# EmilioOlivastri/IPC

Hardware: AMD Instinct MI355X
Metric: candidate-pairs/s (consistency matrix + set-max) (higher is better)
Workload: dtype f64; 1 GPU; C2: INTEL-like SE2 synthetic (V=1228, 256 true loops) + 1000 injected outliers; N=1256 candidates, 789396 cells (i<=j), 531545 solved on rank 0, s=10, fast 6.251/50, slow 11.345/100; parallelism=1 GPU

## Files before the change

__graft_entry__.py:

```python
import os
import subprocess
import sys

ROOT = os.path.dirname(os.path.abspath(__file__))
if ROOT not in sys.path:
    sys.path.insert(0, ROOT)

CSRC = os.path.join(ROOT, "ipc_amd", "csrc")
LIB = os.path.join(ROOT, "ipc_amd", "libipc_amd.so")


def _newer(target, sources):
    if not os.path.exists(target):
        return False
    t = os.path.getmtime(target)
    return all(os.path.getmtime(s) <= t for s in sources)


UNITS = ["engine.hip", "se2_block.hip", "se2_wave.hip", "se2_wave_kt.hip", "se2_pair.hip", "se2_pair_kt.hip", "se2_quad.hip",
         "se3_block.hip",
         "se3_lds_a.hip", "se3_lds_b.hip", "se3_lds_c.hip", "se3_lds_d.hip", "se3_lds_e.hip"]


HIP_FLAGS = ["--offload-arch=gfx950", "-O3", "-std=c++17", "-fPIC", "-Wno-unused-value", "-ffp-contract=on"]


def _build_lib(lib, extra_flags=(), objdir=None):
    from concurrent.futures import ThreadPoolExecutor
    hipcc = os.environ.get("HIPCC", "/opt/rocm/bin/hipcc")
    objdir = objdir or os.path.join(ROOT, "build")
    os.makedirs(objdir, exist_ok=True)
    flags = HIP_FLAGS + list(extra_flags)
    hdrs = [os.path.join(CSRC, f) for f in os.listdir(CSRC) if f.endswith((".hpp", ".h"))]
    hdrs += [os.path.join(ROOT, "include", f) for f in ("ipc_amd.h", "ipc_amd_online_exact.h")]

    def compile_unit(u):
        src, obj = os.path.join(CSRC, u), os.path.join(objdir, u.replace(".hip", ".o"))
        if not _newer(obj, [src] + hdrs) or extra_flags:
            subprocess.check_call([hipcc] + flags + ["-c", src, "-o", obj])
        return obj

    with ThreadPoolExecutor(max_workers=min(len(UNITS), os.cpu_count() or 4)) as ex:
        objs = list(ex.map(compile_unit, UNITS))
    subprocess.check_call([hipcc, "--offload-arch=gfx950", "-shared", "-fPIC", "-o", lib] + objs)


def build(force=False):
    srcs = [os.path.join(CSRC, f) for f in sorted(os.listdir(CSRC)) if f.endswith((".hip", ".hpp", ".h"))]
    srcs += [os.path.join(ROOT, "include", f) for f in ("ipc_amd.h", "ipc_amd_online_exact.h")]
    if force or not _newer(LIB, srcs):
        _build_lib(LIB)
    host = os.path.join(ROOT, "ipc_amd", "host")
    hsrc = [os.path.join(host, f) for f in ("ipc_tester.cpp", "ipc_host.cpp", "ipc_host.hpp")] + [LIB]
    for d in (2, 3):
        exe = os.path.join(host, "ipc_tester_%dD" % d)
        if force or not _newer(exe, hsrc):
            subprocess.check_call(["g++", "-O2", "-std=c++17", "-DIPC_TESTER_DIM=%d" % d, "-o", exe,
                                   os.path.join(host, "ipc_tester.cpp"), os.path.join(host, "ipc_host.cpp"),
                                   "-L" + os.path.join(ROOT, "ipc_amd"), "-lipc_amd",
                                   "-Wl,-rpath,$ORIGIN/..", "-Wl,-rpath,/opt/rocm/lib"])
    gen = os.path.join(host, "generateDataset")
    gsrc = os.path.join(host, "generate_dataset.cpp")
    if force or not _newer(gen, [gsrc]):
        subprocess.check_call(["g++", "-O2", "-std=c++17", "-o", gen, gsrc])
    from oracle import oracle as O
    O.build(force=force)
    import ipc_amd
    from ipc_amd import capi
    capi.load()


def smoke():
    import numpy as np
    from ipc_amd import capi
    capi.export_recommended_environment()
    from ipc_amd import synth
    from ipc_amd.consensus import IPC, Config, unpack_bits
    from oracle import oracle as O

    g = synth.inject_outliers(synth.small_se2(), 6, seed=3)
    cfg = Config(s_factor=10.0)
    eng = IPC(g, cfg, device=0)
    bits, acc = eng.run()
    C = unpack_bits(bits, eng.N)
    ok, _ = O.consistency_matrix(2, g.odom_meas, g.odom_info, cfg.s_factor, g.loop_ids, g.loop_meas,
                                 g.loop_info, cfg.fast_reject_th, cfg.fast_reject_iter_base,
                                 cfg.slow_reject_th, cfg.slow_reject_iter_base)
    ref_acc = O.set_max(ok, O.candidate_order(g.loop_ids))
    assert np.array_equal(C, ok), "consistency matrix differs from the oracle"
    assert np.array_equal(acc, ref_acc), "accepted set differs from the oracle"
    print("smoke OK: N=%d cells=%d accepted=%d" % (eng.N, len(eng.cell_info()), int(acc.sum())))


if __name__ == "__main__":
    build()
    if len(sys.argv) > 1 and sys.argv[1] == "smoke":
        smoke()
```

include/ipc_amd.h:

```cpp
#ifndef IPC_AMD_H
#define IPC_AMD_H

#include <stddef.h>
#include <stdint.h>

#ifdef __cplusplus
extern "C" {
#endif

typedef struct ipc_engine ipc_engine_t;

typedef enum {
    IPC_OK = 0,
    IPC_ERR_ARG = -1,
    IPC_ERR_HIP = -2,
    IPC_ERR_STATE = -3,
    IPC_ERR_LIMIT = -4
} ipc_status;

typedef struct {
    double fast_reject_th;
    int    fast_reject_iter_base;
    double slow_reject_th;
    int    slow_reject_iter_base;
    double s_factor;
} ipc_params_t;

typedef struct {
    int    i, j;
    int    lo, hi;
    double max_chi2;
    double chi2_total;
    int    iterations;
    int    tries;
    int    flags;
    int    evals;
} ipc_cell_info_t;

const char* ipc_last_error(void);

int ipc_create(int dim, int n_vertices, const double* odom_meas, const double* odom_info,
               const ipc_params_t* params, int device, ipc_engine_t** out);

int ipc_destroy(ipc_engine_t* h);

int ipc_set_candidates(ipc_engine_t* h, int n, const int* ids, const double* meas,
                       const double* info);

int ipc_append_candidate(ipc_engine_t* h, const int* ids, const double* meas, const double* info, int* index_out);

int ipc_append_odometry(ipc_engine_t* h, int n_edges, const double* meas, const double* info);
int ipc_reserve_vertices(ipc_engine_t* h, int capacity);
int ipc_vertex_count(ipc_engine_t* h, int* n_vertices);

int ipc_candidate_order(ipc_engine_t* h, int* order_out);

int ipc_initial_poses(ipc_engine_t* h, double* poses_out);


int ipc_rows_per_rank(int n, int world);

int ipc_row_assignment(int n, const int* ids, int world, int policy, int* slot_out);

int ipc_solve_rows(ipc_engine_t* h, int rank, int world, uint64_t* d_upper, void* stream);

typedef struct {
    int cells;
    int long_cells;
    int failed_cells;
    int capped_cells;
    int nan_cells;
    int damped_cells;
    int literal_cells;
} ipc_solve_report_t;
int ipc_solve_report(ipc_engine_t* h, ipc_solve_report_t* out);

int ipc_assemble_matrix(ipc_engine_t* h, const uint64_t* d_gathered, int world,
                        uint64_t* d_bits, void* stream);

int ipc_set_max(ipc_engine_t* h, const uint64_t* d_bits, uint8_t* d_accepted, void* stream);

int ipc_run(ipc_engine_t* h, uint64_t* bits_out, uint8_t* accepted_out);

int ipc_run_set_only(ipc_engine_t* h, uint8_t* accepted_out, int* solved_cells_out);

int ipc_run_sharded(ipc_engine_t** engines, int n_engines, uint64_t* bits_out, uint8_t* accepted_out);

typedef struct {
    int covered_before, covered_after;
    int cells;
    int long_cells, literal_cells, damped_cells;
    int set_max_resumed;
    int grew;
} ipc_online_report_t;
int ipc_run_online(ipc_engine_t* h, uint64_t* bits_out, uint8_t* accepted_out, ipc_online_report_t* report);
int ipc_online_covered(ipc_engine_t* h, int* m);
int ipc_online_reset(ipc_engine_t* h);
int ipc_reserve_candidates(ipc_engine_t* h, int capacity);

typedef struct {
    int thresholds;
    int cells;
    int long_cells, damped_cells;
    int literal_cells;
    int literal_held;
    int reused_solve;
    int chunks;
} ipc_sweep_report_t;
int ipc_run_sweep(ipc_engine_t* h, int n_th, const double* fast_th, const double* slow_th, uint64_t* bits_out,
                  uint8_t* accepted_out, ipc_sweep_report_t* report);
int ipc_sweep_reset(ipc_engine_t* h);

typedef struct {
    int runs;
    int union_candidates;
    int cells;
    long long cells_separate;
    int long_cells, damped_cells, literal_cells;
    int chunks;
} ipc_batch_report_t;
int ipc_run_batch(ipc_engine_t* h, int n_runs, const int* run_offsets, const int* members, uint64_t* bits_out,
                  uint8_t* accepted_out, ipc_batch_report_t* report);

typedef struct {
    int live;
    int greedy_size;
    int best_size;
    int best_seed;
    int best_seed_position;
} ipc_multistart_report_t;
int ipc_set_max_multistart(ipc_engine_t* h, const uint64_t* d_bits, uint8_t* d_accepted, int32_t* d_sizes, void* stream);
int ipc_run_multistart(ipc_engine_t* h, uint64_t* bits_out, uint8_t* accepted_out, uint8_t* greedy_out, int32_t* sizes_out,
                       ipc_multistart_report_t* report);

typedef struct {
    int live, multistart_size, size, upper_bound, proven;
    int subproblems;
    int capped;
    long long steps;
} ipc_exact_report_t;
int ipc_set_max_exact(ipc_engine_t* h, const uint64_t* d_bits, uint8_t* d_accepted, ipc_exact_report_t* report, void* stream);
int ipc_run_exact(ipc_engine_t* h, uint64_t* bits_out, uint8_t* accepted_out, uint8_t* multistart_out, ipc_exact_report_t* report);

#include "ipc_amd_online_exact.h"

int ipc_cell_count(ipc_engine_t* h, int* n_cells);
int ipc_cell_info(ipc_engine_t* h, ipc_cell_info_t* out, int capacity);

int ipc_solver_time_ms(ipc_engine_t* h, double* ms, int* launches);

int ipc_synchronize(ipc_engine_t* h);


typedef struct {
    int    lo, hi;
    int    n_cluster_loops;
    int    iterations, tries, flags;
    double max_chi2;
    double chi2_total;
    double chi2_initial;
} ipc_check_info_t;

int ipc_incremental_reset(ipc_engine_t* h);

int ipc_incremental_prepare(ipc_engine_t* h);

int ipc_agreement_check(ipc_engine_t* h, int k, int* agrees, ipc_check_info_t* info);

typedef struct {
    long host_solver_fallbacks, lost_launches, relaunches, literal_band_solves;
} ipc_incremental_counters_t;
int ipc_incremental_counters(ipc_engine_t* h, ipc_incremental_counters_t* out);

int ipc_consensus_size(ipc_engine_t* h, int* n);
int ipc_consensus_set(ipc_engine_t* h, int* out);

int ipc_remove_from_consensus(ipc_engine_t* h, int k, int* removed);
int ipc_add_to_consensus(ipc_engine_t* h, int k);

int ipc_current_poses(ipc_engine_t* h, double* poses_out);

int ipc_incremental_set_state(ipc_engine_t* h, const double* poses, const int* cns, int n_cns, int resume_position);

int ipc_final_optimize(ipc_engine_t* h, const uint8_t* accepted, int iterations, double* poses_out,
                       ipc_check_info_t* info);

int ipc_debug_dense_solve(int n, const double* system, int mode, int workgroups, double* x_out, int* info_out);

int ipc_debug_band_solve(int nb, int m, int W, const double* system, int workgroups, double* x_out, int* info_out);
int ipc_debug_absorbed_edges(int klo, int khi, int n, const int* lo, const int* hi, int sweep, int* members_out, int* n_members_out,
                             int* lo_out, int* hi_out);
int ipc_debug_band_plan(int d, int nl, const int* a, const int* b, int min_n, int* use_out, int* nlb_out, int* bwb_out,
                        int* order_out);
int ipc_debug_live_resources(int out[3]);

#ifdef __cplusplus
}
#endif
#endif
```

ipc_amd/capi.py:

```python
import ctypes as C
import os

import numpy as np



def export_recommended_environment():
    os.environ.setdefault("GPU_MAX_HW_QUEUES", "24")


_HERE = os.path.dirname(os.path.abspath(__file__))
LIB_PATH = os.environ.get("IPC_AMD_LIB") or os.path.join(_HERE, "libipc_amd.so")

SYMBOLS = [
    "ipc_last_error", "ipc_create", "ipc_destroy", "ipc_set_candidates", "ipc_candidate_order",
    "ipc_initial_poses", "ipc_rows_per_rank", "ipc_solve_rows", "ipc_assemble_matrix", "ipc_set_max",
    "ipc_run", "ipc_cell_count", "ipc_cell_info", "ipc_solve_report", "ipc_solver_time_ms", "ipc_synchronize",
    "ipc_incremental_reset", "ipc_incremental_prepare", "ipc_agreement_check", "ipc_consensus_size", "ipc_consensus_set",
    "ipc_remove_from_consensus", "ipc_add_to_consensus", "ipc_current_poses", "ipc_final_optimize",
    "ipc_debug_dense_solve", "ipc_debug_band_solve", "ipc_debug_band_plan", "ipc_debug_absorbed_edges", "ipc_append_candidate", "ipc_incremental_set_state", "ipc_incremental_counters", "ipc_row_assignment", "ipc_run_sharded", "ipc_run_set_only",
    "ipc_append_odometry", "ipc_reserve_vertices", "ipc_vertex_count",
    "ipc_run_online", "ipc_online_covered", "ipc_online_reset", "ipc_reserve_candidates", "ipc_debug_live_resources",
    "ipc_run_sweep", "ipc_sweep_reset",
    "ipc_run_batch",
    "ipc_set_max_multistart", "ipc_run_multistart",
    "ipc_set_max_exact", "ipc_run_exact",
]
SYMBOLS_ONLINE_EXACT = ["ipc_set_max_exact_resume", "ipc_run_online_exact", "ipc_online_exact_state"]


class Params(C.Structure):
    _fields_ = [("fast_reject_th", C.c_double), ("fast_reject_iter_base", C.c_int),
                ("slow_reject_th", C.c_double), ("slow_reject_iter_base", C.c_int),
                ("s_factor", C.c_double)]


class CellInfo(C.Structure):
    _fields_ = [("i", C.c_int), ("j", C.c_int), ("lo", C.c_int), ("hi", C.c_int),
                ("max_chi2", C.c_double), ("chi2_total", C.c_double),
                ("iterations", C.c_int), ("tries", C.c_int), ("flags", C.c_int), ("evals", C.c_int)]


class CheckInfo(C.Structure):
    _fields_ = [("lo", C.c_int), ("hi", C.c_int), ("n_cluster_loops", C.c_int), ("iterations", C.c_int),
                ("tries", C.c_int), ("flags", C.c_int), ("max_chi2", C.c_double), ("chi2_total", C.c_double),
                ("chi2_initial", C.c_double)]


class IncrementalCounters(C.Structure):
    _fields_ = [("host_solver_fallbacks", C.c_long), ("lost_launches", C.c_long), ("relaunches", C.c_long),
                ("literal_band_solves", C.c_long)]


class SolveReport(C.Structure):
    _fields_ = [("cells", C.c_int), ("long_cells", C.c_int), ("failed_cells", C.c_int), ("capped_cells", C.c_int),
                ("nan_cells", C.c_int), ("damped_cells", C.c_int), ("literal_cells", C.c_int)]


class OnlineReport(C.Structure):
    _fields_ = [("covered_before", C.c_int), ("covered_after", C.c_int), ("cells", C.c_int), ("long_cells", C.c_int),
                ("literal_cells", C.c_int), ("damped_cells", C.c_int), ("set_max_resumed", C.c_int), ("grew", C.c_int)]


class SweepReport(C.Structure):
    _fields_ = [("thresholds", C.c_int), ("cells", C.c_int), ("long_cells", C.c_int), ("damped_cells", C.c_int),
                ("literal_cells", C.c_int), ("literal_held", C.c_int), ("reused_solve", C.c_int), ("chunks", C.c_int)]


class BatchReport(C.Structure):
    _fields_ = [("runs", C.c_int), ("union_candidates", C.c_int), ("cells", C.c_int), ("cells_separate", C.c_longlong),
                ("long_cells", C.c_int), ("damped_cells", C.c_int), ("literal_cells", C.c_int), ("chunks", C.c_int)]


class MultistartReport(C.Structure):
    _fields_ = [("live", C.c_int), ("greedy_size", C.c_int), ("best_size", C.c_int), ("best_seed", C.c_int),
                ("best_seed_position", C.c_int)]


class ExactReport(C.Structure):
    _fields_ = [("live", C.c_int), ("multistart_size", C.c_int), ("size", C.c_int), ("upper_bound", C.c_int),
                ("proven", C.c_int), ("subproblems", C.c_int), ("capped", C.c_int), ("steps", C.c_longlong)]


class ExactResumeReport(C.Structure):
    _fields_ = [("first", C.c_int), ("live", C.c_int), ("newcomers", C.c_int), ("size_before", C.c_int),
                ("multistart_size", C.c_int), ("size", C.c_int), ("upper_bound", C.c_int), ("proven", C.c_int),
                ("changed", C.c_int), ("subproblems", C.c_int), ("capped", C.c_int), ("steps", C.c_longlong)]


CELL_DTYPE = np.dtype([("i", "<i4"), ("j", "<i4"), ("lo", "<i4"), ("hi", "<i4"), ("max_chi2", "<f8"),
                       ("chi2_total", "<f8"), ("iterations", "<i4"), ("tries", "<i4"), ("flags", "<i4"),
                       ("evals", "<i4")])

_lib = None


class IpcError(RuntimeError):
    pass


def load():
    global _lib
    if _lib is not None:
        return _lib
    if not os.path.exists(LIB_PATH):
        raise IpcError("libipc_amd.so is not built (%s); run `python -c 'import __graft_entry__ as g; "
                       "g.build()'` -- there is no CPU fallback" % LIB_PATH)
    try:
        import torch
    except ImportError:
        pass
    lib = C.CDLL(LIB_PATH)
    lib.ipc_last_error.restype = C.c_char_p
    vp, ip, dp = C.c_void_p, C.c_int, C.c_double
    lib.ipc_create.argtypes = [ip, ip, vp, vp, C.POINTER(Params), ip, C.POINTER(vp)]
    lib.ipc_destroy.argtypes = [vp]
    lib.ipc_set_candidates.argtypes = [vp, ip, vp, vp, vp]
    lib.ipc_append_candidate.argtypes = [vp, vp, vp, vp, C.POINTER(ip)]
    lib.ipc_append_odometry.argtypes = [vp, ip, vp, vp]
    lib.ipc_reserve_vertices.argtypes = [vp, ip]
    lib.ipc_vertex_count.argtypes = [vp, C.POINTER(ip)]
    lib.ipc_candidate_order.argtypes = [vp, vp]
    lib.ipc_initial_poses.argtypes = [vp, vp]
    lib.ipc_rows_per_rank.argtypes = [ip, ip]
    lib.ipc_row_assignment.argtypes = [ip, vp, ip, ip, vp]
    lib.ipc_solve_rows.argtypes = [vp, ip, ip, vp, vp]
    lib.ipc_assemble_matrix.argtypes = [vp, vp, ip, vp, vp]
    lib.ipc_set_max.argtypes = [vp, vp, vp, vp]
    lib.ipc_run.argtypes = [vp, vp, vp]
    lib.ipc_run_online.argtypes = [vp, vp, vp, C.POINTER(OnlineReport)]
    lib.ipc_online_covered.argtypes = [vp, C.POINTER(ip)]
    lib.ipc_online_reset.argtypes = [vp]
    lib.ipc_reserve_candidates.argtypes = [vp, ip]
    lib.ipc_run_sweep.argtypes = [vp, ip, vp, vp, vp, vp, C.POINTER(SweepReport)]
    lib.ipc_sweep_reset.argtypes = [vp]
    lib.ipc_run_batch.argtypes = [vp, ip, vp, vp, vp, vp, C.POINTER(BatchReport)]
    lib.ipc_set_max_multistart.argtypes = [vp, vp, vp, vp, vp]
    lib.ipc_run_multistart.argtypes = [vp, vp, vp, vp, vp, C.POINTER(MultistartReport)]
    lib.ipc_set_max_exact.argtypes = [vp, vp, vp, C.POINTER(ExactReport), vp]
    lib.ipc_run_exact.argtypes = [vp, vp, vp, vp, C.POINTER(ExactReport)]
    lib.ipc_set_max_exact_resume.argtypes = [vp, vp, ip, vp, C.POINTER(ExactResumeReport), vp]
    lib.ipc_run_online_exact.argtypes = [vp, vp, vp, vp, C.POINTER(OnlineReport), C.POINTER(ExactResumeReport)]
    lib.ipc_online_exact_state.argtypes = [vp, C.POINTER(ip), C.POINTER(ip)]
    lib.ipc_run_sharded.argtypes =[C.POINTER(vp), ip, vp, vp]
    lib.ipc_run_set_only.argtypes = [vp, vp, C.POINTER(ip)]
    lib.ipc_cell_count.argtypes = [vp, C.POINTER(ip)]
    lib.ipc_cell_info.argtypes = [vp, vp, ip]
    lib.ipc_solve_report.argtypes = [vp, C.POINTER(SolveReport)]
    lib.ipc_solver_time_ms.argtypes = [vp, C.POINTER(dp), C.POINTER(ip)]
    lib.ipc_synchronize.argtypes = [vp]
    lib.ipc_incremental_reset.argtypes = [vp]
    lib.ipc_incremental_prepare.argtypes = [vp]
    lib.ipc_agreement_check.argtypes = [vp, ip, C.POINTER(ip), C.POINTER(CheckInfo)]
    lib.ipc_consensus_size.argtypes = [vp, C.POINTER(ip)]
    lib.ipc_consensus_set.argtypes = [vp, vp]
    lib.ipc_remove_from_consensus.argtypes = [vp, ip, C.POINTER(ip)]
    lib.ipc_add_to_consensus.argtypes = [vp, ip]
    lib.ipc_current_poses.argtypes = [vp, vp]
    lib.ipc_incremental_set_state.argtypes = [vp, vp, vp, ip, ip]
    lib.ipc_incremental_counters.argtypes = [vp, C.POINTER(IncrementalCounters)]
    lib.ipc_final_optimize.argtypes = [vp, vp, ip, vp, C.POINTER(CheckInfo)]
    lib.ipc_debug_dense_solve.argtypes = [ip, vp, ip, ip, vp, C.POINTER(ip)]
    lib.ipc_debug_band_solve.argtypes = [ip, ip, ip, vp, ip, vp, C.POINTER(ip)]
    lib.ipc_debug_absorbed_edges.argtypes = [ip, ip, ip, vp, vp, ip, vp, C.POINTER(ip), C.POINTER(ip), C.POINTER(ip)]
    lib.ipc_debug_band_plan.argtypes = [ip, ip, vp, vp, ip, C.POINTER(ip), C.POINTER(ip), C.POINTER(ip), vp]
    lib.ipc_debug_live_resources.argtypes = [C.POINTER(ip * 3)]
    assert C.sizeof(CellInfo) == CELL_DTYPE.itemsize
    _lib = lib
    return lib


def check(rc):
    if rc != 0:
        raise IpcError("ipc_amd error %d: %s" % (rc, load().ipc_last_error().decode()))
```

ipc_amd/consensus.py:

```python
import ctypes as C
from dataclasses import dataclass

import numpy as np

from . import capi
from .graphio import PoseGraph


@dataclass
class Config:
    fast_reject_th: float = 6.251
    fast_reject_iter_base: int = 50
    slow_reject_th: float = 11.345
    slow_reject_iter_base: int = 100
    s_factor: float = 10.0
    canonic_inliers: int = 0


def _d(a):
    return np.ascontiguousarray(a, dtype=np.float64)


def _p(a):
    return a.ctypes.data_as(C.c_void_p)
# ... 117 lines not shown
        capi.check(self.lib.ipc_reserve_candidates(self.h, int(n)))

    def run_sweep(self, fast_ths, slow_ths, want_bits=False):
        fast, slow = _d(fast_ths).reshape(-1), _d(slow_ths).reshape(-1)
        assert fast.shape == slow.shape
        T = int(fast.shape[0])
        acc = np.zeros((T, self.N), dtype=np.uint8)
        bits = np.zeros((T, self.N, self.words), dtype=np.uint64) if want_bits else None
        r = capi.SweepReport()
        capi.check(self.lib.ipc_run_sweep(self.h, T, _p(fast), _p(slow), _p(bits) if want_bits else None, _p(acc), C.byref(r)))
        report = {k: getattr(r, k) for k, _ in capi.SweepReport._fields_}
        return (bits, acc, report) if want_bits else (acc, report)

    def sweep_reset(self):
        capi.check(self.lib.ipc_sweep_reset(self.h))

    def run_batch(self, runs, want_bits=False):
        runs = [np.ascontiguousarray(r, dtype=np.int32).reshape(-1) for r in runs]
        sizes = [int(r.shape[0]) for r in runs]
        offsets = np.zeros(len(runs) + 1, dtype=np.int32)
        offsets[1:] = np.cumsum(sizes)
        members = np.ascontiguousarray(np.concatenate(runs) if runs else np.zeros(0), dtype=np.int32)
        mats = [n * ((n + 63) // 64) for n in sizes]
        acc = np.zeros(max(int(offsets[-1]), 1), dtype=np.uint8)
        bits = np.zeros(max(sum(mats), 1), dtype=np.uint64) if want_bits else None
        r = capi.BatchReport()
        capi.check(self.lib.ipc_run_batch(self.h, len(runs), _p(offsets), _p(members), _p(bits) if want_bits else None, _p(acc),
                                          C.byref(r)))
        report = {k: getattr(r, k) for k, _ in capi.BatchReport._fields_}
        accs = [acc[offsets[q]:offsets[q + 1]] for q in range(len(runs))]
        if not want_bits:
            return accs, report
        mo = np.concatenate([[0], np.cumsum(mats)])
        return [bits[mo[q]:mo[q + 1]].reshape(sizes[q], -1) for q in range(len(runs))], accs, report

    def run_multistart(self, want_bits=False):
        acc = np.zeros(self.N, dtype=np.uint8)
        greedy = np.zeros(self.N, dtype=np.uint8)
        sizes = np.zeros(self.N, dtype=np.int32)
        bits = np.zeros((self.N, self.words), dtype=np.uint64) if want_bits else None
        r = capi.MultistartReport()
        capi.check(self.lib.ipc_run_multistart(self.h, _p(bits) if want_bits else None, _p(acc), _p(greedy), _p(sizes), C.byref(r)))
        report = {k: getattr(r, k) for k, _ in capi.MultistartReport._fields_}
        return (bits, acc, greedy, sizes, report) if want_bits else (acc, greedy, sizes, report)

    def run_exact(self, want_bits=False):
        acc = np.zeros(self.N, dtype=np.uint8)
        ms = np.zeros(self.N, dtype=np.uint8)
        bits = np.zeros((self.N, self.words), dtype=np.uint64) if want_bits else None
        r = capi.ExactReport()
        capi.check(self.lib.ipc_run_exact(self.h, _p(bits) if want_bits else None, _p(acc), _p(ms), C.byref(r)))
        report = {k: getattr(r, k) for k, _ in capi.ExactReport._fields_}
        return (bits, acc, ms, report) if want_bits else (acc, ms, report)

    def consistency_matrix(self):
        bits, _ = self.run()
        return unpack_bits(bits, self.N)

    def getMaxConsensusSet(self):
        return self._max_consensus_set

    def reset(self):
        capi.check(self.lib.ipc_incremental_reset(self.h))
        self._max_consensus_set = np.zeros(0, dtype=np.int32)

    def agreementCheck(self, k, with_info=False):
        ok, info = C.c_int(0), capi.CheckInfo()
        capi.check(self.lib.ipc_agreement_check(self.h, int(k), C.byref(ok), C.byref(info)))
        self._max_consensus_set = self._consensus()
        return (bool(ok.value), info) if with_info else bool(ok.value)

    def _consensus(self):
        n = C.c_int(0)
        capi.check(self.lib.ipc_consensus_size(self.h, C.byref(n)))
        out = np.zeros(max(n.value, 1), dtype=np.int32)
        capi.check(self.lib.ipc_consensus_set(self.h, _p(out)))
        return out[:n.value]

    def removeEdgeFromCnS(self, k):
        r = C.c_int(0)
        capi.check(self.lib.ipc_remove_from_consensus(self.h, int(k), C.byref(r)))
        self._max_consensus_set = self._consensus()
        return bool(r.value)

    def addEdgeToCnS(self, k):
        capi.check(self.lib.ipc_add_to_consensus(self.h, int(k)))
        self._max_consensus_set = self._consensus()

    def current_poses(self):
        out = np.zeros((self.n_vertices, 3 if self.dim == 2 else 12))
        capi.check(self.lib.ipc_current_poses(self.h, _p(out)))
        return out

    def set_state(self, poses, consensus, resume_position=0):
        poses = _d(poses)
        assert poses.shape == (self.n_vertices, 3 if self.dim == 2 else 12)
        cns = np.ascontiguousarray(consensus, dtype=np.int32)
        capi.check(self.lib.ipc_incremental_set_state(self.h, _p(poses), _p(cns), int(cns.shape[0]), int(resume_position)))
        self._max_consensus_set = cns.copy()

    def incremental_counters(self):
        c = capi.IncrementalCounters()
        capi.check(self.lib.ipc_incremental_counters(self.h, C.byref(c)))
        return {k: getattr(c, k) for k, _ in capi.IncrementalCounters._fields_}

    def final_optimize(self, accepted, iterations=1000):
        acc = np.ascontiguousarray(accepted, dtype=np.uint8)
        out = np.zeros((self.n_vertices, 3 if self.dim == 2 else 12))
        info = capi.CheckInfo()
        capi.check(self.lib.ipc_final_optimize(self.h, _p(acc), int(iterations), _p(out), C.byref(info)))
        return out, info

    def rows_per_rank(self, world):
        return self.lib.ipc_rows_per_rank(self.N, world)

    def solve_rows(self, rank, world, d_upper_ptr, stream=0):
        capi.check(self.lib.ipc_solve_rows(self.h, rank, world, C.c_void_p(d_upper_ptr), C.c_void_p(stream)))

    def assemble_matrix(self, d_gathered_ptr, world, d_bits_ptr, stream=0):
        capi.check(self.lib.ipc_assemble_matrix(self.h, C.c_void_p(d_gathered_ptr), world,
                                                C.c_void_p(d_bits_ptr), C.c_void_p(stream)))

    def set_max(self, d_bits_ptr, d_accepted_ptr, stream=0):
        capi.check(self.lib.ipc_set_max(self.h, C.c_void_p(d_bits_ptr), C.c_void_p(d_accepted_ptr),
                                        C.c_void_p(stream)))

    def set_max_multistart(self, d_bits_ptr, d_accepted_ptr, d_sizes_ptr=0, stream=0):
        capi.check(self.lib.ipc_set_max_multistart(self.h, C.c_void_p(d_bits_ptr), C.c_void_p(d_accepted_ptr),
                                                   C.c_void_p(d_sizes_ptr) if d_sizes_ptr else None, C.c_void_p(stream)))

    def set_max_exact(self, d_bits_ptr, d_accepted_ptr, stream=0):
        r = capi.ExactReport()
        capi.check(self.lib.ipc_set_max_exact(self.h, C.c_void_p(d_bits_ptr), C.c_void_p(d_accepted_ptr), C.byref(r), C.c_void_p(stream)))
        return {k: getattr(r, k) for k, _ in capi.ExactReport._fields_}

    def set_max_exact_resume(self, d_bits_ptr, first, d_accepted_ptr, stream=0):
        r = capi.ExactResumeReport()
        capi.check(self.lib.ipc_set_max_exact_resume(self.h, C.c_void_p(d_bits_ptr), int(first), C.c_void_p(d_accepted_ptr), C.byref(r),
                                                     C.c_void_p(stream)))
        return {k: getattr(r, k) for k, _ in capi.ExactResumeReport._fields_}

    def cell_info(self):
        n = C.c_int(0)
        capi.check(self.lib.ipc_cell_count(self.h, C.byref(n)))
        out = np.zeros(max(n.value, 1), dtype=capi.CELL_DTYPE)
        capi.check(self.lib.ipc_cell_info(self.h, _p(out), n.value))
        return out[:n.value]

    def solve_report(self):
        r = capi.SolveReport()
        capi.check(self.lib.ipc_solve_report(self.h, C.byref(r)))
        return {k: getattr(r, k) for k, _ in capi.SolveReport._fields_}

    def solver_time_ms(self):
        ms, nl = C.c_double(0), C.c_int(0)
        capi.check(self.lib.ipc_solver_time_ms(self.h, C.byref(ms), C.byref(nl)))
        return ms.value, nl.value

    def synchronize(self):
        capi.check(self.lib.ipc_synchronize(self.h))

    def close(self):
        if getattr(self, "h", None) is not None and self.h:
            self.lib.ipc_destroy(self.h)
            self.h = None

    def __del__(self):
        try:
            self.close()
        except Exception:
            pass


def unpack_bits(bits, N):
    b = np.ascontiguousarray(bits, dtype=np.uint64)
    u8 = b.view(np.uint8).reshape(b.shape[0], -1)
    return np.unpackbits(u8, axis=1, bitorder="little")[:, :N].astype(np.uint8)
```

ipc_amd/csrc/cell_kernels.hpp:

```cpp
#pragma once
#include <hip/hip_runtime.h>

#include "se2_cell.hpp"
#include "se3_cell.hpp"

namespace ipc {

struct CellOut {
    double* max_chi2;
    double* chi2_total;
    int4* meta;
};

struct Variant { int W, M; };
static const Variant kVariants[] = {
    {1, 1}, {2, 1}, {3, 1}, {4, 1}, {5, 1}, {6, 1}, {7, 1}, {8, 1}, {10, 1}, {12, 1}, {14, 1}, {16, 1},
    {4, 2}, {5, 2}, {6, 2}, {7, 2}, {8, 2}, {10, 2}, {12, 2}, {16, 2},
    {5, 3}, {6, 3}, {7, 3}, {8, 3},
    {4, 4}, {6, 4}, {8, 4}, {16, 4}, {16, 8}, {16, 16},
    {2, 3}, {2, 4}, {2, 5}, {2, 6},
    {3, 4}, {3, 5}, {3, 6}, {4, 3}, {4, 5},
};
constexpr int kNumVariants = sizeof(kVariants) / sizeof(kVariants[0]);
static const Variant kVariants3[] = { {1, 1}, {2, 1}, {4, 1}, {8, 1}, {16, 1}, {16, 2}, {16, 4},
                                      {4, 2}, {4, 4}, {8, 2}, {8, 4}, {4, 8}, {8, 5},
                                      {1, 2}, {2, 2}, {1, 4}, {2, 4}, {1, 3}, {2, 3} };
constexpr int kNumVariants3 = sizeof(kVariants3) / sizeof(kVariants3[0]);

hipError_t launch_se2_block(int nl, int variant, int n, hipStream_t st, const Se2View& P, const int2* cells,
                            SolveParams prm, CellOut out);
hipError_t launch_se3_block(int nl, int variant, int n, hipStream_t st, const Se3View& P, const int2* cells,
                            SolveParams prm, CellOut out);

struct LdsVariant { int W, M; };
static const LdsVariant kLdsVariants3[] = { {1, 1}, {1, 2}, {1, 3}, {1, 4}, {1, 6}, {1, 8},
                                            {4, 2}, {4, 3}, {4, 4}, {4, 5}, {4, 6}, {4, 7}, {4, 8}, {4, 9}, {4, 10} };
constexpr int kNumLdsVariants3 = sizeof(kLdsVariants3) / sizeof(kLdsVariants3[0]);
constexpr int kLdsVariantBase3 = 400;
#define IPC_SE3_LDS_DECL(WW, MM)                                                                                \
    hipError_t launch_se3_lds_##WW##_##MM(int nl, int n, hipStream_t st, const Se3View& P, const int2* cells,   \
                                          SolveParams prm, CellOut out, unsigned* counter, int n_cu);
IPC_SE3_LDS_DECL(1, 1) IPC_SE3_LDS_DECL(1, 2) IPC_SE3_LDS_DECL(1, 3) IPC_SE3_LDS_DECL(1, 4) IPC_SE3_LDS_DECL(1, 6)
IPC_SE3_LDS_DECL(1, 8) IPC_SE3_LDS_DECL(4, 2) IPC_SE3_LDS_DECL(4, 3) IPC_SE3_LDS_DECL(4, 4) IPC_SE3_LDS_DECL(4, 5)
IPC_SE3_LDS_DECL(4, 6) IPC_SE3_LDS_DECL(4, 7) IPC_SE3_LDS_DECL(4, 8) IPC_SE3_LDS_DECL(4, 9) IPC_SE3_LDS_DECL(4, 10)
#undef IPC_SE3_LDS_DECL

static const int kWaveM[] = {1, 3, 5, 7, 9, 11, 13};
constexpr int kNumWaveM = sizeof(kWaveM) / sizeof(kWaveM[0]);
constexpr int kWaveVariantBase = 100;

hipError_t launch_se2_wave(int nl, int M, int n, hipStream_t st, const Se2View& P, const int2* cells,
                           SolveParams prm, CellOut out, unsigned* counter, int n_cu);

static const int kPairM[] = {5, 7, 9, 11};
constexpr int kNumPairM = sizeof(kPairM) / sizeof(kPairM[0]);
constexpr int kPairVariantBase = 200;
hipError_t launch_se2_pair(int nl, int M, int n, hipStream_t st, const Se2View& P, const int2* cells,
                           SolveParams prm, CellOut out, unsigned* counter, int n_cu);

static const int kQuadM[] = {7, 9, 11, 13};
constexpr int kNumQuadM = sizeof(kQuadM) / sizeof(kQuadM[0]);
constexpr int kQuadVariantBase = 300;
hipError_t launch_se2_quad(int nl, int M, int n, hipStream_t st, const Se2View& P, const int2* cells,
                           SolveParams prm, CellOut out, unsigned* counter, int n_cu);

static const int kWaveKtM[] = {5, 7, 9, 11};
constexpr int kNumWaveKtM = sizeof(kWaveKtM) / sizeof(kWaveKtM[0]);
constexpr int kWaveKtVariantBase = 500;
hipError_t launch_se2_wave_kt(int nl, int M, int n, hipStream_t st, const Se2View& P, const int2* cells,
                              SolveParams prm, CellOut out, unsigned* counter, int n_cu);
static const int kPairKtM[] = {7, 9, 11};
constexpr int kNumPairKtM = sizeof(kPairKtM) / sizeof(kPairKtM[0]);
constexpr int kPairKtVariantBase = 600;
hipError_t launch_se2_pair_kt(int nl, int M, int n, hipStream_t st, const Se2View& P, const int2* cells,
                              SolveParams prm, CellOut out, unsigned* counter, int n_cu);

}
```

ipc_amd/csrc/engine.hip:

```cpp
#include <hip/hip_runtime.h>

#include <algorithm>
#include <cstdarg>
#include <cstdlib>
#include <utility>
#include <cstdio>
#include <cstring>
#include <numeric>
#include <map>
#include <memory>
#include <mutex>
#include <string>
#include <chrono>
#include <thread>
#include <vector>

#include "../../include/ipc_amd.h"
#include "cell_kernels.hpp"
#include "cluster_se2.hpp"
#include "cluster_se3.hpp"
#include "cluster_persist.hpp"

using namespace ipc;

static thread_local std::string g_err;
static int fail(int code, const char* fmt, ...)
{
    char buf[512];
    va_list ap;
    va_start(ap, fmt);
    vsnprintf(buf, sizeof buf, fmt, ap);
    va_end(ap);
    g_err = buf;
    return code;
}
#define HIPCHK(expr)                                                                       \
    do {                                                                                   \
        hipError_t e_ = (expr);                                                            \
        if (e_ != hipSuccess)                                                              \
            return fail(IPC_ERR_HIP, "%s failed: %s (%s:%d)", #expr, hipGetErrorString(e_), \
                        __FILE__, __LINE__);                                               \
    } while (0)

extern "C" const char* ipc_last_error(void) { return g_err.c_str(); }

constexpr int kMaxBins = 32;
struct BinCaps { int n; int cap[kMaxBins]; };

__device__ __forceinline__ int bin_of(const BinCaps& bc, int L)
{
    int b = 0;
    while (b < bc.n && L > bc.cap[b]) ++b;
    return b;
}

__device__ __forceinline__ void inv_sym3(const double* a, double* o)
{
    const double c00 = a[3] * a[5] - a[4] * a[4];
    const double c01 = a[2] * a[4] - a[1] * a[5];
    const double c02 = a[1] * a[4] - a[2] * a[3];
    const double det = a[0] * c00 + a[1] * c01 + a[2] * c02;
    const double id = 1.0 / det;
    o[0] = c00 * id; o[1] = c01 * id; o[2] = c02 * id;
    o[3] = (a[0] * a[5] - a[2] * a[2]) * id;
    o[4] = (a[1] * a[2] - a[0] * a[4]) * id;
    o[5] = (a[0] * a[3] - a[1] * a[1]) * id;
}

__device__ __forceinline__ void se2_prep_record(const double* m, const double* inf, double scale, double unscale, double* rec,
                                                int stride, int k)
{
    const double tx = m[0], ty = m[1], th = m[2];
    double s, c;
    sincos(th, &s, &c);
    rec[(size_t)F_TZX * stride + k] = tx;
    rec[(size_t)F_TZY * stride + k] = ty;
    rec[(size_t)F_CZ * stride + k] = c;
    rec[(size_t)F_SZ * stride + k] = s;
    rec[(size_t)F_THZ * stride + k] = th;
    double om[6], sg[6];
    for (int q = 0; q < 6; ++q) om[q] = unscale == 1.0 ? inf[q] * scale : (inf[q] * scale) / unscale;
    inv_sym3(om, sg);
    for (int q = 0; q < 6; ++q) {
        rec[(size_t)(F_OM + q) * stride + k] = om[q];
        rec[(size_t)(F_SG + q) * stride + k] = sg[q];
    }
}
__global__ void k_se2_prep(int n, const double* meas, const double* info, double scale, double* rec, int stride,
                           double unscale = 1.0)
{
    const int k = blockIdx.x * blockDim.x + threadIdx.x;
    if (k >= n) return;
    se2_prep_record(meas + 3 * (size_t)k, info + 6 * (size_t)k, scale, unscale, rec, stride, k);
}

__global__ void k_records(int n, int nf, const double* rec, int stride, double* out)
{
    const int k = blockIdx.x * blockDim.x + threadIdx.x;
    if (k >= n) return;
    for (int f = 0; f < nf; ++f) out[(size_t)k * nf + f] = rec[(size_t)f * stride + k];
}

__device__ __forceinline__ void se2_compose_step(double& x, double& y, double& th, const double* rec, int stride, int i)
{
    double s, c;
    sincos(th, &s, &c);
    const double tx = rec[(size_t)F_TZX * stride + i - 1], ty = rec[(size_t)F_TZY * stride + i - 1];
    x += c * tx - s * ty;
    y += s * tx + c * ty;
    th = normalize_theta(th + rec[(size_t)F_THZ * stride + i - 1]);
}
__global__ void k_se2_propagate(int V, const double* rec, int stride, double* pose0, int vs)
{
    if (threadIdx.x != 0 || blockIdx.x != 0) return;
    double x = 0, y = 0, th = 0;
    pose0[0] = x; pose0[vs] = y; pose0[2 * (size_t)vs] = th;
    for (int i = 1; i < V; ++i) {
        se2_compose_step(x, y, th, rec, stride, i);
        pose0[i] = x; pose0[(size_t)vs + i] = y; pose0[2 * (size_t)vs + i] = th;
    }
}

__device__ void inv_sym6(const double* up, double* out)
{
    double A[6][6], Li[6][6];
    for (int i = 0; i < 6; ++i)
        for (int j = 0; j < 6; ++j) { A[i][j] = up[sym6_idx(i, j)]; Li[i][j] = 0.0; }
    for (int i = 0; i < 6; ++i)
        for (int j = 0; j <= i; ++j) {
            double sum = A[i][j];
            for (int k = 0; k < j; ++k) sum -= A[i][k] * A[j][k];
            A[i][j] = (j < i) ? sum / A[j][j] : sqrt(sum);
        }
    for (int c = 0; c < 6; ++c)
        for (int i = c; i < 6; ++i) {
            double sum = (i == c) ? 1.0 : 0.0;
            for (int k = c; k < i; ++k) sum -= A[i][k] * Li[k][c];
            Li[i][c] = sum / A[i][i];
        }
    for (int i = 0; i < 6; ++i)
        for (int j = i; j < 6; ++j) {
            double sum = 0.0;
            for (int k = j; k < 6; ++k) sum += Li[k][i] * Li[k][j];
            out[sym6_idx(i, j)] = sum;
        }
}

__device__ __forceinline__ void se3_prep_record(const double* m, const double* inf, double scale, double unscale, double* rec,
                                                int stride, int k)
{
    const double qn = sqrt(m[3] * m[3] + m[4] * m[4] + m[5] * m[5] + m[6] * m[6]);
    double R[9];
    R_from_quat(m[6] / qn, m[3] / qn, m[4] / qn, m[5] / qn, R);
    for (int q = 0; q < 9; ++q) rec[(size_t)(G_RZ + q) * stride + k] = R[q];
    for (int q = 0; q < 3; ++q) rec[(size_t)(G_TZ + q) * stride + k] = m[q];
// ... 203 lines not shown
            if (lane == r) mine = word;
        }
        if (vr) bits[(size_t)ir * words + w] = mine;
    }
}

__device__ __forceinline__ void assemble_tiles(int N, int M, int stride, const int* lo, const int* hi,
                                               const unsigned long long* upper, unsigned long long* bits)
{
    const int lane = threadIdx.x & 63, wave = threadIdx.x >> 6;
    const int w = blockIdx.x;
    auto U = [&](int a, int c) -> unsigned {
        const unsigned long long word = upper[(size_t)a * stride + (c >> 6)];
        return (unsigned)((word >> (c & 63)) & 1ull);
    };
    const int w0 = M >> 6, w1 = (N - 1) >> 6;
    const bool neww = w >= w0;
    const unsigned long long keep = (w == w0 && (M & 63)) ? (1ull << (M & 63)) - 1ull : 0ull;
    const int j = w * 64 + lane;
    const bool vj = j < N;
    const int loj = vj ? lo[j] : 0, hij = vj ? hi[j] : 0;
    const unsigned long long Dword = __ballot(vj && U(j, j));
    for (int rb = (neww ? 0 : w0) + blockIdx.y * 4 + wave; rb <= w1; rb += gridDim.y * 4) {
        const int ir = rb * 64 + lane;
        const bool vr = ir < N;
        const int lor = vr ? lo[ir] : 0, hir = vr ? hi[ir] : 0;
        const unsigned long long dmask = __ballot(vr && U(ir, ir));
        const int nrows = min(64, N - rb * 64);
        unsigned long long mine = 0ull;
        for (int r = 0; r < nrows; ++r) {
            const int i = rb * 64 + r;
            if (i < M && !neww) continue;
            const int loi = __builtin_amdgcn_readlane(lor, r), hii = __builtin_amdgcn_readlane(hir, r);
            unsigned long long word = ((dmask >> r) & 1ull) ? Dword : 0ull;
            const bool ov = vj && j != i && (min(hii, hij) - max(loi, loj) > 0);
            const unsigned long long ovmask = __ballot(ov);
            if (ovmask) {
                const bool bit = ov && U(min(i, j), max(i, j));
                word = (word & ~ovmask) | __ballot(bit);
            }
            if (lane == r) mine = word;
        }
        if (vr) {
            unsigned long long* dst = bits + (size_t)ir * stride + w;
            if (ir >= M) *dst = mine;
            else if (neww) *dst = keep ? ((*dst & keep) | (mine & ~keep)) : mine;
        }
    }
}
__global__ __launch_bounds__(256) void k_assemble_delta(int N, int M, int stride, const int* lo, const int* hi,
                                                        const unsigned long long* upper, unsigned long long* bits)
{
    assemble_tiles(N, M, stride, lo, hi, upper, bits);
}

__device__ __forceinline__ void set_max_rounds(int N, int words, int stride, const int* order,
                                               const unsigned long long* bits, unsigned char* accepted, int* live,
                                               int first, unsigned long long* mask, int* nlive_io)
{
    constexpr int CPW = 4, RC = 16 * CPW;
    extern __shared__ unsigned long long acc[];
    __shared__ int okflag[RC];
    __shared__ unsigned long long conf[RC];
    __shared__ int kk[RC];
    __shared__ int wcount[16];
    __shared__ int nlive_s;
    const int tid = threadIdx.x, wave = tid >> 6, lane = tid & 63;
    for (int w = tid; w < words; w += blockDim.x) acc[w] = first ? mask[w] : 0ull;
    if (first) { for (int q = first + tid; q < N; q += blockDim.x) accepted[order[q]] = 0; }
    else { for (int k = tid; k < N; k += blockDim.x) accepted[k] = 0; }
    if (tid == 0) nlive_s = first ? *nlive_io : 0;
    __syncthreads();
    const int nlive0 = nlive_s;
    for (int base = first; base < N; base += 1024) {
        const int pos = base + tid;
        const int k = pos < N ? order[pos] : -1;
        const bool keep = k >= 0 && ((bits[(size_t)k * stride + (k >> 6)] >> (k & 63)) & 1ull);
        const unsigned long long m = __ballot(keep);
        if (lane == 0) wcount[wave] = __popcll(m);
        __syncthreads();
        int off = nlive_s;
        for (int v = 0; v < wave; ++v) off += wcount[v];
        if (keep) live[off + __popcll(m & ((1ull << lane) - 1ull))] = k;
        __syncthreads();
        if (tid == 0) { int t = 0; for (int v = 0; v < 16; ++v) t += wcount[v]; nlive_s += t; }
        __syncthreads();
    }
    __threadfence_block();
    const int nlive = nlive_s;
    for (int base = nlive0; base < nlive; base += RC) {
        int k[CPW];
        bool bad[CPW];
#pragma unroll
        for (int c = 0; c < CPW; ++c) {
            const int pos = base + c * 16 + wave;
            k[c] = pos < nlive ? live[pos] : -1;
            bad[c] = false;
        }
        for (int w = lane; w < words; w += 64) {
            const unsigned long long a = acc[w];
#pragma unroll
            for (int c = 0; c < CPW; ++c) {
                const unsigned long long r = k[c] >= 0 ? bits[(size_t)k[c] * stride + w] : ~0ull;
                bad[c] = bad[c] || (r & a) != a;
            }
        }
#pragma unroll
        for (int c = 0; c < CPW; ++c) {
            const bool ok = k[c] >= 0 && __ballot(bad[c]) == 0ull;
            if (lane == 0) { okflag[c * 16 + wave] = ok ? 1 : 0; kk[c * 16 + wave] = k[c]; }
        }
        __syncthreads();
#pragma unroll
        for (int c = 0; c < CPW; ++c) {
            if (k[c] < 0) continue;
            unsigned m = 0;
            if (lane < RC && kk[lane] >= 0) {
                const int o = kk[lane];
                m = (unsigned)((bits[(size_t)k[c] * stride + (o >> 6)] >> (o & 63)) & 1ull);
            }
            const unsigned long long bal = __ballot(m != 0);
            if (lane == 0) conf[c * 16 + wave] = bal;
        }
        __syncthreads();
        if (tid == 0) {
            unsigned long long taken = 0;
            for (int w = 0; w < RC; ++w) {
                if (kk[w] < 0 || !okflag[w]) continue;
                if ((conf[w] & taken) != taken) continue;
                taken |= 1ull << w;
                acc[kk[w] >> 6] |= 1ull << (kk[w] & 63);
                accepted[kk[w]] = 1;
            }
        }
        __syncthreads();
    }
    if (mask) {
        for (int w = tid; w < words; w += blockDim.x) mask[w] = acc[w];
        if (tid == 0) *nlive_io = nlive;
    }
}
__global__ __launch_bounds__(1024) void k_set_max(int N, int words, int stride, const int* order,
                                                  const unsigned long long* bits, unsigned char* accepted, int* live,
                                                  int first = 0, unsigned long long* mask = nullptr, int* nlive_io = nullptr)
{
    set_max_rounds(N, words, stride, order, bits, accepted, live, first, mask, nlive_io);
}

struct BinPlan {
    BinCaps caps;
    int variant[kMaxBins];
    int latency_variant[kMaxBins];
    int latency_below[kMaxBins];
};
static const char* kDefaultPolicy = "w1,w3,kw5,kw7,kw9,w11,w13,kp7,kp9,p11,q7,q9,q11,q13,16x4,16x8,16x16";
static const int kDefaultSideStreams2 = 7, kDefaultSideStreams3 = 7;
static const char* kDefaultPolicy3 = "w1,w2,w3,w4,w6,w8,g3,g4,g5,g6,g7,g8,g9,g10,16x4";
static const char* kBlockPolicy3 = "1x1,1x2,1x3,2x2,2x3,4x2,4x4,8x4,8x5,16x4";
static const char* kDefaultLatencyPolicy3 = "1x1,2x1,4x1,4x2,4x4,8x4,8x5,16x4";
static bool make_plan(BinPlan& bp, int dim, std::string& err)
{
    const char* env = getenv(dim == 2 ? "IPC_SE2_POLICY" : "IPC_SE3_POLICY");
    std::string pol = env && *env ? env : (dim == 2 ? kDefaultPolicy : kDefaultPolicy3);
    if (dim == 3 && pol == "block") pol = kBlockPolicy3;
    const Variant* table = dim == 2 ? kVariants : kVariants3;
    const int ntable = dim == 2 ? kNumVariants : kNumVariants3;
    std::vector<std::pair<int, int>> items;
    size_t pos = 0;
    while (pos < pol.size()) {
        size_t e = pol.find(',', pos);
        if (e == std::string::npos) e = pol.size();
        int w = 0, m = 0;
        const std::string tok = pol.substr(pos, e - pos);
        int v = -1;
        if (dim == 2 && sscanf(tok.c_str(), "kw%d", &m) == 1) {
            w = 1;
            for (int k = 0; k < kNumWaveKtM; ++k) if (kWaveKtM[k] == m) v = kWaveKtVariantBase + m;
        } else if (dim == 2 && sscanf(tok.c_str(), "kp%d", &m) == 1) {
            w = 2;
            for (int k = 0; k < kNumPairKtM; ++k) if (kPairKtM[k] == m) v = kPairKtVariantBase + m;
        } else if (dim == 2 && sscanf(tok.c_str(), "w%d", &m) == 1) {
            w = 1;
            for (int k = 0; k < kNumWaveM; ++k) if (kWaveM[k] == m) v = kWaveVariantBase + m;
        } else if (dim == 2 && sscanf(tok.c_str(), "p%d", &m) == 1) {
            w = 2;
            for (int k = 0; k < kNumPairM; ++k) if (kPairM[k] == m) v = kPairVariantBase + m;
        } else if (dim == 2 && sscanf(tok.c_str(), "q%d", &m) == 1) {
            w = 4;
            for (int k = 0; k < kNumQuadM; ++k) if (kQuadM[k] == m) v = kQuadVariantBase + m;
        } else if (dim == 3 && (sscanf(tok.c_str(), "w%d", &m) == 1 || sscanf(tok.c_str(), "g%d", &m) == 1)) {
            w = tok[0] == 'w' ? 1 : 4;
            for (int k = 0; k < kNumLdsVariants3; ++k)
                if (kLdsVariants3[k].W == w && kLdsVariants3[k].M == m) v = kLdsVariantBase3 + k;
        } else {
            if (sscanf(tok.c_str(), "%dx%d", &w, &m) != 2) { err = "bad IPC_SE2_POLICY token"; return false; }
            for (int k = 0; k < ntable; ++k) if (table[k].W == w && table[k].M == m) v = k;
        }
        if (v < 0) { err = "IPC_SE*_POLICY names a variant that is not compiled: " + tok; return false; }
        items.push_back({64 * w * m, v});
        pos = e + 1;
    }
    std::sort(items.begin(), items.end());
    if (items.empty() || (int)items.size() > kMaxBins) { err = "IPC_SE2_POLICY: 1..32 variants"; return false; }
    bp.caps.n = (int)items.size();
    for (int b = 0; b < kMaxBins; ++b) {
        bp.caps.cap[b] = b < bp.caps.n ? items[b].first : 0;
        bp.variant[b] = b < bp.caps.n ? items[b].second : -1;
        bp.latency_variant[b] = -1;
        bp.latency_below[b] = 0;
    }
    if (dim == 3) {
        const char* lenv = getenv("IPC_SE3_LATENCY_POLICY");
        const std::string lpol = lenv && *lenv ? lenv : kDefaultLatencyPolicy3;
        if (lpol != "none") {
            size_t lp = 0;
            std::vector<std::pair<int, int>> lat;
            while (lp < lpol.size()) {
                size_t e = lpol.find(',', lp);
                if (e == std::string::npos) e = lpol.size();
                int w = 0, m = 0, v = -1;
                if (sscanf(lpol.substr(lp, e - lp).c_str(), "%dx%d", &w, &m) != 2) { err = "bad IPC_SE3_LATENCY_POLICY token"; return false; }
                for (int k = 0; k < ntable; ++k) if (table[k].W == w && table[k].M == m) v = k;
                if (v < 0) { err = "IPC_SE3_LATENCY_POLICY names a variant that is not compiled"; return false; }
                lat.push_back({64 * w * m, v});
                lp = e + 1;
            }
            std::sort(lat.begin(), lat.end());
            for (int b = 0; b < bp.caps.n; ++b) {
                if (bp.variant[b] >= kLdsVariantBase3) continue;
                const int wt = table[bp.variant[b]].W;
                for (const auto& lv : lat) {
                    if (lv.first < bp.caps.cap[b]) continue;
                    if (table[lv.second].W > wt) {
                        bp.latency_variant[b] = lv.second;
                        bp.latency_below[b] = wt <= 4 ? 4 / wt : 1;
                    }
                    break;
                }
            }
        }
    }
    return true;
}

static hipError_t launch_se3_lds(int nl, int idx, int n, hipStream_t st, const Se3View& P, const int2* cells,
                                 SolveParams prm, CellOut out, unsigned* counter, int n_cu)
{
#define IPC_LCASE(i, WW, MM) case i: return launch_se3_lds_##WW##_##MM(nl, n, st, P, cells, prm, out, counter, n_cu);
    switch (idx) {
        IPC_LCASE(0, 1, 1) IPC_LCASE(1, 1, 2) IPC_LCASE(2, 1, 3) IPC_LCASE(3, 1, 4) IPC_LCASE(4, 1, 6) IPC_LCASE(5, 1, 8)
        IPC_LCASE(6, 4, 2) IPC_LCASE(7, 4, 3) IPC_LCASE(8, 4, 4) IPC_LCASE(9, 4, 5) IPC_LCASE(10, 4, 6) IPC_LCASE(11, 4, 7)
        IPC_LCASE(12, 4, 8) IPC_LCASE(13, 4, 9) IPC_LCASE(14, 4, 10)
        default: return hipErrorInvalidValue;
    }
#undef IPC_LCASE
}

struct BatchRun;
struct ipc_engine {
    struct OwnStream {
        hipStream_t s = nullptr;
        ~OwnStream() { if (s) hipStreamDestroy(s); }
        operator hipStream_t() const { return s; }
    } own_stream;
    int dim = 2, V = 0, N = 0, device = 0;
    int vcap = 0;
    PinnedBuf<double> h_stage; double* d_stage = nullptr; size_t stage_cap = 0;
    Event ev_stage; bool stage_used = false;
    long chain_growths = 0;
    ipc_params_t prm{};
    double term_eps = 1e-13;
    BinPlan plan{};
    DevBuf<double> d_chain; int estride = 0;
    DevBuf<double> d_chain_rec;
    DevBuf<double2> d_chain_blk;
    DevBuf<double> d_pose0;
    DevBuf<double> d_cand; int cstride = 0;
    DevBuf<int> d_from, d_to, d_lo, d_hi, d_order;
    DevBuf<int> d_live;
    DevBuf<int> d_rowperm;
    std::vector<int> row_group_off;
    bool order_stale = false;
    std::vector<DevBuf<void>> retired;
    Event ev_cand; bool cand_event = false;
    std::vector<int> order, h_lo, h_hi;
    std::vector<int> h_cand_ids; std::vector<double> h_cand_meas, h_cand_info;
    DevBuf<unsigned> d_counters;
    DevBuf<unsigned> d_offsets;
    DevBuf<unsigned> d_wave_ctr;
    int n_cu = 256;
    struct CellBufs {
        DevBuf<int2> d_cells, d_lit_cells; DevBuf<double> d_chi, d_chitot, d_lit_chi, d_lit_chitot; DevBuf<int4> d_meta, d_lit_meta;
        DevBuf<int> d_lit_idx;
        ScratchCap cap;
    } cells;
    bool plan_cached = false; int plan_rank = -1, plan_world = 0; size_t plan_total = 0;
    int slow_first_iterations = 96;
    std::vector<unsigned> plan_counts, plan_offsets;
    DevBuf<unsigned> d_slot_off;
    DevBuf<int> d_recount; PinnedBuf<int> h_recount;
    int last_cells = 0, last_long_cells = 0;
    Event ev0, ev1; bool ev_valid = false; int last_launches = 0;
    static constexpr int kMaxSide = 7;
    int n_side = 0;
    bool side_forced = false;
    hipStream_t side[kMaxSide] = {};
    Event ev_fork, ev_join[kMaxSide], ev_join_own;
    struct RunScratch { DevBuf<uint64_t> d_upper, d_bits; DevBuf<unsigned char> d_acc; ScratchCap cap; } run;
    int on_cov = 0, on_ccap = 0, on_wcap = 0, reserved_cands = 0;
    DevBuf<unsigned long long> d_on_upper, d_on_bits;
    DevBuf<unsigned long long> d_on_mask;
    DevBuf<unsigned char> d_on_acc;
    DevBuf<int> d_on_live;
    long online_growths = 0;
    bool sw_valid = false;
    bool info_from_sweep = false;
    size_t sw_total = 0;
    int sw_long = 0, sw_damped = 0, sw_held = 0;
    struct SweepScratch {
        DevBuf<int2> d_cells; DevBuf<double> d_chi, d_chitot, d_lit; DevBuf<int4> d_meta; DevBuf<int> d_flags;
        ScratchCap cap;
        DevBuf<double> d_th; ScratchCap th;
        DevBuf<unsigned long long> d_upper, d_bits; DevBuf<unsigned char> d_acc; DevBuf<int> d_live;
        ScratchCap mat, vec;
    } sw;
    DevBuf<unsigned> d_sw_slot_off;
    std::vector<unsigned> sw_counts, sw_offsets;
    int sweep_chunk = 0;
    struct BatchScratch {
        DevBuf<unsigned long long> d_memb, d_sep; ScratchCap memb;
        DevBuf<unsigned long long> d_upper, d_bits; ScratchCap mat;
        DevBuf<unsigned char> d_acc; DevBuf<int> d_vec; ScratchCap vec;
        DevBuf<int> d_loc; ScratchCap loc;
        DevBuf<BatchRun> d_runs; ScratchCap runs;
        PinnedBuf<unsigned long long> h_stage; ScratchCap stage;
    } bt;
    int batch_chunk = 0;
    size_t batch_budget = 0;
    struct MultistartScratch {
        DevBuf<unsigned long long> d_P; ScratchCap mat;
        DevBuf<int> d_vec, d_info; DevBuf<unsigned char> d_acc; ScratchCap vec;
        int* live() const { return vec.part(d_vec, 0); }
        int* pos() const { return vec.part(d_vec, 1); }
        int* sz() const { return vec.part(d_vec, 2); }
        int* sizes() const { return vec.part(d_vec, 3); }
    } ms;
    int ms_reg_words = 2;
    struct ExactScratch {
        DevBuf<int> d_info, d_vec; ScratchCap vec;
        DevBuf<unsigned long long> d_ws; ScratchCap ws;
        DevBuf<unsigned short> d_clq; ScratchCap clq;
        DevBuf<int> d_rinfo, d_roots; ScratchCap roots;
        DevBuf<unsigned long long> d_new;
        int* flag() const { return vec.part(d_vec, 0); }
        int* sizes() const { return vec.part(d_vec, 1); }
        unsigned* steps() const { return (unsigned*)vec.part(d_vec, 2); }
    } ex;
    unsigned ex_step_cap = 1u << 20;
    DevBuf<unsigned char> d_on_exact;
    int on_ex_cov = 0, on_ex_proven = 0;
    bool on_ex_resume = true;
    std::vector<double> h_odom_meas, h_odom_info;
    std::vector<int> h_from, h_to, cns;
    DevBuf<double> d_chain1;
    double* d_open = nullptr;
    DevBuf<double> d_open_own;
    DevBuf<double> d_cur;
    std::unique_ptr<ClusterSolver<PersistSe2>> cluster;
    std::unique_ptr<ClusterSolver<PersistSe3>> cluster3;
    bool persist = true;
    bool last_persist = false;
    DevBuf<int> d_slot; int slot_world = 0; int row_policy = 1;
    struct FailedList { DevBuf<int> d_list; ScratchCap cap; } failed;
    int last_lm_cells = 0;
    bool lm_retry = true;
    double borderline_band = -1.0;
    int last_literal_cells = 0;
    long lm_fallbacks = 0;
    long persist_timeouts = 0;
    long persist_relaunches = 0;
    bool cns_dups = false;
    std::unique_ptr<PersistSolver<PersistSe2>> persist2;
    std::unique_ptr<PersistSolver<PersistSe3>> persist3;
    DevBuf<unsigned long long> d_prof;
    int max_helpers = -1;
    PersistKnobs knobs;
    int literal_band_min_n = 3072;
    struct SpecSlot {
        std::unique_ptr<PersistSolver<PersistSe2>> s2;
        std::unique_ptr<PersistSolver<PersistSe3>> s3;
        hipStream_t st = nullptr;
        Event done;
        int cand = -1, pos = -1;
        int state = -1;
        int launch_id = 0;
        int busy_wgs = 0;
        int expect = -1;
        std::chrono::steady_clock::time_point t_launch;
        int lo = 0, hi = 0, nclu = 0;
        double th = 0.0;
        double pred_ratio = -1.0;
    };
    struct SpecState {
        double* d_poses = nullptr;
        DevBuf<double> own_poses;
        bool owned = false;
        Event ready;
        bool has_ready = false;
        std::vector<int> cns;
        int pos = -1;
        int users = 0;
        bool live = false;
        double* d_pred = nullptr; PinnedBuf<double> h_pred; int pred_cap = 0, pred_n = 0;
        Event pred_ev; bool has_pred = false, pred_ready = false;
    };
    struct SpecResult {
        bool valid = false, agree = false, retry_host = false;
        int state = -1, child = -1;
        int lo = 0, hi = 0, nclu = 0;
        ClusterOut o;
    };
    std::vector<SpecSlot> slots;
    std::vector<SpecState> spec_states;
    std::vector<int> tent;
    std::vector<SpecResult> spec_res;
    int committed_state = -1;
    std::vector<int> porder, ppos;
    std::vector<char> handed;
    int spec_head = -1;
    int spec_window = 4, spec_ahead = 256;
    bool window_forced = false;
    int stream_concurrency = 0;
    int spec_active = 0;
    double accept_rate = 0.5;
    std::vector<char> pred_accept;
    double pred_k = 30.0;
    std::vector<double> pred_last;
    int spec_behind = 1;
    double uncertain_from = 0.0;
    int xcd_cus = 0;
    int spec_hedge = 0;
    int helper_limit_reject = 8;
    double gate_release_ms = 0.0;
    int helper_limit = 39;
    double st_acc_s = 0, st_rej_s = 0; long st_acc_it = 0, st_rej_it = 0, st_acc_n = 0, st_rej_n = 0;
    double st_acc_dev_s = 0, st_rej_dev_s = 0;
    unsigned long long commit_count = 0;
    Event ev_commit;
    PinnedBuf<int> h_abort;
    int* d_abort = nullptr;
    int next_launch_id = 1;
    long spec_hits = 0, spec_launches = 0, spec_wasted = 0, spec_tentative = 0, spec_promoted = 0;
    double spec_t_launch = 0, spec_t_tent = 0, spec_t_total = 0;
    unsigned long long idle_why[5] = {0, 0, 0, 0, 0};
// ... 689 lines not shown
    }
}
__global__ void k_slow_first_permute(int ncells, const unsigned* slot_off, int nslots, const int* excl_normal, const int2* cells,
                                     const double* chi, const double* chitot, const int4* meta, int2* cells2, double* chi2,
                                     double* chitot2, int4* meta2)
{
    const int c = blockIdx.x * blockDim.x + threadIdx.x;
    if (c >= ncells) return;
    const int sl = slot_of_cell(slot_off, nslots, c);
    const int s0 = (int)slot_off[sl], s1 = (int)slot_off[sl + 1];
    const int n0 = excl_normal[s0], nc = excl_normal[c], n1 = excl_normal[s1];
    const bool normal = excl_normal[c + 1] != nc;
    const int nslow = (s1 - s0) - (n1 - n0);
    const int dst = normal ? s0 + nslow + (nc - n0) : s0 + ((c - s0) - (nc - n0));
    cells2[dst] = cells[c]; chi2[dst] = chi[c]; chitot2[dst] = chitot[c]; meta2[dst] = meta[c];
}

__global__ void k_scatter_literal(int ncells, const unsigned* slot_off, int nslots, const int* recount, const int* lit_idx,
                                  const double* lit_chi, const double* lit_chitot, const int4* lit_meta, double* chi, double* chitot, int4* meta)
{
    const int t = blockIdx.x * blockDim.x + threadIdx.x;
    if (t >= ncells) return;
    const int sl = slot_of_cell(slot_off, nslots, t);
    if ((int)(t - slot_off[sl]) >= recount[sl]) return;
    const int c = lit_idx[t];
    chi[c] = lit_chi[t]; chitot[c] = lit_chitot[t]; meta[c] = lit_meta[t];
}
static int host_cell_solve(ipc_engine* h, int2 cell, bool damped, bool literal, ClusterOut& o)
{
    const int i = cell.x, j = cell.y, nl = i == j ? 1 : 2;
    const int lo = std::min(h->h_lo[i], h->h_lo[j]), hi = std::max(h->h_hi[i], h->h_hi[j]);
    std::vector<int> members{i};
    if (nl == 2) members.push_back(j);
    int iters = nl == 1 ? h->prm.fast_reject_iter_base : h->prm.slow_reject_iter_base;
    if ((hi - lo) + nl > 100) iters *= 5;
    if (damped) {
        HIPCHK(cluster_solve(h, h->d_chain, h->d_open, lo, hi, members, iters, o, true));
        return IPC_OK;
    }
    const double te = h->term_eps;
    auto set_eps = [&](double v) {
        with_host(h, [&](auto& s) { s.term_eps = v; });
        with_persist(h, [&](auto& s) { s.term_eps = v; });
    };
    if (literal) set_eps(0.0);
    const hipError_t e = cluster_solve(h, h->d_chain, h->d_open, lo, hi, members, iters, o);
    if (literal) set_eps(te);
    HIPCHK(e);
    return IPC_OK;
}

static int resolve_failed_cells(ipc_engine* h, int n)
{
    h->last_lm_cells = 0;
    if (n == 0) return IPC_OK;
    n = std::min(n, (int)h->failed.cap.size());
    if (int rc = ensure_incremental(h, "ipc_solve_rows")) return rc;
    std::vector<int> idx(n);
    HIPCHK(hipMemcpy(idx.data(), h->failed.d_list, sizeof(int) * n, hipMemcpyDeviceToHost));
    std::sort(idx.begin(), idx.end());
    for (int q = 0; q < n; ++q) {
        int2 cell;
        HIPCHK(hipMemcpy(&cell, h->cells.d_cells + idx[q], sizeof(int2), hipMemcpyDeviceToHost));
        ClusterOut o;
        int4 was;
        HIPCHK(hipMemcpy(&was, h->cells.d_meta + idx[q], sizeof(int4), hipMemcpyDeviceToHost));
        if (was.z & 2) {
            if (int rc = host_cell_solve(h, cell, true, false, o)) return rc;
            ++h->last_lm_cells;
        } else {
            if (int rc = host_cell_solve(h, cell, false, true, o)) return rc;
            ++h->last_literal_cells;
        }
        const int4 meta = make_int4(o.iterations, o.tries, o.flags, o.evals);
        HIPCHK(hipMemcpy(h->cells.d_chi + idx[q], &o.max_chi2, sizeof(double), hipMemcpyHostToDevice));
        HIPCHK(hipMemcpy(h->cells.d_chitot + idx[q], &o.chi2_total, sizeof(double), hipMemcpyHostToDevice));
        HIPCHK(hipMemcpy(h->cells.d_meta + idx[q], &meta, sizeof(int4), hipMemcpyHostToDevice));
    }
    HIPCHK(hipStreamSynchronize(nullptr));
    return IPC_OK;
}

static int solve_rows_impl(ipc_engine* h, int rank, int world, uint64_t* d_upper, void* stream, int phase);

constexpr int kPlanSlots = 2 * (kMaxBins + 1);
struct CellPlan { unsigned counts[kPlanSlots], offsets[kPlanSlots]; size_t total = 0; };

template <class LaunchPass>
static int plan_cells(ipc_engine* h, hipStream_t st, CellPlan& pl, size_t min_cap, LaunchPass&& launch_pass)
{
    constexpr int NS = kPlanSlots;
    unsigned* counts = pl.counts; unsigned* offsets = pl.offsets;
    size_t total = 0;
    h->plan_cached = false;
    HIPCHK(hipMemsetAsync(h->d_counters, 0, sizeof(unsigned) * NS * kPlanSub, st));
    launch_pass((int2*)nullptr, 0);
    HIPCHK(hipGetLastError());
    static thread_local unsigned subcounts[NS * kPlanSub], suboffsets[NS * kPlanSub];
    HIPCHK(hipMemcpyAsync(subcounts, h->d_counters, sizeof subcounts, hipMemcpyDeviceToHost, st));
    HIPCHK(hipStreamSynchronize(st));
    for (int s = 0; s < NS; ++s) {
        counts[s] = 0;
        for (int q = 0; q < kPlanSub; ++q) counts[s] += subcounts[s * kPlanSub + q];
    }
    for (int s = 0; s < NS; ++s) { offsets[s] = (unsigned)total; total += counts[s]; }
    for (int s = 0; s < NS; ++s) {
        unsigned o = offsets[s];
        for (int q = 0; q < kPlanSub; ++q) { suboffsets[s * kPlanSub + q] = o; o += subcounts[s * kPlanSub + q]; }
    }
    if (auto& c = h->cells; std::max(total, min_cap) > c.cap.size()) {
        const size_t cap = std::max(total + total / 8 + 1024, min_cap);
        HIPCHK(c.cap.grow(cap, sized(c.d_cells, cap), sized(c.d_chi, cap), sized(c.d_chitot, cap), sized(c.d_meta, cap), sized(c.d_lit_cells, cap),
                          sized(c.d_lit_idx, cap + 1), sized(c.d_lit_chi, cap), sized(c.d_lit_chitot, cap), sized(c.d_lit_meta, cap)));
    }
    if (!h->h_recount) {
        HIPCHK(h->d_slot_off.alloc(NS + 1));
        HIPCHK(h->d_recount.alloc(NS + 1));
        HIPCHK(h->h_recount.alloc(NS + 1));
    }
    static thread_local unsigned slot_off[NS + 1];
    for (int s = 0; s < NS; ++s) slot_off[s] = offsets[s];
    slot_off[NS] = (unsigned)total;
    HIPCHK(hipMemcpyAsync(h->d_slot_off, slot_off, sizeof slot_off, hipMemcpyHostToDevice, st));
    HIPCHK(hipMemcpyAsync(h->d_offsets, suboffsets, sizeof suboffsets, hipMemcpyHostToDevice, st));
    HIPCHK(hipMemsetAsync(h->d_counters, 0, sizeof(unsigned) * NS * kPlanSub, st));
    launch_pass(h->cells.d_cells, 1);
    HIPCHK(hipGetLastError());
    pl.total = total;
    return IPC_OK;
}
static int solve_planned(ipc_engine* h, hipStream_t st, const CellPlan& pl);

extern "C" int ipc_solve_rows(ipc_engine_t* h, int rank, int world, uint64_t* d_upper, void* stream)
{
    if (!h) return fail(IPC_ERR_ARG, "ipc_solve_rows: NULL handle");
    if (h->N <= 0) return fail(IPC_ERR_STATE, "ipc_solve_rows: no candidates set");
    if (world < 1 || rank < 0 || rank >= world) return fail(IPC_ERR_ARG, "ipc_solve_rows: rank %d of %d", rank, world);
    if (!d_upper) return fail(IPC_ERR_ARG, "ipc_solve_rows: d_upper is NULL");
    return solve_rows_impl(h, rank, world, d_upper, stream, 0);
}

struct SlotLauncher {
    const ipc_engine* h;
    Se2View P; Se3View P3; SolveParams sp;
    SlotLauncher(const ipc_engine* e, bool literal)
        : h(e), P(make_view(e)), P3(make_view3(e)), sp{e->prm.fast_reject_iter_base, e->prm.slow_reject_iter_base}
    {
        if (literal) { P.term_eps = 0.0; P3.term_eps = 0.0; }
    }
    hipError_t operator()(int b, int nl, int n, const int2* cells, const CellOut& out, hipStream_t ls, unsigned* ctr) const
    {
        int var = h->plan.variant[b];
        if (h->plan.latency_variant[b] >= 0 && n < h->plan.latency_below[b] * h->n_cu) var = h->plan.latency_variant[b];
        if (h->dim == 2)
            return var >= kPairKtVariantBase ? launch_se2_pair_kt(nl, var - kPairKtVariantBase, n, ls, P, cells, sp, out, ctr, h->n_cu)
                   : var >= kWaveKtVariantBase ? launch_se2_wave_kt(nl, var - kWaveKtVariantBase, n, ls, P, cells, sp, out, ctr, h->n_cu)
                   : var >= kQuadVariantBase ? launch_se2_quad(nl, var - kQuadVariantBase, n, ls, P, cells, sp, out, ctr, h->n_cu)
                   : var >= kPairVariantBase ? launch_se2_pair(nl, var - kPairVariantBase, n, ls, P, cells, sp, out, ctr, h->n_cu)
                   : var >= kWaveVariantBase ? launch_se2_wave(nl, var - kWaveVariantBase, n, ls, P, cells, sp, out, ctr, h->n_cu)
                                             : launch_se2_block(nl, var, n, ls, P, cells, sp, out);
        if (var >= kLdsVariantBase3) return launch_se3_lds(nl, var - kLdsVariantBase3, n, ls, P3, cells, sp, out, ctr, h->n_cu);
        return launch_se3_block(nl, var, n, ls, P3, cells, sp, out);
    }
};

static double borderline_band_of(const ipc_engine* h)
{
    return h->term_eps > 0 ? (h->borderline_band >= 0 ? h->borderline_band : 4.0 * std::sqrt(h->term_eps)) : 0.0;
}

static int solve_first_pass(ipc_engine* h, hipStream_t st, const CellPlan& pl)
{
    constexpr int NS = kPlanSlots;
    const unsigned* counts = pl.counts; const unsigned* offsets = pl.offsets;
    const size_t total = pl.total;
    const int nb = h->plan.caps.n;
    const unsigned n_long = counts[nb] + counts[(kMaxBins + 1) + nb];
    const SlotLauncher launch_slot(h, false);
    int launches = 0;
    HIPCHK(hipMemsetAsync(h->d_wave_ctr, 0, sizeof(unsigned) * NS, st));
    HIPCHK(hipEventRecord(h->ev0, st));
    const int n_side = h->side_forced || total < 300000 ? h->n_side : std::min(h->n_side, h->dim == 2 ? 2 : 3);
    hipStream_t st0 = n_side ? h->own_stream : st;
    if (n_side) {
        HIPCHK(hipEventRecord(h->ev_fork, st));
        if (st0 != st) HIPCHK(hipStreamWaitEvent(st0, h->ev_fork, 0));
        for (int k = 0; k < n_side; ++k) HIPCHK(hipStreamWaitEvent(h->side[k], h->ev_fork, 0));
    }
    for (int b = nb - 1; b >= 0; --b) {
        for (int nl = 2; nl >= 1; --nl) {
            const int s = (nl == 1 ? 0 : (kMaxBins + 1)) + b;
            if (!counts[s]) continue;
            CellOut out{h->cells.d_chi + offsets[s], h->cells.d_chitot + offsets[s], h->cells.d_meta + offsets[s]};
            const int lane_q = launches % (n_side + 1);
            hipStream_t ls = lane_q == 0 ? st0 : h->side[lane_q - 1];
            const hipError_t e = launch_slot(b, nl, (int)counts[s], h->cells.d_cells + offsets[s], out, ls, h->d_wave_ctr + s);
            if (e != hipSuccess) return fail(IPC_ERR_HIP, "cell kernel launch failed: %s", hipGetErrorString(e));
            ++launches;
        }
    }
    if (st0 != st) {
        HIPCHK(hipEventRecord(h->ev_join_own, st0));
        HIPCHK(hipStreamWaitEvent(st, h->ev_join_own, 0));
    }
    for (int k = 0; k < n_side; ++k) {
        HIPCHK(hipEventRecord(h->ev_join[k], h->side[k]));
        HIPCHK(hipStreamWaitEvent(st, h->ev_join[k], 0));
    }
    if (n_long) {
        if (int rc = solve_long_cells(h, st, nb, counts, offsets)) return rc;
    }
    HIPCHK(hipEventRecord(h->ev1, st));
    h->ev_valid = true;
    h->last_launches = launches;
    h->last_cells = (int)total;
    h->last_long_cells = (int)n_long;
    h->last_lm_cells = h->last_literal_cells = 0;
    h->info_from_sweep = false;
    return IPC_OK;
}

static int launch_literal_lists(ipc_engine* h, hipStream_t st, const unsigned* offsets)
{
    constexpr int NS = kPlanSlots;
    const int nb = h->plan.caps.n;
    const SlotLauncher launch_slot(h, true);
    HIPCHK(hipMemsetAsync(h->d_wave_ctr, 0, sizeof(unsigned) * NS, st));
    for (int b = nb - 1; b >= 0; --b) {
        for (int nl = 2; nl >= 1; --nl) {
            const int s = (nl == 1 ? 0 : (kMaxBins + 1)) + b;
            const int n = h->h_recount[s];
            if (!n) continue;
            CellOut out{h->cells.d_lit_chi + offsets[s], h->cells.d_lit_chitot + offsets[s], h->cells.d_lit_meta + offsets[s]};
            const hipError_t e = launch_slot(b, nl, n, h->cells.d_lit_cells + offsets[s], out, st, h->d_wave_ctr + s);
            if (e != hipSuccess) return fail(IPC_ERR_HIP, "cell kernel launch failed: %s", hipGetErrorString(e));
        }
    }
    return IPC_OK;
}

static int ensure_failed_list(ipc_engine* h, size_t total)
{
    if (total <= h->failed.cap.size()) return IPC_OK;
    const size_t cap = std::max<size_t>(16384, total + total / 8);
    HIPCHK(h->failed.cap.grow(cap, sized(h->failed.d_list, cap + 1)));
    return IPC_OK;
}

static int solve_collect(ipc_engine* h, hipStream_t st, const CellPlan& pl, double band)
{
    constexpr int NS = kPlanSlots;
    const size_t total = pl.total;
    const int nb = h->plan.caps.n;
    if (total && (h->lm_retry || band > 0.0)) {
        if (int rc = ensure_failed_list(h, total)) return rc;
        HIPCHK(hipMemsetAsync(h->d_recount, 0, sizeof(int) * (NS + 1), st));
        hipLaunchKernelGGL(k_collect_failed, dim3((unsigned)((total + 255) / 256)), dim3(256), 0, st, (int)total, (const int4*)h->cells.d_meta,
                           (const double*)h->cells.d_chi, (const int2*)h->cells.d_cells, h->prm.fast_reject_th, h->prm.slow_reject_th, band,
                           h->lm_retry, (int)h->failed.cap.size(), h->failed.d_list, h->d_recount, (const unsigned*)h->d_slot_off, NS, h->cells.d_lit_cells, h->cells.d_lit_idx, nb);
        HIPCHK(hipGetLastError());
        HIPCHK(hipMemcpyAsync(h->h_recount, h->d_recount, sizeof(int) * (NS + 1), hipMemcpyDeviceToHost, st));
        HIPCHK(hipStreamSynchronize(st));
        int n_lit = 0;
        for (int s = 0; s < NS; ++s) n_lit += h->h_recount[s];
        if (n_lit) {
            if (int rc = launch_literal_lists(h, st, pl.offsets)) return rc;
            hipLaunchKernelGGL(k_scatter_literal, dim3((unsigned)((total + 255) / 256)), dim3(256), 0, st, (int)total,
                               (const unsigned*)h->d_slot_off, NS, (const int*)h->d_recount, (const int*)h->cells.d_lit_idx, (const double*)h->cells.d_lit_chi,
                               (const double*)h->cells.d_lit_chitot, (const int4*)h->cells.d_lit_meta, h->cells.d_chi, h->cells.d_chitot, h->cells.d_meta);
            HIPCHK(hipGetLastError());
            h->last_literal_cells += n_lit;
        }
        if (h->h_recount[NS]) {
            if (int rc = resolve_failed_cells(h, h->h_recount[NS])) return rc;
        }
    }
    return IPC_OK;
}

static int solve_planned(ipc_engine* h, hipStream_t st, const CellPlan& pl)
{
    if (int rc = solve_first_pass(h, st, pl)) return rc;
    return solve_collect(h, st, pl, borderline_band_of(h));
}

static int plan_rows(ipc_engine* h, hipStream_t st, int rank, int world, int phase, const uint64_t* d_upper, bool keep,
                     CellPlan& pl, bool& cached)
{
    const int N = h->N, words = (N + 63) / 64;
    const BinCaps bc = h->plan.caps;
    constexpr int NS = kPlanSlots;
    cached = phase == 0 && h->plan_cached && h->plan_rank == rank && h->plan_world == world;
    if (cached) {
        std::copy(h->plan_counts.begin(), h->plan_counts.end(), pl.counts);
        std::copy(h->plan_offsets.begin(), h->plan_offsets.end(), pl.offsets);
        pl.total = h->plan_total;
    } else {
        const int nrows = h->row_group_off[rank + 1] - h->row_group_off[rank];
        const int* rows = h->d_rowperm + h->row_group_off[rank];
        const dim3 pgrid((N + 255) / 256, std::max(1, std::min(nrows, 2048))), pblock(256);
        if (int rc = plan_cells(h, st, pl, 0, [&](int2* cells, int fill) {
                hipLaunchKernelGGL(k_plan, pgrid, pblock, 0, st, N, h->d_lo, h->d_hi, rows, nrows, bc, h->d_counters,
                                   h->d_offsets, cells, fill, phase, (const unsigned long long*)d_upper, words);
            })) return rc;
        if (phase == 0 && keep) {
            h->plan_counts.assign(pl.counts, pl.counts + NS);
// ... 766 lines not shown
        for (int k = run_offsets[r]; k < run_offsets[r + 1]; ++k) memb[(size_t)members[k] * mw + (r >> 6)] |= 1ull << (r & 63);
    HIPCHK(hipMemcpyAsync(h->bt.d_memb, memb, sizeof(unsigned long long) * need_memb, hipMemcpyHostToDevice, st));
    HIPCHK(hipMemsetAsync(h->bt.d_sep, 0, sizeof(unsigned long long), st));
    if (int rc = ensure_row_map(h, 1)) return rc;
    CellPlan pl;
    {
        const BinCaps bc = h->plan.caps;
        const dim3 pgrid((N + 255) / 256, std::max(1, std::min(N, 2048))), pblock(256);
        if (int rc = plan_cells(h, st, pl, 0, [&](int2* cells, int fill) {
                hipLaunchKernelGGL(k_plan_batch, pgrid, pblock, 0, st, N, (const int*)h->d_lo, (const int*)h->d_hi, (const int*)h->d_rowperm, N, bc,
                                   h->d_counters, (const unsigned*)h->d_offsets, cells, fill, (const unsigned long long*)h->bt.d_memb, mw, h->bt.d_sep);
            })) return rc;
    }
    const size_t total = pl.total;
    if (int rc = solve_planned(h, st, pl)) return rc;
    ipc_batch_report_t rep{};
    rep.runs = R; rep.union_candidates = N; rep.cells = (int)total;
    rep.long_cells = h->last_long_cells; rep.damped_cells = h->last_lm_cells; rep.literal_cells = h->last_literal_cells;
    {
        unsigned long long sep = 0;
        HIPCHK(hipMemcpyAsync(&sep, h->bt.d_sep, sizeof sep, hipMemcpyDeviceToHost, st));
        HIPCHK(hipStreamSynchronize(st));
        rep.cells_separate = (long long)sep;
    }
    std::vector<int> locmap((size_t)N);
    size_t bits_done = 0;
    for (int q = 0; q < n_chunks; ++q) {
        const int c0 = chunk_first[q], n = chunk_first[q + 1] - c0, v0 = run_offsets[c0];
        const size_t nvec = (size_t)(run_offsets[c0 + n] - v0);
        BatchRun* s_runs = (BatchRun*)(unsigned long long*)h->bt.h_stage;
        int* s_order = (int*)((unsigned long long*)h->bt.h_stage + stage_runs);
        int* s_memb = (int*)((unsigned long long*)h->bt.h_stage + stage_runs + stage_vec);
        int* s_loc = (int*)((unsigned long long*)h->bt.h_stage + stage_runs + 2 * stage_vec);
        size_t mat = 0;
        int max_n = 0;
        for (int rc = 0; rc < n; ++rc) {
            const int r = c0 + rc, nr = run_n(r), words = (nr + 63) / 64, voff = run_offsets[r] - v0;
            s_runs[rc] = BatchRun{nr, words, voff, 0, (long long)mat};
            mat += (size_t)nr * words;
            max_n = std::max(max_n, nr);
            int* loc = s_loc + (size_t)rc * N;
            std::fill(loc, loc + N, -1);
            for (int k = 0; k < nr; ++k) { loc[members[run_offsets[r] + k]] = k; s_memb[voff + k] = members[run_offsets[r] + k]; }
            int pos = 0;
            for (int p = 0; p < N; ++p) { const int l = loc[h->order[p]]; if (l >= 0) s_order[voff + pos++] = l; }
        }
        int* d_live = b.vec.part(b.d_vec, 0); int* d_lo_r = b.vec.part(b.d_vec, 1); int* d_hi_r = b.vec.part(b.d_vec, 2);
        int* d_order_r = b.vec.part(b.d_vec, 3); int* d_memb_r = b.vec.part(b.d_vec, 4);
        HIPCHK(hipMemcpyAsync(h->bt.d_runs, s_runs, sizeof(BatchRun) * n, hipMemcpyHostToDevice, st));
        HIPCHK(hipMemcpyAsync(d_order_r, s_order, sizeof(int) * nvec, hipMemcpyHostToDevice, st));
        HIPCHK(hipMemcpyAsync(d_memb_r, s_memb, sizeof(int) * nvec, hipMemcpyHostToDevice, st));
        HIPCHK(hipMemcpyAsync(h->bt.d_loc, s_loc, sizeof(int) * (size_t)n * N, hipMemcpyHostToDevice, st));
        HIPCHK(hipMemsetAsync(h->bt.d_upper, 0, sizeof(unsigned long long) * mat, st));
        const int max_words = (max_n + 63) / 64, max_tiles = ((max_n - 1) >> 6) + 1;
        hipLaunchKernelGGL(k_batch_gather, dim3((max_n + 255) / 256, n), dim3(256), 0, st, (const BatchRun*)h->bt.d_runs, (const int*)d_memb_r,
                           (const int*)h->d_lo, (const int*)h->d_hi, d_lo_r, d_hi_r);
        if (total)
            hipLaunchKernelGGL(k_batch_scatter, dim3((unsigned)((total + 255) / 256)), dim3(256), 0, st, (int)total, (const int2*)h->cells.d_cells,
                               (const double*)h->cells.d_chi, h->prm.fast_reject_th, h->prm.slow_reject_th, (const unsigned long long*)h->bt.d_memb, mw, c0, n,
                               N, (const BatchRun*)h->bt.d_runs, (const int*)h->bt.d_loc, h->bt.d_upper);
        hipLaunchKernelGGL(k_batch_assemble, dim3(max_words, std::min((max_tiles + 3) / 4, 1024), n), dim3(256), 0, st, (const BatchRun*)h->bt.d_runs,
                           (const int*)d_lo_r, (const int*)d_hi_r, (const unsigned long long*)h->bt.d_upper, h->bt.d_bits);
        hipLaunchKernelGGL(k_batch_set_max, dim3(n), dim3(1024), sizeof(unsigned long long) * max_words, st, (const BatchRun*)h->bt.d_runs,
                           (const int*)d_order_r, (const unsigned long long*)h->bt.d_bits, h->bt.d_acc, d_live);
        HIPCHK(hipGetLastError());
        HIPCHK(hipStreamSynchronize(st));
        if (bits_out) HIPCHK(hipMemcpy(bits_out + bits_done, h->bt.d_bits, sizeof(uint64_t) * mat, hipMemcpyDeviceToHost));
        if (accepted_out) HIPCHK(hipMemcpy(accepted_out + v0, h->bt.d_acc, nvec, hipMemcpyDeviceToHost));
        bits_done += mat;
        ++rep.chunks;
    }
    if (report) *report = rep;
    return IPC_OK;
}

extern "C" int ipc_cell_count(ipc_engine_t* h, int* n_cells)
{
    if (!h || !n_cells) return fail(IPC_ERR_ARG, "ipc_cell_count: NULL argument");
    *n_cells = h->last_cells;
    return IPC_OK;
}

extern "C" int ipc_cell_info(ipc_engine_t* h, ipc_cell_info_t* out, int capacity)
{
    if (!h || !out) return fail(IPC_ERR_ARG, "ipc_cell_info: NULL argument");
    HIPCHK(hipSetDevice(h->device));
    HIPCHK(hipDeviceSynchronize());
    const int n = std::min(capacity, h->last_cells);
    if (n <= 0) return IPC_OK;
    std::vector<int2> cells(n);
    std::vector<double> chi(n), tot(n);
    std::vector<int4> meta(n);
    const bool sw = h->info_from_sweep;
    HIPCHK(hipMemcpy(cells.data(), sw ? h->sw.d_cells : h->cells.d_cells, sizeof(int2) * n, hipMemcpyDeviceToHost));
    HIPCHK(hipMemcpy(chi.data(), sw ? h->sw.d_chi : h->cells.d_chi, sizeof(double) * n, hipMemcpyDeviceToHost));
    HIPCHK(hipMemcpy(tot.data(), sw ? h->sw.d_chitot : h->cells.d_chitot, sizeof(double) * n, hipMemcpyDeviceToHost));
    HIPCHK(hipMemcpy(meta.data(), sw ? h->sw.d_meta : h->cells.d_meta, sizeof(int4) * n, hipMemcpyDeviceToHost));
    for (int c = 0; c < n; ++c) {
        ipc_cell_info_t& o = out[c];
        o.i = cells[c].x; o.j = cells[c].y;
        o.lo = std::min(h->h_lo[o.i], h->h_lo[o.j]);
        o.hi = std::max(h->h_hi[o.i], h->h_hi[o.j]);
        o.max_chi2 = chi[c]; o.chi2_total = tot[c];
        o.iterations = meta[c].x; o.tries = meta[c].y; o.flags = meta[c].z; o.evals = meta[c].w;
    }
    return IPC_OK;
}

__global__ void k_report(int n, const int4* meta, const double* chi, unsigned* out)
{
    const int c = blockIdx.x * blockDim.x + threadIdx.x;
    if (c >= n) return;
    const int4 m = meta[c];
    if (m.z & 2) atomicAdd(&out[0], 1u);
    if (!(m.z & 1) && !(m.z & 2)) atomicAdd(&out[1], 1u);
    if (chi[c] != chi[c]) atomicAdd(&out[2], 1u);
}

extern "C" int ipc_solve_report(ipc_engine_t* h, ipc_solve_report_t* out)
{
    if (!h || !out) return fail(IPC_ERR_ARG, "ipc_solve_report: NULL argument");
    HIPCHK(hipSetDevice(h->device));
    HIPCHK(hipDeviceSynchronize());
    memset(out, 0, sizeof *out);
    out->cells = h->last_cells;
    out->long_cells = h->last_long_cells;
    if (h->last_cells <= 0) return IPC_OK;
    unsigned host[3] = {0, 0, 0};
    HIPCHK(hipMemsetAsync(h->d_counters, 0, sizeof(unsigned) * 3, h->own_stream));
    const bool sw = h->info_from_sweep;
    hipLaunchKernelGGL(k_report, dim3((h->last_cells + 255) / 256), dim3(256), 0, h->own_stream, h->last_cells,
                       (const int4*)(sw ? h->sw.d_meta : h->cells.d_meta), (const double*)(sw ? h->sw.d_chi : h->cells.d_chi), h->d_counters);
    HIPCHK(hipGetLastError());
    HIPCHK(hipMemcpyAsync(host, h->d_counters, sizeof host, hipMemcpyDeviceToHost, h->own_stream));
    HIPCHK(hipStreamSynchronize(h->own_stream));
    out->failed_cells = (int)host[0];
    out->capped_cells = (int)host[1];
    out->nan_cells = (int)host[2];
    out->damped_cells = h->last_lm_cells;
    out->literal_cells = h->last_literal_cells;
    return IPC_OK;
}

extern "C" int ipc_solver_time_ms(ipc_engine_t* h, double* ms, int* launches)
{
    if (!h || !ms) return fail(IPC_ERR_ARG, "ipc_solver_time_ms: NULL argument");
    if (!h->ev_valid) return fail(IPC_ERR_STATE, "ipc_solver_time_ms: no solve recorded");
    HIPCHK(hipSetDevice(h->device));
    HIPCHK(hipEventSynchronize(h->ev1));
    float t = 0;
    HIPCHK(hipEventElapsedTime(&t, h->ev0, h->ev1));
    *ms = t;
    if (launches) *launches = h->last_launches;
    return IPC_OK;
}

#if defined(IPC_PHASE_TIMING)
extern "C" int ipc_dbg_read(ipc_engine_t* h, double* out, int n)
{
    Se2View P = make_view(h);
    hipDeviceSynchronize();
    hipMemcpy(out, P.dbg, sizeof(double) * n, hipMemcpyDeviceToHost);
    return 0;
}
#endif
extern "C" int ipc_synchronize(ipc_engine_t* h)
{
    if (!h) return fail(IPC_ERR_ARG, "ipc_synchronize: NULL handle");
    HIPCHK(hipSetDevice(h->device));
    HIPCHK(hipDeviceSynchronize());
    return IPC_OK;
}

__global__ void k_pose5_init(int V, const double* pose0, int is, double* out, int os, int first = 0)
{
    const int i = first + blockIdx.x * blockDim.x + threadIdx.x;
    if (i >= V) return;
    const double th = pose0[2 * (size_t)is + i];
    double s, c;
    sincos_pi(th, s, c);
    out[i] = pose0[i]; out[(size_t)os + i] = pose0[(size_t)is + i]; out[2 * (size_t)os + i] = th;
    out[3 * (size_t)os + i] = c; out[4 * (size_t)os + i] = s;
}

__global__ void k_se2_propagate_tail(int V, int start, const double* rec, int stride, double* cur)
{
    if (threadIdx.x != 0 || blockIdx.x != 0) return;
    double x = cur[start], y = cur[(size_t)V + start], th = cur[2 * (size_t)V + start];
    double c = cur[3 * (size_t)V + start], s = cur[4 * (size_t)V + start];
    for (int i = start + 1; i < V; ++i) {
        const double tx = rec[(size_t)F_TZX * stride + i - 1], ty = rec[(size_t)F_TZY * stride + i - 1];
        x += c * tx - s * ty;
        y += s * tx + c * ty;
        th = normalize_theta(th + rec[(size_t)F_THZ * stride + i - 1]);
        sincos_pi(th, s, c);
        cur[i] = x; cur[(size_t)V + i] = y; cur[2 * (size_t)V + i] = th;
        cur[3 * (size_t)V + i] = c; cur[4 * (size_t)V + i] = s;
    }
}

__global__ void k_se3_propagate_tail(int V, int start, const double* rec, int stride, double* cur)
{
    if (threadIdx.x != 0 || blockIdx.x != 0) return;
    double R[9], t[3];
    for (int q = 0; q < 9; ++q) R[q] = cur[(size_t)q * V + start];
    for (int q = 0; q < 3; ++q) t[q] = cur[(size_t)(9 + q) * V + start];
    for (int i = start + 1; i < V; ++i) {
        double Rz[9], tz[3], Rn[9], d[3];
        for (int q = 0; q < 9; ++q) Rz[q] = rec[(size_t)(G_RZ + q) * stride + i - 1];
        for (int q = 0; q < 3; ++q) tz[q] = rec[(size_t)(G_TZ + q) * stride + i - 1];
        m3_mul(R, Rz, Rn);
        m3_vec(R, tz, d);
        for (int q = 0; q < 3; ++q) t[q] += d[q];
        for (int q = 0; q < 9; ++q) R[q] = Rn[q];
        for (int q = 0; q < 9; ++q) cur[(size_t)q * V + i] = R[q];
        for (int q = 0; q < 3; ++q) cur[(size_t)(9 + q) * V + i] = t[q];
    }
}

__global__ void k_cand_own_chi2_se2(const double* poses, int V, const double* cand, int cstride, const int* from, const int* to,
                                    int n, double* out)
{
    const int c = blockIdx.x * blockDim.x + threadIdx.x;
    if (c >= n) return;
    const int ia = from[c], ib = to[c];
    const Pose2 a{poses[ia], poses[V + ia], poses[2 * (size_t)V + ia], poses[3 * (size_t)V + ia], poses[4 * (size_t)V + ia]};
    const Pose2 b{poses[ib], poses[V + ib], poses[2 * (size_t)V + ib], poses[3 * (size_t)V + ib], poses[4 * (size_t)V + ib]};
    double e0, e1, e2;
    se2_error(a, b, cand[(size_t)F_TZX * cstride + c], cand[(size_t)F_TZY * cstride + c], cand[(size_t)F_CZ * cstride + c],
              cand[(size_t)F_SZ * cstride + c], cand[(size_t)F_THZ * cstride + c], e0, e1, e2);
    out[c] = gk_sym(cand, cstride, F_OM, c).quad(e0, e1, e2);
}
__global__ void k_cand_own_chi2_se3(const double* poses, int V, const double* cand, int cstride, const int* from, const int* to,
                                    int n, double* out)
{
    const int c = blockIdx.x * blockDim.x + threadIdx.x;
    if (c >= n) return;
    double Rz[9], tz[3], om[21];
    gk3_rz(cand, cstride, c, Rz, tz);
    Edge3 E;
    se3_edge(gk3_pose(poses, V, from[c]), gk3_pose(poses, V, to[c]), Rz, tz, E);
    gk3_sym(cand, cstride, G_OM, c, om);
    out[c] = sym6_quad(om, E.e);
}

__device__ __forceinline__ void se2_tail_D(double xT, double yT, double thT, const double* open, size_t Vs, int hi, double* D)
{
    const double thP = open[2 * Vs + hi];
    const double thD = normalize_theta(thT - thP);
    double sD, cD;
    sincos_pi(thD, sD, cD);
    const double xP = open[hi], yP = open[Vs + hi];
    const double xD = xT - (cD * xP - sD * yP), yD = yT - (sD * xP + cD * yP);
    D[0] = xD; D[1] = yD; D[2] = thD; D[3] = cD; D[4] = sD;
}
__device__ __forceinline__ void se2_tail_apply(const double* D, const double* open, size_t Vs, double* dst, int i)
{
    const double xD = D[0], yD = D[1], thD = D[2], cD = D[3], sD = D[4];
    const double x = open[i], y = open[Vs + i];
    const double th = normalize_theta(thD + open[2 * Vs + i]);
    double sn, cs;
    sincos_pi(th, sn, cs);
    dst[i] = xD + (cD * x - sD * y);
    dst[Vs + i] = yD + (sD * x + cD * y);
    dst[2 * Vs + i] = th;
    dst[3 * Vs + i] = cs;
    dst[4 * Vs + i] = sn;
}
__device__ __forceinline__ void se3_tail_D(const double* T, size_t ldt, const double* open, size_t Vs, int hi, double* D)
{
    double RT[9], tT[3], RP[9], tP[3], d[3];
    double* RD = D;
    for (int q = 0; q < 9; ++q) { RT[q] = T[(size_t)q * ldt]; RP[q] = open[(size_t)q * Vs + hi]; }
    for (int q = 0; q < 3; ++q) { tT[q] = T[(size_t)(9 + q) * ldt]; tP[q] = open[(size_t)(9 + q) * Vs + hi]; }
    for (int r = 0; r < 3; ++r)
        for (int c = 0; c < 3; ++c) RD[3 * r + c] = RT[3 * r] * RP[3 * c] + RT[3 * r + 1] * RP[3 * c + 1] + RT[3 * r + 2] * RP[3 * c + 2];
    m3_vec(RD, tP, d);
    for (int q = 0; q < 3; ++q) D[9 + q] = tT[q] - d[q];
}
__device__ __forceinline__ void se3_tail_apply(const double* D, const double* open, size_t Vs, double* dst, int i)
{
    const double* RD = D;
    const double* tD = D + 9;
    double Ri[9], ti[3], Rn[9], d[3];
    for (int q = 0; q < 9; ++q) Ri[q] = open[(size_t)q * Vs + i];
    for (int q = 0; q < 3; ++q) ti[q] = open[(size_t)(9 + q) * Vs + i];
    m3_mul(RD, Ri, Rn);
    m3_vec(RD, ti, d);
    for (int q = 0; q < 9; ++q) dst[(size_t)q * Vs + i] = Rn[q];
    for (int q = 0; q < 3; ++q) dst[(size_t)(9 + q) * Vs + i] = tD[q] + d[q];
}
template <int NF>
__global__ __launch_bounds__(256) void k_apply_accept(int V, int vs, int lo, int hi, const double* parent, const double* X, int ldx,
                                                      const double* open, double* dst)
{
    const int tid = threadIdx.x;
    for (int q = tid; q < NF * V; q += 256) {
        const int f = q / V, i = q - f * V;
        const size_t a = (size_t)f * vs + i;
        if (i >= lo && i <= hi) dst[a] = X[(size_t)f * ldx + (i - lo)];
        else if (i < lo && dst != parent) dst[a] = parent[a];
    }
    const size_t Vs = (size_t)vs;
    double D[12];
    if (NF == 5) se2_tail_D(X[hi - lo], X[(size_t)ldx + (hi - lo)], X[2 * (size_t)ldx + (hi - lo)], open, Vs, hi, D);
    else se3_tail_D(X + (hi - lo), (size_t)ldx, open, Vs, hi, D);
// ... 1339 lines not shown
```

ipc_amd/csrc/se2_group_kernel.hpp:

```cpp
#pragma once
#include "cell_kernels.hpp"
#include "se2_wave_cell.hpp"

namespace ipc {

constexpr int kWavesPerGroup = 4;
#ifndef IPC_LDS_BUDGET
#define IPC_LDS_BUDGET (160 * 1024)
#endif
constexpr int kLdsBudget = IPC_LDS_BUDGET;

#define IPC_GROUP_KERNEL_NAME se2_group_kernel
#define IPC_GROUP_KEEP_TRIAL false
#include "se2_group_kernel_def.hpp"
#undef IPC_GROUP_KERNEL_NAME
#undef IPC_GROUP_KEEP_TRIAL
#define IPC_GROUP_KERNEL_NAME se2_group_kernel_kt
#define IPC_GROUP_KEEP_TRIAL true
#include "se2_group_kernel_def.hpp"
#undef IPC_GROUP_KERNEL_NAME
#undef IPC_GROUP_KEEP_TRIAL

template <int W, int M, int NL, bool STAGED, bool KEEP_TRIAL>
constexpr auto se2_group_kernel_of()
{
    if constexpr (KEEP_TRIAL) return &se2_group_kernel_kt<W, M, NL, STAGED>;
    else return &se2_group_kernel<W, M, NL, STAGED>;
}

template <int W, int M, int NL, bool KEEP_TRIAL = false>
static hipError_t launch_group(int n, hipStream_t st, const Se2View& P, const int2* cells, SolveParams prm, CellOut out,
                              unsigned* counter, int n_cu)
{
    const int E = P.V - 1;
    const int wstride = E + 32;
    constexpr int kPairs = kWavesPerGroup / W;
    const size_t scratch = kPairs * (((sizeof(WaveScratch<NL>) + 7) / 8) + ((sizeof(PairBox) + 7) / 8)) * sizeof(double);
    const size_t staged = scratch + sizeof(double) * (size_t)F_SG * wstride;
    const int groups = std::max(1, std::min(n_cu, (n + kPairs - 1) / kPairs));
    if (staged <= (size_t)kLdsBudget) {
        auto k = se2_group_kernel_of<W, M, NL, true, KEEP_TRIAL>();
        hipError_t e = hipFuncSetAttribute(reinterpret_cast<const void*>(k), hipFuncAttributeMaxDynamicSharedMemorySize, (int)staged);
        if (e != hipSuccess) return e;
        hipLaunchKernelGGL(k, dim3(groups), dim3(64 * kWavesPerGroup), staged, st, P, cells, n, counter, prm, out, 0, E, wstride);
    } else {
        auto k = se2_group_kernel_of<W, M, NL, false, KEEP_TRIAL>();
        hipLaunchKernelGGL(k, dim3(groups), dim3(64 * kWavesPerGroup), scratch, st, P, cells, n, counter, prm, out, 0, E, wstride);
    }
    return hipGetLastError();
}

}
```

ipc_amd/csrc/se2_group_kernel_def.hpp:

```cpp
template <int W, int M, int NL, bool STAGED>
__global__ __launch_bounds__(64 * kWavesPerGroup, 1) void IPC_GROUP_KERNEL_NAME(Se2View P, const int2* cells, int ncells,
                                                                                unsigned* counter, SolveParams prm,
                                                                                CellOut out, int wlo, int wlen, int wstride)
{
    extern __shared__ double dyn_lds[];
    constexpr int kPairs = kWavesPerGroup / W;
    constexpr int kScratchDoubles = (sizeof(WaveScratch<NL>) + 7) / 8;
    constexpr int kBoxDoubles = (sizeof(PairBox) + 7) / 8;
    const int wave = threadIdx.x >> 6, lane = threadIdx.x & 63, pair = wave / W, wsub = wave & (W - 1);
    WaveScratch<NL>& sh = *reinterpret_cast<WaveScratch<NL>*>(dyn_lds + pair * kScratchDoubles);
    PairBox* box = reinterpret_cast<PairBox*>(dyn_lds + kPairs * kScratchDoubles + pair * kBoxDoubles);
    double* cst = dyn_lds + kPairs * (kScratchDoubles + kBoxDoubles);
    if (STAGED) {
        for (int f = 0; f < (int)F_SG; ++f)
            for (int i = threadIdx.x; i < wstride; i += 64 * kWavesPerGroup)
                cst[i * (int)F_SG + f] = i < wlen ? P.chain[(size_t)f * P.estride + wlo + i] : 0.0;
    }
    if (lane == 0) box->flag[wsub] = 0;
    __syncthreads();
    int seq = 0;
    for (;;) {
        ++seq;
        unsigned c = 0;
        if (wsub == 0 && lane == 0) {
            c = atomicAdd(counter, 1u);
            mb_store(&box->data[0][seq & 1][0], (double)c);
        }
        wave_sync();
        if (lane == 0) __hip_atomic_store(&box->flag[wsub], seq, __ATOMIC_RELEASE, __HIP_MEMORY_SCOPE_WORKGROUP);
#pragma unroll
        for (int o = 0; o < W; ++o) {
            if (o == wsub) continue;
            while (__hip_atomic_load(&box->flag[o], __ATOMIC_ACQUIRE, __HIP_MEMORY_SCOPE_WORKGROUP) - seq < 0)
                IPC_SPIN_WAIT();
        }
        wave_sync();
        c = (unsigned)mb_load(&box->data[0][seq & 1][0]);
        c = (unsigned)__builtin_amdgcn_readfirstlane((int)c);
        if (c >= (unsigned)ncells) break;
        const int2 cc = cells[c];
        int cand[2] = {cc.x, cc.y};
        int lo = min(P.cand_from[cc.x], P.cand_to[cc.x]), hi = max(P.cand_from[cc.x], P.cand_to[cc.x]);
        if (NL == 2) {
            lo = min(lo, min(P.cand_from[cc.y], P.cand_to[cc.y]));
            hi = max(hi, max(P.cand_from[cc.y], P.cand_to[cc.y]));
        }
        const int L = hi - lo;
        const int base = NL == 1 ? prm.fast_iter : prm.slow_iter;
        const int iterations = (L + NL > 100) ? base * 5 : base;
        CellResult r;
        se2_wave_solve<M, NL, STAGED, W, se2_err_store<M>(), IPC_GROUP_KEEP_TRIAL>(P, lo, L, cand, iterations, sh, cst, wlo,
                                                                                   wstride, r, box, seq, &seq);
        if (wsub == 0 && lane == 0) {
            out.max_chi2[c] = r.max_chi2;
            out.chi2_total[c] = r.chi2_total;
            out.meta[c] = make_int4(r.iterations, r.tries, r.flags, r.evals);
        }
        wave_sync();
    }
}
```

ipc_amd/csrc/se2_wave_cell.hpp:

```cpp
#pragma once
#include "se2_cell.hpp"

namespace ipc {

template <int NL>
struct WaveScratch {
    LoopConst lc[NL];
    LoopState ls[2][NL];
    double lvec[NL][2][3];
    double red[4][32];
};

struct PairBox {
    double data[4][2][8];
    int flag[4];
};
__device__ __forceinline__ void mb_store(double* p, double v)
{
#ifdef IPC_MAILBOX_PLAIN
    *p = v;
#else
    __hip_atomic_store(p, v, __ATOMIC_RELAXED, __HIP_MEMORY_SCOPE_WORKGROUP);
#endif
}
__device__ __forceinline__ double mb_load(const double* p)
{
#ifdef IPC_MAILBOX_PLAIN
    return *p;
#else
    return __hip_atomic_load(p, __ATOMIC_RELAXED, __HIP_MEMORY_SCOPE_WORKGROUP);
#endif
}

#ifndef IPC_SPIN_SLEEP
#define IPC_SPIN_SLEEP 1
#endif
#if IPC_SPIN_SLEEP > 0
#define IPC_SPIN_WAIT() __builtin_amdgcn_s_sleep(IPC_SPIN_SLEEP)
#else
#define IPC_SPIN_WAIT() asm volatile("s_nop 0")
#endif

__device__ __forceinline__ void wave_sync()
{
    __builtin_amdgcn_fence(__ATOMIC_ACQ_REL, "wavefront");
    __builtin_amdgcn_wave_barrier();
}

template <int N>
__device__ __forceinline__ bool ldl_solve(double (&A)[N][N], double (&b)[N])
{
    bool ok = true;
    double inv[N];
#pragma unroll
    for (int j = 0; j < N; ++j) {
        double d = A[j][j];
#pragma unroll
        for (int k = 0; k < j; ++k) d -= A[j][k] * A[j][k] * A[k][k];
        ok = ok && (d > 0);
        double r = __builtin_amdgcn_rcp(d);
        r = fma(fma(-d, r, 1.0), r, r);
        r = fma(fma(-d, r, 1.0), r, r);
        inv[j] = r;
        A[j][j] = d;
#pragma unroll
        for (int i = j + 1; i < N; ++i) {
            double v = A[i][j];
#pragma unroll
            for (int k = 0; k < j; ++k) v -= A[i][k] * A[j][k] * A[k][k];
            A[i][j] = v * r;
        }
    }
#pragma unroll
    for (int i = 0; i < N; ++i) {
        double v = b[i];
#pragma unroll
        for (int k = 0; k < i; ++k) v -= A[i][k] * b[k];
        b[i] = v;
    }
#pragma unroll
    for (int i = 0; i < N; ++i) b[i] *= inv[i];
#pragma unroll
    for (int i = N - 1; i >= 0; --i) {
        double v = b[i];
#pragma unroll
        for (int k = i + 1; k < N; ++k) v -= A[k][i] * b[k];
        b[i] = v;
    }
    return ok;
}

__device__ __forceinline__ double se2_gamma(double Aq, double Bq, double Kx, double Ky, double sigma, int i, int a)
{
    const double g02 = Aq * Kx + Bq * Ky, g12 = -Bq * Kx + Aq * Ky, nB = -Bq;
    const double g0 = a == 0 ? Aq : (a == 1 ? Bq : g02);
    const double g1 = a == 0 ? nB : (a == 1 ? Aq : g12);
    const double g2 = a == 2 ? 1.0 : 0.0;
    const double g = i == 0 ? g0 : (i == 1 ? g1 : g2);
    return sigma * g;
}

template <int V> struct IntC { static constexpr int value = V; };

#define IPC_SLOT_FENCE() __builtin_amdgcn_sched_barrier(0)
#define IPC_PIN1(a) asm volatile("" : "+v"(a) : : "memory")
#define IPC_PIN2(a, b) asm volatile("" : "+v"(a), "+v"(b) : : "memory")
#define IPC_PIN3(a, b, c) asm volatile("" : "+v"(a), "+v"(b), "+v"(c) : : "memory")

#ifndef IPC_KEEPE_MAX
#define IPC_KEEPE_MAX 8
#endif
#ifndef IPC_PF_MAX
#define IPC_PF_MAX 9
#endif
#ifndef IPC_PF_MAX_W1
#define IPC_PF_MAX_W1 (IPC_PF_MAX < 9 ? IPC_PF_MAX : 11)
#endif
#ifndef IPC_PARKE_SET
#define IPC_PARKE_SET ((1 << 9) | (1 << 11))
#endif
template <int M>
constexpr int se2_err_store() { return M <= IPC_KEEPE_MAX ? 1 : (((IPC_PARKE_SET >> M) & 1) ? 2 : 0); }

struct ParkedE { int w[6]; };
__device__ __forceinline__ void park_e(ParkedE& p, double e0, double e1, double e2)
{
    asm volatile("v_accvgpr_write_b32 %0, %6\n\tv_accvgpr_write_b32 %1, %7\n\tv_accvgpr_write_b32 %2, %8\n\t"
                 "v_accvgpr_write_b32 %3, %9\n\tv_accvgpr_write_b32 %4, %10\n\tv_accvgpr_write_b32 %5, %11"
                 : "=a"(p.w[0]), "=a"(p.w[1]), "=a"(p.w[2]), "=a"(p.w[3]), "=a"(p.w[4]), "=a"(p.w[5])
                 : "v"(__double2loint(e0)), "v"(__double2hiint(e0)), "v"(__double2loint(e1)), "v"(__double2hiint(e1)),
                   "v"(__double2loint(e2)), "v"(__double2hiint(e2)));
}
__device__ __forceinline__ void unpark_e(const ParkedE& p, double& e0, double& e1, double& e2)
{
    int l0, h0, l1, h1, l2, h2;
    asm volatile("v_accvgpr_read_b32 %0, %6\n\tv_accvgpr_read_b32 %1, %7\n\tv_accvgpr_read_b32 %2, %8\n\t"
                 "v_accvgpr_read_b32 %3, %9\n\tv_accvgpr_read_b32 %4, %10\n\tv_accvgpr_read_b32 %5, %11"
                 : "=v"(l0), "=v"(h0), "=v"(l1), "=v"(h1), "=v"(l2), "=v"(h2)
                 : "a"(p.w[0]), "a"(p.w[1]), "a"(p.w[2]), "a"(p.w[3]), "a"(p.w[4]), "a"(p.w[5]));
    e0 = __hiloint2double(h0, l0); e1 = __hiloint2double(h1, l1); e2 = __hiloint2double(h2, l2);
}

struct ParkedPose { int w[10]; };
__device__ __forceinline__ void park_pose(ParkedPose& p, const Pose2& Y)
{
    asm volatile("v_accvgpr_write_b32 %0, %10\n\tv_accvgpr_write_b32 %1, %11\n\tv_accvgpr_write_b32 %2, %12\n\t"
                 "v_accvgpr_write_b32 %3, %13\n\tv_accvgpr_write_b32 %4, %14\n\tv_accvgpr_write_b32 %5, %15\n\t"
                 "v_accvgpr_write_b32 %6, %16\n\tv_accvgpr_write_b32 %7, %17\n\tv_accvgpr_write_b32 %8, %18\n\t"
                 "v_accvgpr_write_b32 %9, %19"
                 : "=a"(p.w[0]), "=a"(p.w[1]), "=a"(p.w[2]), "=a"(p.w[3]), "=a"(p.w[4]), "=a"(p.w[5]), "=a"(p.w[6]),
                   "=a"(p.w[7]), "=a"(p.w[8]), "=a"(p.w[9])
                 : "v"(__double2loint(Y.x)), "v"(__double2hiint(Y.x)), "v"(__double2loint(Y.y)), "v"(__double2hiint(Y.y)),
                   "v"(__double2loint(Y.th)), "v"(__double2hiint(Y.th)), "v"(__double2loint(Y.c)), "v"(__double2hiint(Y.c)),
                   "v"(__double2loint(Y.s)), "v"(__double2hiint(Y.s)));
}
__device__ __forceinline__ void unpark_pose(const ParkedPose& p, Pose2& Y)
{
    int l0, h0, l1, h1, l2, h2, l3, h3, l4, h4;
    asm volatile("v_accvgpr_read_b32 %0, %10\n\tv_accvgpr_read_b32 %1, %11\n\tv_accvgpr_read_b32 %2, %12\n\t"
                 "v_accvgpr_read_b32 %3, %13\n\tv_accvgpr_read_b32 %4, %14\n\tv_accvgpr_read_b32 %5, %15\n\t"
                 "v_accvgpr_read_b32 %6, %16\n\tv_accvgpr_read_b32 %7, %17\n\tv_accvgpr_read_b32 %8, %18\n\t"
                 "v_accvgpr_read_b32 %9, %19"
                 : "=v"(l0), "=v"(h0), "=v"(l1), "=v"(h1), "=v"(l2), "=v"(h2), "=v"(l3), "=v"(h3), "=v"(l4), "=v"(h4)
                 : "a"(p.w[0]), "a"(p.w[1]), "a"(p.w[2]), "a"(p.w[3]), "a"(p.w[4]), "a"(p.w[5]), "a"(p.w[6]), "a"(p.w[7]),
                   "a"(p.w[8]), "a"(p.w[9]));
    Y.x = __hiloint2double(h0, l0); Y.y = __hiloint2double(h1, l1); Y.th = __hiloint2double(h2, l2);
    Y.c = __hiloint2double(h3, l3); Y.s = __hiloint2double(h4, l4);
}

template <int M, int NL, bool STAGED, int W = 1, int E_STORE = se2_err_store<M>(), bool KEEP_TRIAL = false>
__device__ __forceinline__ void se2_wave_solve(const Se2View& P, int lo_abs, int L, const int (&cand)[2], int iterations,
                               WaveScratch<NL>& sh, const double* cst, int wlo, int wstride, CellResult& res,
                               PairBox* box = nullptr, int seq0 = 0, int* seq_out = nullptr)
{
    static_assert(W == 1 || W == 2 || W == 4, "one, two or four cooperating waves per cell");
    constexpr bool KEEP_E = E_STORE == 1, PARK_E = E_STORE == 2;
    constexpr int NS = NL * 3;
    const double term_scale = P.term_eps / (double)(L + NL);
    bool lastGN = false;
    const int lane = threadIdx.x & 63;
    const int wsub = W > 1 ? (__builtin_amdgcn_readfirstlane((int)(threadIdx.x >> 6)) & (W - 1)) : 0;
    const int gl = wsub * 64 + lane;
    int j0 = gl * M + 1;

#ifdef IPC_PHASE_TIMING
    unsigned long long gnEvals = 0, gnRejected = 0, nBig = 0, tmBig = 0, tmSmall = 0;
    unsigned long long tmA = 0, tmB1 = 0, tmB2 = 0, tmC = 0, tmT = 0, tmW = 0, tmK = 0, tm0 = __builtin_amdgcn_s_memtime();
#define IPC_WTICK(acc) { const unsigned long long t_ = __builtin_amdgcn_s_memtime(); acc += t_ - tm0; tm0 = t_; }
#else
#define IPC_WTICK(acc)
#endif
    int seq = seq0;
    auto post_wait = [&](const double (&mine)[8], int n) {
        if constexpr (W > 1) {
            ++seq;
            double* my = box->data[wsub][seq & 1];
            if (lane == 0) {
#pragma unroll
                for (int k = 0; k < 8; ++k) if (k < n) mb_store(&my[k], mine[k]);
            }
            wave_sync();
            if (lane == 0) __hip_atomic_store(&box->flag[wsub], seq, __ATOMIC_RELEASE, __HIP_MEMORY_SCOPE_WORKGROUP);
#ifdef IPC_PHASE_TIMING
            const unsigned long long tw0 = __builtin_amdgcn_s_memtime();
#endif
#pragma unroll
            for (int o = 0; o < W; ++o) {
                if (o == wsub) continue;
                while (__hip_atomic_load(&box->flag[o], __ATOMIC_ACQUIRE, __HIP_MEMORY_SCOPE_WORKGROUP) - seq < 0)
                    IPC_SPIN_WAIT();
            }
#ifdef IPC_PHASE_TIMING
            tmW += __builtin_amdgcn_s_memtime() - tw0;
#endif
#ifdef IPC_MB_DELAY_WAVE
            if (wsub == IPC_MB_DELAY_WAVE) { __builtin_amdgcn_s_sleep(127); __builtin_amdgcn_s_sleep(127); }
#endif
            __builtin_amdgcn_fence(__ATOMIC_ACQUIRE, "workgroup", "local");
            wave_sync();
        }
    };
    auto peer = [&](int o, int k) -> double { return mb_load(&box->data[o][seq & 1][k]); };
    auto pair_barrier = [&]() {
        if constexpr (W > 1) { double a[8] = {0, 0, 0, 0, 0, 0, 0, 0}; post_wait(a, 0); }
    };
    auto cell_sum2 = [&](double v0, double v1, double& s0, double& s1) {
        const double t0 = wave_sum(v0), t1 = wave_sum(v1);
        if constexpr (W > 1) {
            double a[8] = {t0, t1, 0, 0, 0, 0, 0, 0};
            post_wait(a, 2);
#if defined(IPC_MAILBOX_PLAIN) && defined(IPC_DBG_SUM_SIDE)
            auto rdx = [&](int o, int k) -> double {
                return ((IPC_DBG_SUM_SIDE >> o) & 1) ? __hip_atomic_load(&box->data[o][seq & 1][k], __ATOMIC_RELAXED, __HIP_MEMORY_SCOPE_WORKGROUP) : peer(o, k);
            };
#else
            auto rdx = [&](int o, int k) -> double { return peer(o, k); };
#endif
            s0 = wsub == 0 ? t0 : rdx(0, 0);
            s1 = wsub == 0 ? t1 : rdx(0, 1);
#pragma unroll
            for (int o = 1; o < W; ++o) { s0 += o == wsub ? t0 : rdx(o, 0); s1 += o == wsub ? t1 : rdx(o, 1); }
        } else { s0 = t0; s1 = t1; }
    };
    auto cell_excl = [&](double run) -> double {
        const double inc = wave_inclusive_scan(run);
        double off = inc - run;
        if constexpr (W > 1) {
            double a[8] = {read_lane(inc, 63), 0, 0, 0, 0, 0, 0, 0};
            post_wait(a, 1);
            double lower = 0.0;
#pragma unroll
            for (int o = 0; o < W - 1; ++o) if (o < wsub) lower += peer(o, 0);
            off += lower;
        }
        return off;
    };
    auto cell_excl2 = [&](double r0, double r1, double& o0, double& o1) {
        const double i0 = wave_inclusive_scan(r0), i1 = wave_inclusive_scan(r1);
        o0 = i0 - r0; o1 = i1 - r1;
        if constexpr (W > 1) {
            double a[8] = {read_lane(i0, 63), read_lane(i1, 63), 0, 0, 0, 0, 0, 0};
            post_wait(a, 2);
            double l0 = 0.0, l1 = 0.0;
#pragma unroll
            for (int o = 0; o < W - 1; ++o) if (o < wsub) { l0 += peer(o, 0); l1 += peer(o, 1); }
            o0 += l0; o1 += l1;
        }
    };

    if (lane < NL && wsub == 0) {
        const int l = lane, c = cand[l];
        LoopConst& q = sh.lc[l];
        q.f = P.cand_from[c] - lo_abs;
        q.t = P.cand_to[c] - lo_abs;
        q.lo = min(q.f, q.t);
        q.hi = max(q.f, q.t);
        q.sigma = q.t > q.f ? 1.0 : -1.0;
        q.tzx = P.cand[(size_t)F_TZX * P.cstride + c];
        q.tzy = P.cand[(size_t)F_TZY * P.cstride + c];
        q.cz = P.cand[(size_t)F_CZ * P.cstride + c];
        q.sz = P.cand[(size_t)F_SZ * P.cstride + c];
        q.thz = P.cand[(size_t)F_THZ * P.cstride + c];
#pragma unroll
        for (int k = 0; k < 6; ++k) {
            q.om[k] = P.cand[(size_t)(F_OM + k) * P.cstride + c];
            q.sg[k] = P.cand[(size_t)(F_SG + k) * P.cstride + c];
        }
    }

    Pose2 X[M];
    double ex[KEEP_E ? M : 1], ey[KEEP_E ? M : 1], eth[KEEP_E ? M : 1];
    ParkedE pe[PARK_E ? M : 1];
    ParkedPose tY[KEEP_TRIAL ? M : 1];
    ParkedE tE[(KEEP_TRIAL && KEEP_E) ? M : 1];
    double bx[M], by[M], bth[M];
    double hx[M], hy[M], hth[M];
    Pose2 gauge;
    gauge.x = P.pose0[lo_abs];
    gauge.y = P.pose0[(size_t)P.VS + lo_abs];
    gauge.th = P.pose0[(size_t)2 * P.VS + lo_abs];
    sincos_pi(gauge.th, gauge.s, gauge.c);
#pragma unroll
    for (int s = 0; s < M; ++s) {
        const int j = j0 + s;
        const int ja = j <= L ? lo_abs + j : lo_abs;
        X[s].x = P.pose0[ja];
        X[s].y = P.pose0[(size_t)P.VS + ja];
        X[s].th = P.pose0[(size_t)2 * P.VS + ja];
        sincos_pi(X[s].th, X[s].s, X[s].c);
        if (KEEP_E) ex[s] = ey[s] = eth[s] = 0.0;
        bx[s] = by[s] = bth[s] = 0.0;
        hx[s] = hy[s] = hth[s] = 0.0;
    }
    wave_sync();
    pair_barrier();
    int lf[NL], lt[NL], of[NL], sf[NL], ot[NL], st_[NL], llo[NL], lhi[NL];
#pragma unroll
    for (int l = 0; l < NL; ++l) {
        lf[l] = __builtin_amdgcn_readfirstlane(sh.lc[l].f);
        lt[l] = __builtin_amdgcn_readfirstlane(sh.lc[l].t);
        llo[l] = min(lf[l], lt[l]); lhi[l] = max(lf[l], lt[l]);
        of[l] = lf[l] > 0 ? (lf[l] - 1) / M : -1; sf[l] = lf[l] > 0 ? (lf[l] - 1) % M : -1;
        ot[l] = lt[l] > 0 ? (lt[l] - 1) / M : -1; st_[l] = lt[l] > 0 ? (lt[l] - 1) % M : -1;
    }
    unsigned ownSlots = 0;
#pragma unroll
    for (int l = 0; l < NL; ++l) {
        if (of[l] >= 0 && (of[l] >> 6) == wsub) ownSlots |= 1u << sf[l];
        if (ot[l] >= 0 && (ot[l] >> 6) == wsub) ownSlots |= 1u << st_[l];
    }
    if (gl == 0) {
#pragma unroll
        for (int l = 0; l < NL; ++l)
#pragma unroll
            for (int bsel = 0; bsel < 2; ++bsel) {
                double* pf = sh.ls[bsel][l].pf;
                double* pt = sh.ls[bsel][l].pt;
                if (lf[l] == 0) { pf[0] = gauge.x; pf[1] = gauge.y; pf[2] = gauge.th; pf[3] = gauge.c; pf[4] = gauge.s; }
                if (lt[l] == 0) { pt[0] = gauge.x; pt[1] = gauge.y; pt[2] = gauge.th; pt[3] = gauge.c; pt[4] = gauge.s; }
            }
    }

    int eloc = gl * M < L ? gl * M : 0;
    typedef const __attribute__((address_space(3))) double* LdsRec;
    LdsRec crec = nullptr;
    auto opaque = [&]() {
        asm volatile("" : "+v"(eloc), "+v"(j0));
        if (STAGED) { crec = (LdsRec)(cst + (lo_abs - wlo + eloc) * (int)F_SG); asm volatile("" : "+v"(crec)); }
    };
    auto ldc = [&](int field, int s) -> double {
        if (STAGED && field < (int)F_SG) return crec[s * (int)F_SG + field];
        return P.chain_rec[((size_t)(lo_abs + eloc) + s) * (int)F_NFIELDS + field];
    };
    auto ldsym = [&](int field0, int s) -> Sym3 {
        Sym3 m;
        m.a00 = ldc(field0 + 0, s); m.a01 = ldc(field0 + 1, s); m.a02 = ldc(field0 + 2, s);
        m.a11 = ldc(field0 + 3, s); m.a12 = ldc(field0 + 4, s); m.a22 = ldc(field0 + 5, s);
        return m;
    };
    struct SlotConst { double tzx, tzy, thz, cz, sz; Sym3 om, sg; };
    auto ld_slot = [&](int s, SlotConst& c, auto want_c) {
        constexpr int WANT = decltype(want_c)::value;
        if (WANT & 1) { c.tzx = ldc(F_TZX, s); c.tzy = ldc(F_TZY, s); c.thz = ldc(F_THZ, s); }
        if (WANT & 2) { c.cz = ldc(F_CZ, s); c.sz = ldc(F_SZ, s); }
        if (WANT & 4) c.om = ldsym(F_OM, s);
        if (WANT & 8) c.sg = ldsym(F_SG, s);
    };
    constexpr int kErrWant = KEEP_E ? 0 : 3;
    constexpr int kErrWantBC = (KEEP_E || PARK_E) ? 0 : 3;
    constexpr bool PF = M <= (W == 1 ? IPC_PF_MAX_W1 : IPC_PF_MAX);

    auto prev0 = [&](const Pose2& last) -> Pose2 {
        Pose2 cr = gauge;
        if constexpr (W > 1) {
            double a[8] = {read_lane(last.x, 63), read_lane(last.y, 63), read_lane(last.th, 63), read_lane(last.c, 63),
                           read_lane(last.s, 63), 0, 0, 0};
            post_wait(a, 5);
            if (wsub > 0) { cr.x = peer(wsub - 1, 0); cr.y = peer(wsub - 1, 1); cr.th = peer(wsub - 1, 2); cr.c = peer(wsub - 1, 3); cr.s = peer(wsub - 1, 4); }
        }
        Pose2 p;
        p.x = lane_prev(last.x, cr.x); p.y = lane_prev(last.y, cr.y); p.th = lane_prev(last.th, cr.th);
        p.c = lane_prev(last.c, cr.c); p.s = lane_prev(last.s, cr.s);
        return p;
    };
    auto prev3 = [&](double vx, double vy, double vth, double& ox, double& oy, double& oth) {
        double c0 = 0.0, c1 = 0.0, c2 = 0.0;
        if constexpr (W > 1) {
            double a[8] = {read_lane(vx, 63), read_lane(vy, 63), read_lane(vth, 63), 0, 0, 0, 0, 0};
            post_wait(a, 3);
            if (wsub > 0) { c0 = peer(wsub - 1, 0); c1 = peer(wsub - 1, 1); c2 = peer(wsub - 1, 2); }
        }
        ox = lane_prev(vx, c0); oy = lane_prev(vy, c1); oth = lane_prev(vth, c2);
    };
    auto next3 = [&](double vx, double vy, double vth, double& ox, double& oy, double& oth) {
        double c0 = 0.0, c1 = 0.0, c2 = 0.0;
        if constexpr (W > 1) {
            double a[8] = {read_lane(vx, 0), read_lane(vy, 0), read_lane(vth, 0), 0, 0, 0, 0, 0};
            post_wait(a, 3);
            if (wsub < W - 1) { c0 = peer(wsub + 1, 0); c1 = peer(wsub + 1, 1); c2 = peer(wsub + 1, 2); }
        }
        ox = lane_next(vx, c0); oy = lane_next(vy, c1); oth = lane_next(vth, c2);
    };

    auto loop_eval = [&](int l, int bsel) -> double {
        const LoopConst& q = sh.lc[l];
        LoopState& st = sh.ls[bsel][l];
        Pose2 a{st.pf[0], st.pf[1], st.pf[2], st.pf[3], st.pf[4]};
        Pose2 b{st.pt[0], st.pt[1], st.pt[2], st.pt[3], st.pt[4]};
        double e0, e1, e2;
        se2_error(a, b, q.tzx, q.tzy, q.cz, q.sz, q.thz, e0, e1, e2);
        Sym3 om{q.om[0], q.om[1], q.om[2], q.om[3], q.om[4], q.om[5]};
        double q0, q1, q2;
        om.mul(e0, e1, e2, q0, q1, q2);
        const double chi = e0 * q0 + e1 * q1 + e2 * q2;
        st.e[0] = e0; st.e[1] = e1; st.e[2] = e2;
        st.chi = chi;
        return chi;
    };
    int cur = 0;
    auto loop_force = [&](int l) {
        const LoopConst& q = sh.lc[l];
        LoopState& st = sh.ls[cur][l];
        Sym3 om{q.om[0], q.om[1], q.om[2], q.om[3], q.om[4], q.om[5]};
        double q0, q1, q2;
        om.mul(st.e[0], st.e[1], st.e[2], q0, q1, q2);
        const double cP = st.pf[3] * q.cz - st.pf[4] * q.sz, sP = st.pf[4] * q.cz + st.pf[3] * q.sz;
        st.g[0] = cP * q0 - sP * q1; st.g[1] = sP * q0 + cP * q1; st.g[2] = q2;
    };

    bool sweepChanged = false;
    auto launder = [&]() {
#pragma unroll
        for (int s = 0; s < M; ++s) {
            asm volatile("" : "+v"(X[s].x), "+v"(X[s].y), "+v"(X[s].c), "+v"(X[s].s));
            if (KEEP_E) asm volatile("" : "+v"(ex[s]), "+v"(ey[s]), "+v"(eth[s]));
        }
    };
    auto err_of = [&](int s, const Pose2& a, const SlotConst& K, double& e0, double& e1, double& e2) {
        if (KEEP_E) { e0 = ex[s]; e1 = ey[s]; e2 = eth[s]; return; }
        se2_error(a, X[s], K.tzx, K.tzy, K.cz, K.sz, K.thz, e0, e1, e2);
        if (!(j0 + s <= L)) { e0 = 0.0; e1 = 0.0; e2 = 0.0; }
    };
    auto err_again = [&](int s, const Pose2& a, const SlotConst& K, double& e0, double& e1, double& e2) {
        if (PARK_E) unpark_e(pe[s], e0, e1, e2);
        else err_of(s, a, K, e0, e1, e2);
    };
    auto sweep = [&](auto mode_c, bool big, double p, double q, int bsel, bool gn = false, bool wantChanged = true) -> double {
        constexpr int MODE = decltype(mode_c)::value;
        opaque();
        launder();
        asm volatile("" : "+v"(p), "+v"(q));
        auto stepped = [&](int s) -> Pose2 {
            Pose2 Y;
            double dx, dy, dth;
            if (gn) { dx = hx[s]; dy = hy[s]; dth = hth[s]; }
            else { dx = fma(p, bx[s], q * hx[s]); dy = fma(p, by[s], q * hy[s]); dth = fma(p, bth[s], q * hth[s]); }
            Y.x = X[s].x + dx;
            Y.y = X[s].y + dy;
            Y.th = wrap_pi(X[s].th + dth);
            if (big) sincos_pi(Y.th, Y.s, Y.c);
            else rotate_small(X[s].c, X[s].s, Y.th - X[s].th, Y.c, Y.s);
            return Y;
        };
        const Pose2 last = MODE == 0 ? X[M - 1] : stepped(M - 1);
        Pose2 prev = last;
        if (MODE != 2 || KEEP_E) prev = prev0(last);
        double part = 0.0;
        bool changed = false;
        constexpr int kWant = (MODE != 2 || KEEP_E) ? (MODE != 2 ? 7 : 3) : 0;
        SlotConst Kn;
        if (PF) ld_slot(0, Kn, IntC<kWant>{});
#pragma unroll
        for (int s = 0; s < M; ++s) {
            SlotConst K;
            if (PF) { K = Kn; if (s + 1 < M) ld_slot(s + 1, Kn, IntC<kWant>{}); }
            else ld_slot(s, K, IntC<kWant>{});
            const Pose2 Y = MODE == 0 ? X[s] : (s == M - 1 ? last : stepped(s));
            const bool v = j0 + s <= L;
            if (MODE == 1 && wantChanged) changed |= v && ((Y.x != X[s].x) || (Y.y != X[s].y) || (Y.th != X[s].th));
            double e0 = 0.0, e1 = 0.0, e2 = 0.0;
            if (MODE != 2 || KEEP_E) se2_error(prev, Y, K.tzx, K.tzy, K.cz, K.sz, K.thz, e0, e1, e2);
            if (MODE != 2) {
                const double c2 = K.om.quad(e0, e1, e2);
                part += v ? c2 : 0.0;
            }
            if (MODE != 1 && KEEP_E) { ex[s] = v ? e0 : 0.0; ey[s] = v ? e1 : 0.0; eth[s] = v ? e2 : 0.0; }
            if constexpr (MODE == 1 && KEEP_TRIAL) {
                park_pose(tY[s], Y);
                if constexpr (KEEP_E) park_e(tE[s], v ? e0 : 0.0, v ? e1 : 0.0, v ? e2 : 0.0);
            }
            if (MODE != 2 && ((ownSlots >> s) & 1u)) {
#pragma unroll
                for (int l = 0; l < NL; ++l) {
                    if (sf[l] == s && gl == of[l]) {
                        double* w = sh.ls[bsel][l].pf;
                        w[0] = Y.x; w[1] = Y.y; w[2] = Y.th; w[3] = Y.c; w[4] = Y.s;
                    }
                    if (st_[l] == s && gl == ot[l]) {
                        double* w = sh.ls[bsel][l].pt;
                        w[0] = Y.x; w[1] = Y.y; w[2] = Y.th; w[3] = Y.c; w[4] = Y.s;
                    }
                }
            }
            if (MODE == 2) X[s] = Y;
            prev = Y;
            if (MODE != 2) IPC_PIN1(part);
            if (MODE != 1 && KEEP_E) IPC_PIN3(ex[s], ey[s], eth[s]);
            if (MODE == 2) IPC_PIN3(X[s].x, X[s].y, X[s].th);
            IPC_PIN3(prev.x, prev.y, prev.th);
            IPC_PIN2(prev.c, prev.s);
            IPC_SLOT_FENCE();
        }
        if (MODE == 2) return 0.0;
        wave_sync();
        if constexpr (W > 1) {
            double tot, chg;
            cell_sum2(part, (MODE == 1 && changed) ? 1.0 : 0.0, tot, chg);
            const double lc = lane < NL ? loop_eval(lane, bsel) : 0.0;
#pragma unroll
            for (int l = 0; l < NL; ++l) tot += read_lane(lc, l);
            if (MODE == 1) sweepChanged = chg != 0.0;
            return tot;
        } else {
            if (lane < NL) part += loop_eval(lane, bsel);
            double tot, chg;
            cell_sum2(part, (MODE == 1 && changed) ? 1.0 : 0.0, tot, chg);
            if (MODE == 1) sweepChanged = chg != 0.0;
            return tot;
        }
    };

    int evals = 1;
    double currentChi = sweep(IntC<0>{}, false, 0.0, 0.0, cur);

    double delta = 1e4;
    const int maxTrials = 100;
    int it_done = 0, tries_total = 0, flags = 0;

    IPC_WTICK(tmT)
    for (int it = 0; it < iterations; ++it) {
        opaque();
        launder();
        if (gl < NL) loop_force(gl);
        wave_sync();
        const Pose2 a0 = prev0(X[M - 1]);
        constexpr int kWantA = 2 | 4 | kErrWant;
        auto force = [&](int s, const Pose2& a, const SlotConst& K, double& gx, double& gy, double& gth, double& mx,
                         double& my, double& mth) {
            const double cz = K.cz, sz = K.sz;
            const double cP = a.c * cz - a.s * sz, sP = a.s * cz + a.c * sz;
            double e0, e1, e2, qx, qy, qth;
            err_of(s, a, K, e0, e1, e2);
            if (PARK_E) park_e(pe[s], e0, e1, e2);
            K.om.mul(e0, e1, e2, qx, qy, qth);
            gx = cP * qx - sP * qy;
            gy = sP * qx + cP * qy;
            gth = qth;
            const double dx = X[s].x - a.x, dy = X[s].y - a.y;
            mx = gx; my = gy;
            mth = gth + (-dy * gx + dx * gy);
        };
        double bbp = 0.0;
        {
            double g0x, g0y, g0th, m0x, m0y, m0th;
            SlotConst Kn;
            {
                SlotConst K0;
                ld_slot(0, K0, IntC<kWantA>{});
                if (PF && M > 1) ld_slot(M - 1, Kn, IntC<kWantA>{});
                force(0, a0, K0, g0x, g0y, g0th, m0x, m0y, m0th);
            }
            double nx, ny, nth;
            next3(m0x, m0y, m0th, nx, ny, nth);
#pragma unroll
            for (int s = M - 1; s >= 0; --s) {
                double gx, gy, gth, mx, my, mth;
                if (s == 0) { gx = g0x; gy = g0y; gth = g0th; mx = m0x; my = m0y; mth = m0th; }
                else {
                    SlotConst K;
                    if (PF) { K = Kn; if (s - 1 > 0) ld_slot(s - 1, Kn, IntC<kWantA>{}); }
                    else ld_slot(s, K, IntC<kWantA>{});
                    force(s, X[s - 1], K, gx, gy, gth, mx, my, mth);
                }
                const bool v = j0 + s <= L;
                double tx = nx - gx, ty = ny - gy, tth = nth - gth;
                if ((ownSlots >> s) & 1u) {
#pragma unroll
                for (int l = 0; l < NL; ++l) {
                    const LoopState& st = sh.ls[cur][l];
                    if (st_[l] == s && gl == ot[l]) { tx -= st.g[0]; ty -= st.g[1]; tth -= st.g[2]; }
                    if (sf[l] == s && gl == of[l]) {
                        const double dx = st.pt[0] - st.pf[0], dy = st.pt[1] - st.pf[1];
                        tx += st.g[0]; ty += st.g[1];
                        tth += st.g[2] + (-dy * st.g[0] + dx * st.g[1]);
                    }
                }
                }
                bx[s] = v ? tx : 0.0; by[s] = v ? ty : 0.0; bth[s] = v ? tth : 0.0;
                bbp += bx[s] * bx[s] + by[s] * by[s] + bth[s] * bth[s];
                nx = mx; ny = my; nth = mth;
                IPC_PIN3(bx[s], by[s], bth[s]);
                IPC_PIN3(nx, ny, nth);
                IPC_PIN1(bbp);
                IPC_SLOT_FENCE();
            }
        }
        IPC_WTICK(tmA)
        double bb, bHb, alpha, hsdNorm;
        double nu[NL][3];
        opaque();
        launder();
        {
#pragma unroll
            for (int l = 0; l < NL; ++l) {
                if (gl == 0) {
                    if (lf[l] == 0) { sh.lvec[l][0][0] = 0.0; sh.lvec[l][0][1] = 0.0; sh.lvec[l][0][2] = 0.0; }
                    if (lt[l] == 0) { sh.lvec[l][1][0] = 0.0; sh.lvec[l][1][1] = 0.0; sh.lvec[l][1][2] = 0.0; }
                }
#pragma unroll
                for (int s = 0; s < M; ++s) {
                    if (!((ownSlots >> s) & 1u)) continue;
                    if (sf[l] == s && gl == of[l]) { sh.lvec[l][0][0] = bx[s]; sh.lvec[l][0][1] = by[s]; sh.lvec[l][0][2] = bth[s]; }
                    if (st_[l] == s && gl == ot[l]) { sh.lvec[l][1][0] = bx[s]; sh.lvec[l][1][1] = by[s]; sh.lvec[l][1][2] = bth[s]; }
                }
            }
            double v1[16], v2[16];
#pragma unroll
            for (int k = 0; k < 16; ++k) { v1[k] = 0.0; v2[k] = 0.0; }
            v1[0] = bbp;
            double qbx, qby, qbth;
            prev3(bx[M - 1], by[M - 1], bth[M - 1], qbx, qby, qbth);
            constexpr int kWantB = 2 | 4 | 8 | kErrWantBC;
            SlotConst Kn;
            if (PF) ld_slot(0, Kn, IntC<kWantB>{});
#pragma unroll
            for (int s = 0; s < M; ++s) {
                SlotConst K;
                if (PF) { K = Kn; if (s + 1 < M) ld_slot(s + 1, Kn, IntC<kWantB>{}); }
                else ld_slot(s, K, IntC<kWantB>{});
                const Pose2& a = s == 0 ? a0 : X[s - 1];
                const bool v = j0 + s <= L;
                const double cz = K.cz, sz = K.sz;
                double wx, wy, wth;
                se2_apply_J(a, X[s], cz, sz, qbx, qby, qbth, bx[s], by[s], bth[s], wx, wy, wth);
                const double hq = K.om.quad(wx, wy, wth);
                v1[1] += v ? hq : 0.0;
                const Sym3 sg = K.sg;
                const double c = a.c * cz - a.s * sz, sn = a.s * cz + a.c * sz;
                const double kx = -(X[s].y - gauge.y), ky = X[s].x - gauge.x;
                const double cc = c * c, ss = sn * sn, cs = c * sn;
                const double C00 = cc * sg.a00 - 2 * cs * sg.a01 + ss * sg.a11;
                const double C01 = cs * (sg.a00 - sg.a11) + (cc - ss) * sg.a01;
                const double C11 = ss * sg.a00 + 2 * cs * sg.a01 + cc * sg.a11;
                const double c0 = c * sg.a02 - sn * sg.a12, c1 = sn * sg.a02 + c * sg.a12;
                const double sth = sg.a22;
                double psi[6];
                psi[2] = c0 - sth * kx;
                psi[4] = c1 - sth * ky;
                psi[0] = C00 - kx * c0 - kx * psi[2];
                psi[1] = C01 - kx * c1 - ky * psi[2];
                psi[3] = C11 - ky * c1 - ky * psi[4];
                psi[5] = sth;
                double e0, e1, e2;
                err_again(s, a, K, e0, e1, e2);
                const double w0 = c * e0 - sn * e1 - kx * e2;
                const double w1 = sn * e0 + c * e1 - ky * e2;
                const double w2 = e2;
                const int j = j0 + s;
                const double m1 = (v && j > llo[0] && j <= lhi[0]) ? 1.0 : 0.0;
                v1[2] += m1 * w0; v1[3] += m1 * w1; v1[4] += m1 * w2;
#pragma unroll
                for (int k = 0; k < 6; ++k) v1[5 + k] += m1 * psi[k];
                if constexpr (NL == 2) {
                    const double m2 = (v && j > llo[1] && j <= lhi[1]) ? 1.0 : 0.0;
                    const double m12 = m1 * m2;
                    v2[0] += m2 * w0; v2[1] += m2 * w1; v2[2] += m2 * w2;
#pragma unroll
                    for (int k = 0; k < 6; ++k) { v2[3 + k] += m2 * psi[k]; v2[9 + k] += m12 * psi[k]; }
                }
                qbx = bx[s]; qby = by[s]; qbth = bth[s];
                asm volatile("" : "+v"(v1[0]), "+v"(v1[1]), "+v"(v1[2]), "+v"(v1[3]), "+v"(v1[4]), "+v"(v1[5]),
                             "+v"(v1[6]), "+v"(v1[7]), "+v"(v1[8]), "+v"(v1[9]), "+v"(v1[10]) : : "memory");
                if constexpr (NL == 2)
                    asm volatile("" : "+v"(v2[0]), "+v"(v2[1]), "+v"(v2[2]), "+v"(v2[3]), "+v"(v2[4]), "+v"(v2[5]),
                                 "+v"(v2[6]), "+v"(v2[7]), "+v"(v2[8]), "+v"(v2[9]), "+v"(v2[10]), "+v"(v2[11]),
                                 "+v"(v2[12]), "+v"(v2[13]), "+v"(v2[14]) : : "memory");
                IPC_SLOT_FENCE();
            }
            wave_sum16_store(v1, &sh.red[wsub][0]);
            if constexpr (NL == 2) wave_sum16_store(v2, &sh.red[wsub][16]);
            wave_sync();
            pair_barrier();
            IPC_WTICK(tmB1)
            constexpr int RS = NS + 1;
            int bl = lane;
            asm volatile("" : "+v"(bl));
            const int r = bl / RS, c = bl % RS;
            const bool inS = bl < NS * RS;
            const int l1 = (NL > 1 && inS) ? r / 3 : 0, i = r % 3;
            const int l2 = (NL > 1 && c < NS) ? c / 3 : 0, k3 = c % 3;
            const int lq_l = bl < NL ? bl : 0;
            const int g_l = (NL > 1 && bl < NL * 9) ? bl / 9 : 0, g_i = (bl % 9) / 3, g_a = bl % 3;
            const LoopConst& qg = sh.lc[g_l];
            const LoopState& sg_ = sh.ls[cur][g_l];
            const double gcz = qg.cz, gsz = qg.sz, gsig = qg.sigma;
            const double gpc = sg_.pf[3], gps = sg_.pf[4], gtx = sg_.pt[0], gty = sg_.pt[1];
            const double s1e = sh.ls[cur][l1].e[i];
            const int mb = l1 == l2 ? (l1 == 0 ? 5 : 19) : 25, wb = l1 == 0 ? 2 : 16;
            double mred[W][6], wred[W][3], bred[W][2];
#pragma unroll
            for (int o = 0; o < W; ++o) {
#pragma unroll
                for (int k = 0; k < 6; ++k) mred[o][k] = sh.red[o][mb + k];
#pragma unroll
                for (int k = 0; k < 3; ++k) wred[o][k] = sh.red[o][wb + k];
                bred[o][0] = sh.red[o][0]; bred[o][1] = sh.red[o][1];
            }
            const int lo_ = i < k3 ? i : k3, hi_ = i < k3 ? k3 : i;
            const double sgv = sh.lc[l1].sg[lo_ * 3 - lo_ * (lo_ - 1) / 2 + (hi_ - lo_)];
            const LoopConst& qq = sh.lc[lq_l];
            const LoopState& sq = sh.ls[cur][lq_l];
            const Pose2 qa{sq.pf[0], sq.pf[1], sq.pf[2], sq.pf[3], sq.pf[4]};
            const Pose2 qb{sq.pt[0], sq.pt[1], sq.pt[2], sq.pt[3], sq.pt[4]};
            const double qcz = qq.cz, qsz = qq.sz;
            const Sym3 qom{qq.om[0], qq.om[1], qq.om[2], qq.om[3], qq.om[4], qq.om[5]};
            double qv[2][3];
#pragma unroll
            for (int e = 0; e < 2; ++e)
#pragma unroll
                for (int k = 0; k < 3; ++k) qv[e][k] = sh.lvec[lq_l][e][k];
            __builtin_amdgcn_sched_barrier(0);
            double g1[3], g2[3], gam;
            {
                const double Aq = gpc * gcz - gps * gsz, Bq = gps * gcz + gpc * gsz;
                const double Kx = -(gty - gauge.y), Ky = gtx - gauge.x;
                gam = se2_gamma(Aq, Bq, Kx, Ky, gsig, g_i, g_a);
#pragma unroll
                for (int a = 0; a < 3; ++a) {
                    g1[a] = __shfl(gam, l1 * 9 + i * 3 + a, 64);
                    g2[a] = __shfl(gam, l2 * 9 + k3 * 3 + a, 64);
                }
            }
            __builtin_amdgcn_sched_barrier(0);
            double m[6], w[3];
#pragma unroll
            for (int k = 0; k < 6; ++k) {
                m[k] = mred[0][k];
#pragma unroll
                for (int o = 1; o < W; ++o) m[k] += mred[o][k];
            }
#pragma unroll
            for (int k = 0; k < 3; ++k) {
                w[k] = wred[0][k];
#pragma unroll
                for (int o = 1; o < W; ++o) w[k] += wred[o][k];
            }
            bb = bred[0][0];
            bHb = bred[0][1];
#pragma unroll
            for (int o = 1; o < W; ++o) { bb += bred[o][0]; bHb += bred[o][1]; }
            {
                double wx, wy, wth;
                se2_apply_J(qa, qb, qcz, qsz, qv[0][0], qv[0][1], qv[0][2], qv[1][0], qv[1][1], qv[1][2], wx, wy, wth);
                const double lq = bl < NL ? qom.quad(wx, wy, wth) : 0.0;
#pragma unroll
                for (int l = 0; l < NL; ++l) bHb += read_lane(lq, l);
            }
            IPC_PIN2(bb, bHb);
            __builtin_amdgcn_sched_barrier(0);
            double val;
            {
                const double g10 = g1[0], g11 = g1[1], g12 = g1[2];
                const double m00 = m[0], m01 = m[1], m02 = m[2], m11 = m[3], m12 = m[4], m22 = m[5];
                const double t0 = g10 * m00 + g11 * m01 + g12 * m02;
                const double t1 = g10 * m01 + g11 * m11 + g12 * m12;
                const double t2 = g10 * m02 + g11 * m12 + g12 * m22;
                double vS = t0 * g2[0] + t1 * g2[1] + t2 * g2[2];
                const double vSd = vS + sgv;
                vS = l1 == l2 ? vSd : vS;
                const double vR = s1e - (g10 * w[0] + g11 * w[1] + g12 * w[2]);
                val = c < NS ? vS : vR;
                val = inS ? val : 0.0;
            }
            bool okS = true;
            alpha = 0.0; hsdNorm = 0.0;
#pragma unroll
            for (int k = 0; k < NS; ++k) {
                const double rowk = __shfl(val, k * RS + c, 64);
                const double colk = __shfl(val, r * RS + k, 64);
                __builtin_amdgcn_sched_barrier(0);
                const double piv = read_lane(val, k * RS + k);
                okS = okS && (piv > 0);
                double inv = __builtin_amdgcn_rcp(piv);
                inv = fma(fma(-piv, inv, 1.0), inv, inv);
                inv = fma(fma(-piv, inv, 1.0), inv, inv);
                if (k == 0) {
                    alpha = bb / bHb;
                    IPC_PIN1(alpha);
                } else if (k == 1) {
                    hsdNorm = sqrt(alpha * alpha * bb);
                    IPC_PIN1(hsdNorm);
                }
                __builtin_amdgcn_sched_barrier(0);
                val = (r == k) ? rowk * inv : fma(-(colk * rowk), inv, val);
            }
            {
                double mu[3], gn[3];
#pragma unroll
                for (int rr = 0; rr < 3; ++rr) {
                    mu[rr] = __shfl(val, (3 * l1 + rr) * RS + NS, 64);
                    gn[rr] = __shfl(gam, l1 * 9 + rr * 3 + k3, 64);
                }
                double nv = 0.0;
#pragma unroll
                for (int rr = 0; rr < 3; ++rr) nv += gn[rr] * mu[rr];
#pragma unroll
                for (int l = 0; l < NL; ++l)
#pragma unroll
                    for (int k = 0; k < 3; ++k) nu[l][k] = read_lane(nv, 3 * l * RS + k);
            }
            if (!okS) { flags |= 2; break; }
        }
        IPC_WTICK(tmB2)
        double hgnNorm, bh, hHh;
        opaque();
        launder();
        {
            double run = 0.0;
            constexpr int kWantC = 2 | 8 | kErrWantBC;
            SlotConst Kn;
            if (PF) ld_slot(0, Kn, IntC<kWantC>{});
#pragma unroll
            for (int s = 0; s < M; ++s) {
                SlotConst K;
                if (PF) { K = Kn; if (s + 1 < M) ld_slot(s + 1, Kn, IntC<kWantC>{}); }
                else ld_slot(s, K, IntC<kWantC>{});
                const Pose2& a = s == 0 ? a0 : X[s - 1];
                const int j = j0 + s;
                const bool v = j <= L;
                const double m1 = (v && j > llo[0] && j <= lhi[0]) ? 1.0 : 0.0;
                double n0 = m1 * nu[0][0], n1 = m1 * nu[0][1], n2 = m1 * nu[0][2];
                if constexpr (NL == 2) {
                    const double m2 = (v && j > llo[1] && j <= lhi[1]) ? 1.0 : 0.0;
                    n0 += m2 * nu[1][0]; n1 += m2 * nu[1][1]; n2 += m2 * nu[1][2];
                }
                const double cz = K.cz, sz = K.sz;
                const double c = a.c * cz - a.s * sz, sn = a.s * cz + a.c * sz;
                const double kx = -(X[s].y - gauge.y), ky = X[s].x - gauge.x;
                const double wx = c * n0 + sn * n1, wy = -sn * n0 + c * n1, wth = -(kx * n0 + ky * n1) + n2;
                double vx, vy, vth;
                K.sg.mul(wx, wy, wth, vx, vy, vth);
                double e0, e1, e2;
                err_again(s, a, K, e0, e1, e2);
                const double ux = -vx - e0, uy = -vy - e1, uth = -vth - e2;
                hx[s] = v ? c * ux - sn * uy : 0.0;
                hy[s] = v ? sn * ux + c * uy : 0.0;
                run += v ? uth : 0.0;
                hth[s] = run;
                IPC_PIN3(hx[s], hy[s], hth[s]);
                IPC_SLOT_FENCE();
            }
            const double offT = cell_excl(run);
            double rx = 0.0, ry = 0.0, thPrev = offT;
#pragma unroll
            for (int s = 0; s < M; ++s) {
                const Pose2& a = s == 0 ? a0 : X[s - 1];
                const bool v = j0 + s <= L;
                hth[s] += offT;
                const double dx = X[s].x - a.x, dy = X[s].y - a.y;
                rx += v ? hx[s] - dy * thPrev : 0.0;
                ry += v ? hy[s] + dx * thPrev : 0.0;
                hx[s] = rx; hy[s] = ry;
                thPrev = hth[s];
                IPC_PIN3(hx[s], hy[s], hth[s]);
                IPC_SLOT_FENCE();
            }
            double offX, offY;
            cell_excl2(rx, ry, offX, offY);
            double p0 = 0.0, p1 = 0.0;
#pragma unroll
            for (int s = 0; s < M; ++s) {
                const bool v = j0 + s <= L;
                hx[s] = v ? hx[s] + offX : 0.0;
                hy[s] = v ? hy[s] + offY : 0.0;
                hth[s] = v ? hth[s] : 0.0;
                p0 += hx[s] * hx[s] + hy[s] * hy[s] + hth[s] * hth[s];
                p1 += bx[s] * hx[s] + by[s] * hy[s] + bth[s] * hth[s];
            }
            double hh;
            cell_sum2(p0, p1, hh, bh);
            hgnNorm = sqrt(hh);
            hHh = bh;
        }
        IPC_WTICK(tmC)
        if (lastGN && hgnNorm < delta && fabs(bh) < term_scale * currentChi) { it_done = it + 1; tries_total += maxTrials; flags |= 1; break; }
        const double deltaAtEntry = delta;
        bool goodStep = false, dlReady = false;
        double dlC = 0.0, dlBma = 0.0;
        int numTries = 0;
        do {
            ++numTries;
            int stepType;
            double beta = 0.0, sdScale = 0.0;
            if (hgnNorm < delta) stepType = 0;
            else if (hsdNorm > delta) { stepType = 1; sdScale = delta / hsdNorm; }
            else {
                stepType = 2;
                if (!dlReady) {
                    double p0 = 0.0, p1 = 0.0;
#pragma unroll
                    for (int s = 0; s < M; ++s) {
                        const double sx = alpha * bx[s], sy = alpha * by[s], sth = alpha * bth[s];
                        const double ax = hx[s] - sx, ay = hy[s] - sy, ath = hth[s] - sth;
                        p0 += sx * ax + sy * ay + sth * ath;
                        p1 += ax * ax + ay * ay + ath * ath;
                    }
                    cell_sum2(p0, p1, dlC, dlBma);
                    dlReady = true;
                }
                const double c = dlC, bma = dlBma;
                const double hsdSq = alpha * alpha * bb;
                if (c <= 0.) beta = (-c + sqrt(c * c + bma * (delta * delta - hsdSq))) / bma;
                else beta = (delta * delta - hsdSq) / (c + sqrt(c * c + bma * (delta * delta - hsdSq)));
            }
            double pcoef, qcoef, hdlNorm;
            if (stepType == 0) { pcoef = 0.0; qcoef = 1.0; hdlNorm = hgnNorm; }
            else if (stepType == 1) { pcoef = sdScale * alpha; qcoef = 0.0; hdlNorm = delta; }
            else { pcoef = alpha - beta * alpha; qcoef = beta; hdlNorm = delta; }
            const double hdlHhdl = pcoef * pcoef * bHb + 2 * pcoef * qcoef * bb + qcoef * qcoef * hHh;
            const double bhdl = pcoef * bb + qcoef * bh;
            double linearGain = -1 * hdlHhdl + 2 * bhdl;
            bool big = false;
            double pc2 = pcoef, qc2 = qcoef;
            asm volatile("" : "+v"(pc2), "+v"(qc2));
#pragma unroll
            for (int s = 0; s < M; ++s) {
                const double thn = wrap_pi(X[s].th + (stepType == 0 ? hth[s] : fma(pc2, bth[s], qc2 * hth[s])));
                big |= fabs(thn - X[s].th) >= 0.015625;
            }
            const bool anyBig = __ballot(big) != 0ull;
            const int trial = cur ^ 1;
#ifdef IPC_PHASE_TIMING
            const unsigned long long tb0 = __builtin_amdgcn_s_memtime();
#endif
            const double newChi = sweep(IntC<1>{}, anyBig, pcoef, qcoef, trial, stepType == 0, stepType == 1);
#ifdef IPC_PHASE_TIMING
            if (anyBig) { ++nBig; tmBig += __builtin_amdgcn_s_memtime() - tb0; } else { tmSmall += __builtin_amdgcn_s_memtime() - tb0; }
#endif
            const bool anyChanged = stepType == 1 ? sweepChanged : true;
            ++evals;
            const double nonLinearGain = currentChi - newChi;
#ifdef IPC_PHASE_TIMING
            if (stepType == 0) { ++gnEvals; if (!(linearGain > 0 ? nonLinearGain > 0 : nonLinearGain < 0)) ++gnRejected; }
#endif
            if (fabs(linearGain) < 1e-12) linearGain = 1e-12;
            const bool linPos = linearGain > 0;
            auto rho_gt = [&](double t) { return linPos ? nonLinearGain > t * linearGain : nonLinearGain < t * linearGain; };
            auto rho_lt = [&](double t) { return linPos ? nonLinearGain < t * linearGain : nonLinearGain > t * linearGain; };
            if (rho_gt(0.0)) {
                goodStep = true;
                currentChi = newChi;
                cur = trial;
                IPC_WTICK(tmT)
                if constexpr (KEEP_TRIAL) {
#pragma unroll
                    for (int s = 0; s < M; ++s) {
                        unpark_pose(tY[s], X[s]);
                        if constexpr (W > 1) IPC_PIN3(X[s].x, X[s].y, X[s].th);
                        if constexpr (KEEP_E) unpark_e(tE[s], ex[s], ey[s], eth[s]);
                    }
                } else {
                    sweep(IntC<2>{}, anyBig, pcoef, qcoef, trial, stepType == 0, false);
                }
                IPC_WTICK(tmK)
            }
            if (rho_gt(0.75)) delta = fmax(delta, 3 * hdlNorm);
            else if (rho_lt(0.25)) delta *= 0.5;
            if (!goodStep) {
                if (nonLinearGain != nonLinearGain) {
                    numTries = maxTrials;
                } else if (stepType == 0) {
                    while (numTries < maxTrials && hgnNorm < delta) { ++numTries; delta *= 0.5; }
                } else if (stepType == 1 && !anyChanged) {
                    numTries = maxTrials;
                }
            }
        } while (!goodStep && numTries < maxTrials);
        lastGN = goodStep && numTries == 1 && hgnNorm < deltaAtEntry;
        it_done = it + 1;
        tries_total += numTries;
        IPC_WTICK(tmT)
        if (numTries == maxTrials || !goodStep) { flags |= 1; break; }
    }
#ifdef IPC_PHASE_TIMING
    if (lane == 0 && wsub == 0 && P.dbg) {
        unsigned long long* d = reinterpret_cast<unsigned long long*>(P.dbg) + 64 + 16 * (M + 16 * (W - 1));
        atomicAdd(d + 0, tmA); atomicAdd(d + 1, tmB1); atomicAdd(d + 2, tmB2); atomicAdd(d + 3, tmC);
        atomicAdd(d + 4, tmT); atomicAdd(d + 5, tmW);
        atomicAdd(d + 6, (unsigned long long)it_done); atomicAdd(d + 7, (unsigned long long)evals);
        atomicAdd(d + 8, (unsigned long long)it_done * (unsigned long long)L);
        atomicAdd(d + 9, 1ull); atomicAdd(d + 10, tmK); atomicAdd(d + 11, (unsigned long long)(evals - 1 - it_done)); atomicAdd(d + 12, gnEvals); atomicAdd(d + 13, gnRejected); atomicAdd(d + 14, nBig); atomicAdd(d + 15, tmBig); atomicAdd(d + 1024, tmSmall);
    }
#endif

    double mx = 0.0;
    bool nan = false;
    opaque();
    {
        const Pose2 a0 = prev0(X[M - 1]);
#pragma unroll
        for (int s = 0; s < M; ++s) {
            SlotConst K;
            ld_slot(s, K, IntC<(4 | kErrWant)>{});
            double e0, e1, e2;
            err_of(s, s == 0 ? a0 : X[s - 1], K, e0, e1, e2);
            if (j0 + s > L) continue;
            const double c = K.om.quad(e0, e1, e2);
            if (c != c) nan = true;
            else mx = fmax(mx, c);
        }
    }
    mx = wave_max(mx);
    nan = __ballot(nan) != 0ull;
    if constexpr (W > 1) {
        double a[8] = {mx, nan ? 1.0 : 0.0, 0, 0, 0, 0, 0, 0};
        post_wait(a, 2);
#pragma unroll
        for (int o = 0; o < W; ++o) {
            if (o == wsub) continue;
            mx = fmax(mx, peer(o, 0));
            nan = nan || peer(o, 1) != 0.0;
        }
    }
    wave_sync();
#pragma unroll
    for (int l = 0; l < NL; ++l) {
        const double c = sh.ls[cur][l].chi;
        if (c != c) nan = true;
        else mx = fmax(mx, c);
    }
    if (nan && !(mx > 0.0)) mx = __longlong_as_double(0x7ff8000000000000ll);
    res.max_chi2 = mx;
    res.chi2_total = currentChi;
    res.iterations = it_done;
    res.tries = tries_total;
    res.flags = flags;
    res.evals = evals;
    if (seq_out) *seq_out = seq;
}

}
```

ipc_amd/csrc/se2_wave_kernel.hpp:

```cpp
#pragma once
#include "cell_kernels.hpp"
#include "se2_wave_cell.hpp"

using namespace ipc;

#ifndef IPC_SE2_DENSE_MAXM
#define IPC_SE2_DENSE_MAXM 1
#endif
template <int M>
constexpr int se2_waves() { return M <= IPC_SE2_DENSE_MAXM ? 8 : 4; }

#define IPC_WAVE_KERNEL_NAME se2_wave_kernel
#define IPC_WAVE_KEEP_TRIAL false
#include "se2_wave_kernel_def.hpp"
#undef IPC_WAVE_KERNEL_NAME
#undef IPC_WAVE_KEEP_TRIAL
#define IPC_WAVE_KERNEL_NAME se2_wave_kernel_kt
#define IPC_WAVE_KEEP_TRIAL true
#include "se2_wave_kernel_def.hpp"
#undef IPC_WAVE_KERNEL_NAME
#undef IPC_WAVE_KEEP_TRIAL

template <int M, int NL, bool STAGED, bool KEEP_TRIAL>
constexpr auto se2_wave_kernel_of()
{
    if constexpr (KEEP_TRIAL) return &se2_wave_kernel_kt<M, NL, STAGED>;
    else return &se2_wave_kernel<M, NL, STAGED>;
}

#ifndef IPC_LDS_BUDGET
#define IPC_LDS_BUDGET (160 * 1024)
#endif
constexpr int kLdsBudget = IPC_LDS_BUDGET;

template <int M, int NL, bool KEEP_TRIAL>
static hipError_t launch_wave_one(int n, hipStream_t st, const Se2View& P, const int2* cells, SolveParams prm, CellOut out,
                                  unsigned* counter, int n_cu)
{
    constexpr int kWavesPerGroup = se2_waves<M>();
    const int E = P.V - 1;
    const int wstride = E + 32;
    const size_t scratch = kWavesPerGroup * ((sizeof(WaveScratch<NL>) + 7) / 8) * sizeof(double);
    const size_t staged = scratch + sizeof(double) * (size_t)F_SG * wstride;
    const int groups = std::max(1, std::min(n_cu, (n + kWavesPerGroup - 1) / kWavesPerGroup));
    if (staged <= (size_t)kLdsBudget) {
        auto k = se2_wave_kernel_of<M, NL, true, KEEP_TRIAL>();
        hipError_t e = hipFuncSetAttribute(reinterpret_cast<const void*>(k), hipFuncAttributeMaxDynamicSharedMemorySize, (int)staged);
        if (e != hipSuccess) return e;
        hipLaunchKernelGGL(k, dim3(groups), dim3(64 * kWavesPerGroup), staged, st, P, cells, n, counter, prm, out, 0, E, wstride);
    } else {
        auto k = se2_wave_kernel_of<M, NL, false, KEEP_TRIAL>();
        hipLaunchKernelGGL(k, dim3(groups), dim3(64 * kWavesPerGroup), scratch, st, P, cells, n, counter, prm, out, 0, E, wstride);
    }
    return hipGetLastError();
}
```

ipc_amd/csrc/se2_wave_kernel_def.hpp:

```cpp
template <int M, int NL, bool STAGED>
__global__ __launch_bounds__((64 * se2_waves<M>()), 1) void IPC_WAVE_KERNEL_NAME(Se2View P, const int2* cells, int ncells,
                                                                               unsigned* counter, SolveParams prm,
                                                                               CellOut out, int wlo, int wlen, int wstride)
{
    extern __shared__ double dyn_lds[];
    constexpr int kWavesPerGroup = se2_waves<M>();
    constexpr int kScratchDoubles = (sizeof(WaveScratch<NL>) + 7) / 8;
    const int wave = threadIdx.x >> 6, lane = threadIdx.x & 63;
    WaveScratch<NL>& sh = *reinterpret_cast<WaveScratch<NL>*>(dyn_lds + wave * kScratchDoubles);
    double* cst = dyn_lds + kWavesPerGroup * kScratchDoubles;
    if (STAGED) {
        for (int f = 0; f < (int)F_SG; ++f)
            for (int i = threadIdx.x; i < wstride; i += 64 * kWavesPerGroup)
                cst[i * (int)F_SG + f] = i < wlen ? P.chain[(size_t)f * P.estride + wlo + i] : 0.0;
    }
    __syncthreads();
    for (;;) {
        unsigned c = 0;
        if (lane == 0) c = atomicAdd(counter, 1u);
        c = (unsigned)__builtin_amdgcn_readfirstlane((int)c);
        if (c >= (unsigned)ncells) break;
        const int2 cc = cells[c];
        int cand[2] = {cc.x, cc.y};
        int lo = min(P.cand_from[cc.x], P.cand_to[cc.x]), hi = max(P.cand_from[cc.x], P.cand_to[cc.x]);
        if (NL == 2) {
            lo = min(lo, min(P.cand_from[cc.y], P.cand_to[cc.y]));
            hi = max(hi, max(P.cand_from[cc.y], P.cand_to[cc.y]));
        }
        const int L = hi - lo;
        const int base = NL == 1 ? prm.fast_iter : prm.slow_iter;
        const int iterations = (L + NL > 100) ? base * 5 : base;
        CellResult r;
        se2_wave_solve<M, NL, STAGED, 1, se2_err_store<M>(), IPC_WAVE_KEEP_TRIAL>(P, lo, L, cand, iterations, sh, cst, wlo,
                                                                                  wstride, r);
        if (lane == 0) {
            out.max_chi2[c] = r.max_chi2;
            out.chi2_total[c] = r.chi2_total;
            out.meta[c] = make_int4(r.iterations, r.tries, r.flags, r.evals);
        }
        wave_sync();
    }
}
```

Measured before the change: 2.062 million candidate-pairs/s.

## Compute steepest-descent terms lazily only when the dogleg step needs them

Adds lazy-SD variants of the SE2 wave and pair solver kernels. In these variants the steepest-descent quantities (the bHb quadratic form, alpha and the SD norm) are computed only when some lane in the wave needs a non-Gauss-Newton step or bb is very large, instead of on every iteration. It is on by default for selected bins (wave M=5,7,11 and pair M=11) and can be changed with IPC_SE2_LAZY_SD. The aim is to skip the per-iteration J·b pass and reduction when the Gauss-Newton step fits inside the trust region, at the cost of more kernel variants, more code size and possible extra register pressure.

```diff
diff --git a/__graft_entry__.py b/__graft_entry__.py
--- a/__graft_entry__.py
+++ b/__graft_entry__.py
@@ -17,7 +17,8 @@
     return all(os.path.getmtime(s) <= t for s in sources)
 
 
-UNITS = ["engine.hip", "se2_block.hip", "se2_wave.hip", "se2_wave_kt.hip", "se2_pair.hip", "se2_pair_kt.hip", "se2_quad.hip",
+UNITS = ["engine.hip", "se2_block.hip", "se2_wave.hip", "se2_wave_kt.hip", "se2_wave_lz.hip", "se2_pair.hip", "se2_pair_kt.hip",
+         "se2_pair_lz.hip", "se2_quad.hip",
          "se3_block.hip",
          "se3_lds_a.hip", "se3_lds_b.hip", "se3_lds_c.hip", "se3_lds_d.hip", "se3_lds_e.hip"]
 
@@ -32,7 +33,7 @@
     os.makedirs(objdir, exist_ok=True)
     flags = HIP_FLAGS + list(extra_flags)
     hdrs = [os.path.join(CSRC, f) for f in os.listdir(CSRC) if f.endswith((".hpp", ".h"))]
-    hdrs += [os.path.join(ROOT, "include", f) for f in ("ipc_amd.h", "ipc_amd_online_exact.h")]
+    hdrs += [os.path.join(ROOT, "include", f) for f in ("ipc_amd.h", "ipc_amd_online_exact.h", "ipc_amd_lazy_sd.h")]
 
     def compile_unit(u):
         src, obj = os.path.join(CSRC, u), os.path.join(objdir, u.replace(".hip", ".o"))
@@ -47,7 +48,7 @@
 
 def build(force=False):
     srcs = [os.path.join(CSRC, f) for f in sorted(os.listdir(CSRC)) if f.endswith((".hip", ".hpp", ".h"))]
-    srcs += [os.path.join(ROOT, "include", f) for f in ("ipc_amd.h", "ipc_amd_online_exact.h")]
+    srcs += [os.path.join(ROOT, "include", f) for f in ("ipc_amd.h", "ipc_amd_online_exact.h", "ipc_amd_lazy_sd.h")]
     if force or not _newer(LIB, srcs):
         _build_lib(LIB)
     host = os.path.join(ROOT, "ipc_amd", "host")
diff --git a/include/ipc_amd.h b/include/ipc_amd.h
--- a/include/ipc_amd.h
+++ b/include/ipc_amd.h
@@ -143,6 +143,7 @@
 int ipc_run_exact(ipc_engine_t* h, uint64_t* bits_out, uint8_t* accepted_out, uint8_t* multistart_out, ipc_exact_report_t* report);
 
 #include "ipc_amd_online_exact.h"
+#include "ipc_amd_lazy_sd.h"
 
 int ipc_cell_count(ipc_engine_t* h, int* n_cells);
 int ipc_cell_info(ipc_engine_t* h, ipc_cell_info_t* out, int capacity);
diff --git a/include/ipc_amd_lazy_sd.h b/include/ipc_amd_lazy_sd.h
--- /dev/null
+++ b/include/ipc_amd_lazy_sd.h
@@ -0,0 +1,9 @@
+#ifndef IPC_AMD_LAZY_SD_H
+#define IPC_AMD_LAZY_SD_H
+#ifndef IPC_AMD_H
+#error "include ipc_amd.h, which includes this header"
+#endif
+
+int ipc_se2_lazy_sd_launches(ipc_engine_t* h, long long* launches);
+
+#endif
diff --git a/ipc_amd/capi.py b/ipc_amd/capi.py
--- a/ipc_amd/capi.py
+++ b/ipc_amd/capi.py
@@ -27,6 +27,7 @@
     "ipc_set_max_exact", "ipc_run_exact",
 ]
 SYMBOLS_ONLINE_EXACT = ["ipc_set_max_exact_resume", "ipc_run_online_exact", "ipc_online_exact_state"]
+SYMBOLS_LAZY_SD = ["ipc_se2_lazy_sd_launches"]
 
 
 class Params(C.Structure):
@@ -149,6 +150,8 @@
     lib.ipc_solve_report.argtypes = [vp, C.POINTER(SolveReport)]
     lib.ipc_solver_time_ms.argtypes = [vp, C.POINTER(dp), C.POINTER(ip)]
     lib.ipc_synchronize.argtypes = [vp]
+    if hasattr(lib, "ipc_se2_lazy_sd_launches"):
+        lib.ipc_se2_lazy_sd_launches.argtypes = [vp, C.POINTER(C.c_longlong)]
     lib.ipc_incremental_reset.argtypes = [vp]
     lib.ipc_incremental_prepare.argtypes = [vp]
     lib.ipc_agreement_check.argtypes = [vp, ip, C.POINTER(ip), C.POINTER(CheckInfo)]
diff --git a/ipc_amd/consensus.py b/ipc_amd/consensus.py
--- a/ipc_amd/consensus.py
+++ b/ipc_amd/consensus.py
@@ -293,6 +293,11 @@
         capi.check(self.lib.ipc_solve_report(self.h, C.byref(r)))
         return {k: getattr(r, k) for k, _ in capi.SolveReport._fields_}
 
+    def lazy_sd_launches(self):
+        n = C.c_longlong(0)
+        capi.check(self.lib.ipc_se2_lazy_sd_launches(self.h, C.byref(n)))
+        return n.value
+
     def solver_time_ms(self):
         ms, nl = C.c_double(0), C.c_int(0)
         capi.check(self.lib.ipc_solver_time_ms(self.h, C.byref(ms), C.byref(nl)))
diff --git a/ipc_amd/csrc/cell_kernels.hpp b/ipc_amd/csrc/cell_kernels.hpp
--- a/ipc_amd/csrc/cell_kernels.hpp
+++ b/ipc_amd/csrc/cell_kernels.hpp
@@ -75,4 +75,14 @@
 hipError_t launch_se2_pair_kt(int nl, int M, int n, hipStream_t st, const Se2View& P, const int2* cells,
                               SolveParams prm, CellOut out, unsigned* counter, int n_cu);
 
+constexpr int kLazyKeepTrialMaxM = 9;
+static const int kWaveLzM[] = {5, 7, 9, 11, 13};
+constexpr int kNumWaveLzM = sizeof(kWaveLzM) / sizeof(kWaveLzM[0]);
+hipError_t launch_se2_wave_lz(int nl, int M, int n, hipStream_t st, const Se2View& P, const int2* cells,
+                              SolveParams prm, CellOut out, unsigned* counter, int n_cu);
+static const int kPairLzM[] = {7, 9, 11};
+constexpr int kNumPairLzM = sizeof(kPairLzM) / sizeof(kPairLzM[0]);
+hipError_t launch_se2_pair_lz(int nl, int M, int n, hipStream_t st, const Se2View& P, const int2* cells,
+                              SolveParams prm, CellOut out, unsigned* counter, int n_cu);
+
 }
diff --git a/ipc_amd/csrc/engine.hip b/ipc_amd/csrc/engine.hip
--- a/ipc_amd/csrc/engine.hip
+++ b/ipc_amd/csrc/engine.hip
@@ -1,6 +1,7 @@
 #include <hip/hip_runtime.h>
 
 #include <algorithm>
+#include <atomic>
 #include <cstdarg>
 #include <cstdlib>
 #include <utility>
@@ -510,8 +511,29 @@
     int variant[kMaxBins];
     int latency_variant[kMaxBins];
     int latency_below[kMaxBins];
+    bool lazy_sd[kMaxBins];
 };
 static const char* kDefaultPolicy = "w1,w3,kw5,kw7,kw9,w11,w13,kp7,kp9,p11,q7,q9,q11,q13,16x4,16x8,16x16";
+static const int kLazySdWaveM[] = {5, 7, 11};
+static const int kLazySdPairM[] = {11};
+static bool lazy_sd_serves(int variant, bool every)
+{
+    bool wave = false, pair = false;
+    int m = 0;
+    if (variant >= kPairKtVariantBase) { pair = true; m = variant - kPairKtVariantBase; if (m > kLazyKeepTrialMaxM) return false; }
+    else if (variant >= kWaveKtVariantBase) { wave = true; m = variant - kWaveKtVariantBase; if (m > kLazyKeepTrialMaxM) return false; }
+    else if (variant >= kQuadVariantBase) return false;
+    else if (variant >= kPairVariantBase) { pair = true; m = variant - kPairVariantBase; if (m <= kLazyKeepTrialMaxM) return false; }
+    else if (variant >= kWaveVariantBase) { wave = true; m = variant - kWaveVariantBase; if (m <= kLazyKeepTrialMaxM) return false; }
+    if (every) {
+        if (wave) for (int k : kWaveLzM) if (k == m) return true;
+        if (pair) for (int k : kPairLzM) if (k == m) return true;
+        return false;
+    }
+    if (wave) for (int k : kLazySdWaveM) if (k == m) return true;
+    if (pair) for (int k : kLazySdPairM) if (k == m) return true;
+    return false;
+}
 static const int kDefaultSideStreams2 = 7, kDefaultSideStreams3 = 7;
 static const char* kDefaultPolicy3 = "w1,w2,w3,w4,w6,w8,g3,g4,g5,g6,g7,g8,g9,g10,16x4";
 static const char* kBlockPolicy3 = "1x1,1x2,1x3,2x2,2x3,4x2,4x4,8x4,8x5,16x4";
@@ -566,6 +588,13 @@
         bp.variant[b] = b < bp.caps.n ? items[b].second : -1;
         bp.latency_variant[b] = -1;
         bp.latency_below[b] = 0;
+        bp.lazy_sd[b] = false;
+    }
+    if (dim == 2) {
+        const char* lz = getenv("IPC_SE2_LAZY_SD");
+        if (lz && *lz && strcmp(lz, "0") != 0 && strcmp(lz, "1") != 0 && strcmp(lz, "2") != 0) { err = "IPC_SE2_LAZY_SD: 0, 1 or 2"; return false; }
+        const bool lazy_on = !(lz && *lz == '0'), every = lz && *lz == '2';
+        for (int b = 0; b < bp.caps.n; ++b) bp.lazy_sd[b] = lazy_on && lazy_sd_serves(bp.variant[b], every);
     }
     if (dim == 3) {
         const char* lenv = getenv("IPC_SE3_LATENCY_POLICY");
@@ -658,6 +687,7 @@
     DevBuf<unsigned> d_slot_off;
     DevBuf<int> d_recount; PinnedBuf<int> h_recount;
     int last_cells = 0, last_long_cells = 0;
+    mutable std::atomic<long long> lazy_sd_launches{0};
     Event ev0, ev1; bool ev_valid = false; int last_launches = 0;
     static constexpr int kMaxSide = 7;
     int n_side = 0;
@@ -1653,6 +1683,13 @@
     {
         int var = h->plan.variant[b];
         if (h->plan.latency_variant[b] >= 0 && n < h->plan.latency_below[b] * h->n_cu) var = h->plan.latency_variant[b];
+        if (h->dim == 2 && var == h->plan.variant[b] && h->plan.lazy_sd[b]) {
+            h->lazy_sd_launches.fetch_add(1, std::memory_order_relaxed);
+            const bool pair = var >= kPairKtVariantBase || (var < kWaveKtVariantBase && var >= kPairVariantBase);
+            const int m = var % 100;
+            return pair ? launch_se2_pair_lz(nl, m, n, ls, P, cells, sp, out, ctr, h->n_cu)
+                        : launch_se2_wave_lz(nl, m, n, ls, P, cells, sp, out, ctr, h->n_cu);
+        }
         if (h->dim == 2)
             return var >= kPairKtVariantBase ? launch_se2_pair_kt(nl, var - kPairKtVariantBase, n, ls, P, cells, sp, out, ctr, h->n_cu)
                    : var >= kWaveKtVariantBase ? launch_se2_wave_kt(nl, var - kWaveKtVariantBase, n, ls, P, cells, sp, out, ctr, h->n_cu)
@@ -2725,6 +2762,13 @@
     HIPCHK(hipEventElapsedTime(&t, h->ev0, h->ev1));
     *ms = t;
     if (launches) *launches = h->last_launches;
+    return IPC_OK;
+}
+
+extern "C" int ipc_se2_lazy_sd_launches(ipc_engine_t* h, long long* launches)
+{
+    if (!h || !launches) return fail(IPC_ERR_ARG, "ipc_se2_lazy_sd_launches: NULL argument");
+    *launches = h->lazy_sd_launches.load(std::memory_order_relaxed);
     return IPC_OK;
 }
 
diff --git a/ipc_amd/csrc/se2_group_kernel.hpp b/ipc_amd/csrc/se2_group_kernel.hpp
--- a/ipc_amd/csrc/se2_group_kernel.hpp
+++ b/ipc_amd/csrc/se2_group_kernel.hpp
@@ -12,6 +12,7 @@
 
 #define IPC_GROUP_KERNEL_NAME se2_group_kernel
 #define IPC_GROUP_KEEP_TRIAL false
+#define IPC_GROUP_LAZY_SD false
 #include "se2_group_kernel_def.hpp"
 #undef IPC_GROUP_KERNEL_NAME
 #undef IPC_GROUP_KEEP_TRIAL
@@ -20,15 +21,24 @@
 #include "se2_group_kernel_def.hpp"
 #undef IPC_GROUP_KERNEL_NAME
 #undef IPC_GROUP_KEEP_TRIAL
+#undef IPC_GROUP_LAZY_SD
+#define IPC_GROUP_KERNEL_NAME se2_group_kernel_lz
+#define IPC_GROUP_KEEP_TRIAL (M <= kLazyKeepTrialMaxM)
+#define IPC_GROUP_LAZY_SD true
+#include "se2_group_kernel_def.hpp"
+#undef IPC_GROUP_KERNEL_NAME
+#undef IPC_GROUP_KEEP_TRIAL
+#undef IPC_GROUP_LAZY_SD
 
-template <int W, int M, int NL, bool STAGED, bool KEEP_TRIAL>
+template <int W, int M, int NL, bool STAGED, bool KEEP_TRIAL, bool LAZY_SD>
 constexpr auto se2_group_kernel_of()
 {
-    if constexpr (KEEP_TRIAL) return &se2_group_kernel_kt<W, M, NL, STAGED>;
+    if constexpr (LAZY_SD) return &se2_group_kernel_lz<W, M, NL, STAGED>;
+    else if constexpr (KEEP_TRIAL) return &se2_group_kernel_kt<W, M, NL, STAGED>;
     else return &se2_group_kernel<W, M, NL, STAGED>;
 }
 
-template <int W, int M, int NL, bool KEEP_TRIAL = false>
+template <int W, int M, int NL, bool KEEP_TRIAL = false, bool LAZY_SD = false>
 static hipError_t launch_group(int n, hipStream_t st, const Se2View& P, const int2* cells, SolveParams prm, CellOut out,
                               unsigned* counter, int n_cu)
 {
@@ -39,12 +49,12 @@
     const size_t staged = scratch + sizeof(double) * (size_t)F_SG * wstride;
     const int groups = std::max(1, std::min(n_cu, (n + kPairs - 1) / kPairs));
     if (staged <= (size_t)kLdsBudget) {
-        auto k = se2_group_kernel_of<W, M, NL, true, KEEP_TRIAL>();
+        auto k = se2_group_kernel_of<W, M, NL, true, KEEP_TRIAL, LAZY_SD>();
         hipError_t e = hipFuncSetAttribute(reinterpret_cast<const void*>(k), hipFuncAttributeMaxDynamicSharedMemorySize, (int)staged);
         if (e != hipSuccess) return e;
         hipLaunchKernelGGL(k, dim3(groups), dim3(64 * kWavesPerGroup), staged, st, P, cells, n, counter, prm, out, 0, E, wstride);
     } else {
-        auto k = se2_group_kernel_of<W, M, NL, false, KEEP_TRIAL>();
+        auto k = se2_group_kernel_of<W, M, NL, false, KEEP_TRIAL, LAZY_SD>();
         hipLaunchKernelGGL(k, dim3(groups), dim3(64 * kWavesPerGroup), scratch, st, P, cells, n, counter, prm, out, 0, E, wstride);
     }
     return hipGetLastError();
diff --git a/ipc_amd/csrc/se2_group_kernel_def.hpp b/ipc_amd/csrc/se2_group_kernel_def.hpp
--- a/ipc_amd/csrc/se2_group_kernel_def.hpp
+++ b/ipc_amd/csrc/se2_group_kernel_def.hpp
@@ -49,8 +49,8 @@
         const int base = NL == 1 ? prm.fast_iter : prm.slow_iter;
         const int iterations = (L + NL > 100) ? base * 5 : base;
         CellResult r;
-        se2_wave_solve<M, NL, STAGED, W, se2_err_store<M>(), IPC_GROUP_KEEP_TRIAL>(P, lo, L, cand, iterations, sh, cst, wlo,
-                                                                                   wstride, r, box, seq, &seq);
+        se2_wave_solve<M, NL, STAGED, W, se2_err_store<M>(), IPC_GROUP_KEEP_TRIAL, IPC_GROUP_LAZY_SD>(P, lo, L, cand, iterations, sh, cst,
+                                                                                                      wlo, wstride, r, box, seq, &seq);
         if (wsub == 0 && lane == 0) {
             out.max_chi2[c] = r.max_chi2;
             out.chi2_total[c] = r.chi2_total;
diff --git a/ipc_amd/csrc/se2_pair_lz.hip b/ipc_amd/csrc/se2_pair_lz.hip
--- /dev/null
+++ b/ipc_amd/csrc/se2_pair_lz.hip
@@ -0,0 +1,23 @@
+#include "se2_group_kernel.hpp"
+
+namespace ipc {
+hipError_t launch_se2_pair_lz(int nl, int M, int n, hipStream_t st, const Se2View& P, const int2* cells, SolveParams prm,
+                              CellOut out, unsigned* counter, int n_cu)
+{
+#define IPC_PCASE(MM)                                                                                                  \
+    case MM:                                                                                                           \
+        return nl == 1 ? launch_group<2, MM, 1, (MM <= kLazyKeepTrialMaxM), true>(n, st, P, cells, prm, out, counter, n_cu)    \
+                       : launch_group<2, MM, 2, (MM <= kLazyKeepTrialMaxM), true>(n, st, P, cells, prm, out, counter, n_cu);
+    switch (M) {
+#ifdef IPC_PAIR_LZ_ONLY_M
+        IPC_PCASE(IPC_PAIR_LZ_ONLY_M)
+#else
+        IPC_PCASE(7)
+        IPC_PCASE(9)
+        IPC_PCASE(11)
+#endif
+        default: return hipErrorInvalidValue;
+    }
+#undef IPC_PCASE
+}
+}
diff --git a/ipc_amd/csrc/se2_wave_cell.hpp b/ipc_amd/csrc/se2_wave_cell.hpp
--- a/ipc_amd/csrc/se2_wave_cell.hpp
+++ b/ipc_amd/csrc/se2_wave_cell.hpp
@@ -168,7 +168,17 @@
     Y.c = __hiloint2double(h3, l3); Y.s = __hiloint2double(h4, l4);
 }
 
-template <int M, int NL, bool STAGED, int W = 1, int E_STORE = se2_err_store<M>(), bool KEEP_TRIAL = false>
+__device__ __forceinline__ double wave_sum16_entry1(double v)
+{
+    const double r0 = pair32(v, 0.0);
+    double q = pair16(r0, 0.0);
+    q = row_inclusive_scan(q);
+    return read_lane(q, 15);
+}
+constexpr double kLazySdMaxBb = 0x1p500;
+
+template <int M, int NL, bool STAGED, int W = 1, int E_STORE = se2_err_store<M>(), bool KEEP_TRIAL = false,
+          bool LAZY_SD = false>
 __device__ __forceinline__ void se2_wave_solve(const Se2View& P, int lo_abs, int L, const int (&cand)[2], int iterations,
                                WaveScratch<NL>& sh, const double* cst, int wlo, int wstride, CellResult& res,
                                PairBox* box = nullptr, int seq0 = 0, int* seq_out = nullptr)
@@ -184,7 +194,7 @@
     int j0 = gl * M + 1;
 
 #ifdef IPC_PHASE_TIMING
-    unsigned long long gnEvals = 0, gnRejected = 0, nBig = 0, tmBig = 0, tmSmall = 0;
+    unsigned long long gnEvals = 0, gnRejected = 0, nBig = 0, tmBig = 0, tmSmall = 0, nSd = 0;
     unsigned long long tmA = 0, tmB1 = 0, tmB2 = 0, tmC = 0, tmT = 0, tmW = 0, tmK = 0, tm0 = __builtin_amdgcn_s_memtime();
 #define IPC_WTICK(acc) { const unsigned long long t_ = __builtin_amdgcn_s_memtime(); acc += t_ - tm0; tm0 = t_; }
 #else
@@ -339,6 +349,13 @@
                 if (lf[l] == 0) { pf[0] = gauge.x; pf[1] = gauge.y; pf[2] = gauge.th; pf[3] = gauge.c; pf[4] = gauge.s; }
                 if (lt[l] == 0) { pt[0] = gauge.x; pt[1] = gauge.y; pt[2] = gauge.th; pt[3] = gauge.c; pt[4] = gauge.s; }
             }
+        if constexpr (LAZY_SD) {
+#pragma unroll
+            for (int l = 0; l < NL; ++l) {
+                if (lf[l] == 0) { sh.lvec[l][0][0] = 0.0; sh.lvec[l][0][1] = 0.0; sh.lvec[l][0][2] = 0.0; }
+                if (lt[l] == 0) { sh.lvec[l][1][0] = 0.0; sh.lvec[l][1][1] = 0.0; sh.lvec[l][1][2] = 0.0; }
+            }
+        }
     }
 
     int eloc = gl * M < L ? gl * M : 0;
@@ -611,6 +628,7 @@
         opaque();
         launder();
         {
+            if constexpr (!LAZY_SD) {
 #pragma unroll
             for (int l = 0; l < NL; ++l) {
                 if (gl == 0) {
@@ -624,13 +642,14 @@
                     if (st_[l] == s && gl == ot[l]) { sh.lvec[l][1][0] = bx[s]; sh.lvec[l][1][1] = by[s]; sh.lvec[l][1][2] = bth[s]; }
                 }
             }
+            }
             double v1[16], v2[16];
 #pragma unroll
             for (int k = 0; k < 16; ++k) { v1[k] = 0.0; v2[k] = 0.0; }
             v1[0] = bbp;
             double qbx, qby, qbth;
-            prev3(bx[M - 1], by[M - 1], bth[M - 1], qbx, qby, qbth);
-            constexpr int kWantB = 2 | 4 | 8 | kErrWantBC;
+            if constexpr (!LAZY_SD) prev3(bx[M - 1], by[M - 1], bth[M - 1], qbx, qby, qbth);
+            constexpr int kWantB = 2 | (LAZY_SD ? 0 : 4) | 8 | kErrWantBC;
             SlotConst Kn;
             if (PF) ld_slot(0, Kn, IntC<kWantB>{});
 #pragma unroll
@@ -641,10 +660,12 @@
                 const Pose2& a = s == 0 ? a0 : X[s - 1];
                 const bool v = j0 + s <= L;
                 const double cz = K.cz, sz = K.sz;
+                if constexpr (!LAZY_SD) {
                 double wx, wy, wth;
                 se2_apply_J(a, X[s], cz, sz, qbx, qby, qbth, bx[s], by[s], bth[s], wx, wy, wth);
                 const double hq = K.om.quad(wx, wy, wth);
                 v1[1] += v ? hq : 0.0;
+                }
                 const Sym3 sg = K.sg;
                 const double c = a.c * cz - a.s * sz, sn = a.s * cz + a.c * sz;
                 const double kx = -(X[s].y - gauge.y), ky = X[s].x - gauge.x;
@@ -678,7 +699,11 @@
 #pragma unroll
                     for (int k = 0; k < 6; ++k) { v2[3 + k] += m2 * psi[k]; v2[9 + k] += m12 * psi[k]; }
                 }
-                qbx = bx[s]; qby = by[s]; qbth = bth[s];
+                if constexpr (!LAZY_SD) { qbx = bx[s]; qby = by[s]; qbth = bth[s]; }
+                if constexpr (LAZY_SD)
+                    asm volatile("" : "+v"(v1[0]), "+v"(v1[2]), "+v"(v1[3]), "+v"(v1[4]), "+v"(v1[5]),
+                                 "+v"(v1[6]), "+v"(v1[7]), "+v"(v1[8]), "+v"(v1[9]), "+v"(v1[10]) : : "memory");
+                else
                 asm volatile("" : "+v"(v1[0]), "+v"(v1[1]), "+v"(v1[2]), "+v"(v1[3]), "+v"(v1[4]), "+v"(v1[5]),
                              "+v"(v1[6]), "+v"(v1[7]), "+v"(v1[8]), "+v"(v1[9]), "+v"(v1[10]) : : "memory");
                 if constexpr (NL == 2)
@@ -714,21 +739,27 @@
                 for (int k = 0; k < 6; ++k) mred[o][k] = sh.red[o][mb + k];
 #pragma unroll
                 for (int k = 0; k < 3; ++k) wred[o][k] = sh.red[o][wb + k];
-                bred[o][0] = sh.red[o][0]; bred[o][1] = sh.red[o][1];
+                bred[o][0] = sh.red[o][0];
+                if constexpr (!LAZY_SD) bred[o][1] = sh.red[o][1];
             }
             const int lo_ = i < k3 ? i : k3, hi_ = i < k3 ? k3 : i;
             const double sgv = sh.lc[l1].sg[lo_ * 3 - lo_ * (lo_ - 1) / 2 + (hi_ - lo_)];
+            Pose2 qa, qb;
+            double qcz, qsz;
+            Sym3 qom;
+            double qv[2][3];
+            if constexpr (!LAZY_SD) {
             const LoopConst& qq = sh.lc[lq_l];
             const LoopState& sq = sh.ls[cur][lq_l];
-            const Pose2 qa{sq.pf[0], sq.pf[1], sq.pf[2], sq.pf[3], sq.pf[4]};
-            const Pose2 qb{sq.pt[0], sq.pt[1], sq.pt[2], sq.pt[3], sq.pt[4]};
-            const double qcz = qq.cz, qsz = qq.sz;
-            const Sym3 qom{qq.om[0], qq.om[1], qq.om[2], qq.om[3], qq.om[4], qq.om[5]};
-            double qv[2][3];
+            qa = Pose2{sq.pf[0], sq.pf[1], sq.pf[2], sq.pf[3], sq.pf[4]};
+            qb = Pose2{sq.pt[0], sq.pt[1], sq.pt[2], sq.pt[3], sq.pt[4]};
+            qcz = qq.cz; qsz = qq.sz;
+            qom = Sym3{qq.om[0], qq.om[1], qq.om[2], qq.om[3], qq.om[4], qq.om[5]};
 #pragma unroll
             for (int e = 0; e < 2; ++e)
 #pragma unroll
                 for (int k = 0; k < 3; ++k) qv[e][k] = sh.lvec[lq_l][e][k];
+            }
             __builtin_amdgcn_sched_barrier(0);
             double g1[3], g2[3], gam;
             {
@@ -756,6 +787,12 @@
                 for (int o = 1; o < W; ++o) w[k] += wred[o][k];
             }
             bb = bred[0][0];
+            if constexpr (LAZY_SD) {
+                bHb = 0.0;
+#pragma unroll
+                for (int o = 1; o < W; ++o) bb += bred[o][0];
+                IPC_PIN1(bb);
+            } else {
             bHb = bred[0][1];
 #pragma unroll
             for (int o = 1; o < W; ++o) { bb += bred[o][0]; bHb += bred[o][1]; }
@@ -767,6 +804,7 @@
                 for (int l = 0; l < NL; ++l) bHb += read_lane(lq, l);
             }
             IPC_PIN2(bb, bHb);
+            }
             __builtin_amdgcn_sched_barrier(0);
             double val;
             {
@@ -794,12 +832,14 @@
                 double inv = __builtin_amdgcn_rcp(piv);
                 inv = fma(fma(-piv, inv, 1.0), inv, inv);
                 inv = fma(fma(-piv, inv, 1.0), inv, inv);
+                if constexpr (!LAZY_SD) {
                 if (k == 0) {
                     alpha = bb / bHb;
                     IPC_PIN1(alpha);
                 } else if (k == 1) {
                     hsdNorm = sqrt(alpha * alpha * bb);
                     IPC_PIN1(hsdNorm);
+                }
                 }
                 __builtin_amdgcn_sched_barrier(0);
                 val = (r == k) ? rowk * inv : fma(-(colk * rowk), inv, val);
@@ -894,12 +934,109 @@
         }
         IPC_WTICK(tmC)
         if (lastGN && hgnNorm < delta && fabs(bh) < term_scale * currentChi) { it_done = it + 1; tries_total += maxTrials; flags |= 1; break; }
+        [[maybe_unused]] bool sdReady = false;
+        [[maybe_unused]] auto sd_terms = [&]() {
+#ifdef IPC_PHASE_TIMING
+            ++nSd;
+#endif
+            __builtin_amdgcn_sched_barrier(0);
+            asm volatile(";ipc_sd_terms_begin" : : : "memory");
+            opaque();
+            launder();
+#pragma unroll
+            for (int l = 0; l < NL; ++l) {
+#pragma unroll
+                for (int s = 0; s < M; ++s) {
+                    if (!((ownSlots >> s) & 1u)) continue;
+                    if (sf[l] == s && gl == of[l]) { sh.lvec[l][0][0] = bx[s]; sh.lvec[l][0][1] = by[s]; sh.lvec[l][0][2] = bth[s]; }
+                    if (st_[l] == s && gl == ot[l]) { sh.lvec[l][1][0] = bx[s]; sh.lvec[l][1][1] = by[s]; sh.lvec[l][1][2] = bth[s]; }
+                }
+            }
+            Pose2 cr = gauge;
+            double c0 = 0.0, c1 = 0.0, c2 = 0.0;
+            if constexpr (W > 1) {
+                double a[8] = {read_lane(X[M - 1].x, 63), read_lane(X[M - 1].y, 63), read_lane(X[M - 1].th, 63),
+                               read_lane(X[M - 1].c, 63), read_lane(X[M - 1].s, 63),
+                               read_lane(bx[M - 1], 63), read_lane(by[M - 1], 63), read_lane(bth[M - 1], 63)};
+                post_wait(a, 8);
+                if (wsub > 0) {
+                    cr.x = peer(wsub - 1, 0); cr.y = peer(wsub - 1, 1); cr.th = peer(wsub - 1, 2); cr.c = peer(wsub - 1, 3);
+                    cr.s = peer(wsub - 1, 4);
+                    c0 = peer(wsub - 1, 5); c1 = peer(wsub - 1, 6); c2 = peer(wsub - 1, 7);
+                }
+            } else {
+                wave_sync();
+            }
+            Pose2 as0;
+            as0.x = lane_prev(X[M - 1].x, cr.x); as0.y = lane_prev(X[M - 1].y, cr.y); as0.th = lane_prev(X[M - 1].th, cr.th);
+            as0.c = lane_prev(X[M - 1].c, cr.c); as0.s = lane_prev(X[M - 1].s, cr.s);
+            double qbx = lane_prev(bx[M - 1], c0), qby = lane_prev(by[M - 1], c1), qbth = lane_prev(bth[M - 1], c2);
+            double acc = 0.0;
+            constexpr int kWantS = 2 | 4;
+            SlotConst Kn;
+            if (PF) ld_slot(0, Kn, IntC<kWantS>{});
+#pragma unroll
+            for (int s = 0; s < M; ++s) {
+                SlotConst K;
+                if (PF) { K = Kn; if (s + 1 < M) ld_slot(s + 1, Kn, IntC<kWantS>{}); }
+                else ld_slot(s, K, IntC<kWantS>{});
+                const Pose2& a = s == 0 ? as0 : X[s - 1];
+                const bool v = j0 + s <= L;
+                const double cz = K.cz, sz = K.sz;
+                double wx, wy, wth;
+                se2_apply_J(a, X[s], cz, sz, qbx, qby, qbth, bx[s], by[s], bth[s], wx, wy, wth);
+                const double hq = K.om.quad(wx, wy, wth);
+                acc += v ? hq : 0.0;
+                qbx = bx[s]; qby = by[s]; qbth = bth[s];
+                IPC_PIN1(acc);
+                IPC_SLOT_FENCE();
+            }
+            const double t = wave_sum16_entry1(acc);
+            if constexpr (W > 1) {
+                double a[8] = {t, 0, 0, 0, 0, 0, 0, 0};
+                post_wait(a, 1);
+                bHb = wsub == 0 ? t : peer(0, 0);
+#pragma unroll
+                for (int o = 1; o < W; ++o) bHb += o == wsub ? t : peer(o, 0);
+            } else {
+                bHb = t;
+            }
+            {
+                int bl = lane;
+                asm volatile("" : "+v"(bl));
+                const int lq_l = bl < NL ? bl : 0;
+                const LoopConst& qq = sh.lc[lq_l];
+                const LoopState& sq = sh.ls[cur][lq_l];
+                const Pose2 qa{sq.pf[0], sq.pf[1], sq.pf[2], sq.pf[3], sq.pf[4]};
+                const Pose2 qb{sq.pt[0], sq.pt[1], sq.pt[2], sq.pt[3], sq.pt[4]};
+                const double qcz = qq.cz, qsz = qq.sz;
+                const Sym3 qom{qq.om[0], qq.om[1], qq.om[2], qq.om[3], qq.om[4], qq.om[5]};
+                double qv[2][3];
+#pragma unroll
+                for (int e = 0; e < 2; ++e)
+#pragma unroll
+                    for (int k = 0; k < 3; ++k) qv[e][k] = sh.lvec[lq_l][e][k];
+                double wx, wy, wth;
+                se2_apply_J(qa, qb, qcz, qsz, qv[0][0], qv[0][1], qv[0][2], qv[1][0], qv[1][1], qv[1][2], wx, wy, wth);
+                const double lq = bl < NL ? qom.quad(wx, wy, wth) : 0.0;
+#pragma unroll
+                for (int l = 0; l < NL; ++l) bHb += read_lane(lq, l);
+            }
+            alpha = bb / bHb;
+            hsdNorm = sqrt(alpha * alpha * bb);
+            IPC_PIN3(bHb, alpha, hsdNorm);
+            __builtin_amdgcn_sched_barrier(0);
+            asm volatile(";ipc_sd_terms_end" : : : "memory");
+        };
         const double deltaAtEntry = delta;
         bool goodStep = false, dlReady = false;
         double dlC = 0.0, dlBma = 0.0;
         int numTries = 0;
         do {
             ++numTries;
+            if constexpr (LAZY_SD) {
+                if (!sdReady && __ballot(!(hgnNorm < delta) || !(bb <= kLazySdMaxBb)) != 0ull) { sd_terms(); sdReady = true; }
+            }
             int stepType;
             double beta = 0.0, sdScale = 0.0;
             if (hgnNorm < delta) stepType = 0;
@@ -1000,6 +1137,7 @@
         atomicAdd(d + 6, (unsigned long long)it_done); atomicAdd(d + 7, (unsigned long long)evals);
         atomicAdd(d + 8, (unsigned long long)it_done * (unsigned long long)L);
         atomicAdd(d + 9, 1ull); atomicAdd(d + 10, tmK); atomicAdd(d + 11, (unsigned long long)(evals - 1 - it_done)); atomicAdd(d + 12, gnEvals); atomicAdd(d + 13, gnRejected); atomicAdd(d + 14, nBig); atomicAdd(d + 15, tmBig); atomicAdd(d + 1024, tmSmall);
+        if constexpr (LAZY_SD) atomicAdd(d + 1025, nSd);
     }
 #endif
 
diff --git a/ipc_amd/csrc/se2_wave_kernel.hpp b/ipc_amd/csrc/se2_wave_kernel.hpp
--- a/ipc_amd/csrc/se2_wave_kernel.hpp
+++ b/ipc_amd/csrc/se2_wave_kernel.hpp
@@ -12,6 +12,7 @@
 
 #define IPC_WAVE_KERNEL_NAME se2_wave_kernel
 #define IPC_WAVE_KEEP_TRIAL false
+#define IPC_WAVE_LAZY_SD false
 #include "se2_wave_kernel_def.hpp"
 #undef IPC_WAVE_KERNEL_NAME
 #undef IPC_WAVE_KEEP_TRIAL
@@ -20,11 +21,20 @@
 #include "se2_wave_kernel_def.hpp"
 #undef IPC_WAVE_KERNEL_NAME
 #undef IPC_WAVE_KEEP_TRIAL
+#undef IPC_WAVE_LAZY_SD
+#define IPC_WAVE_KERNEL_NAME se2_wave_kernel_lz
+#define IPC_WAVE_KEEP_TRIAL (M <= kLazyKeepTrialMaxM)
+#define IPC_WAVE_LAZY_SD true
+#include "se2_wave_kernel_def.hpp"
+#undef IPC_WAVE_KERNEL_NAME
+#undef IPC_WAVE_KEEP_TRIAL
+#undef IPC_WAVE_LAZY_SD
 
-template <int M, int NL, bool STAGED, bool KEEP_TRIAL>
+template <int M, int NL, bool STAGED, bool KEEP_TRIAL, bool LAZY_SD>
 constexpr auto se2_wave_kernel_of()
 {
-    if constexpr (KEEP_TRIAL) return &se2_wave_kernel_kt<M, NL, STAGED>;
+    if constexpr (LAZY_SD) return &se2_wave_kernel_lz<M, NL, STAGED>;
+    else if constexpr (KEEP_TRIAL) return &se2_wave_kernel_kt<M, NL, STAGED>;
     else return &se2_wave_kernel<M, NL, STAGED>;
 }
 
@@ -33,7 +43,7 @@
 #endif
 constexpr int kLdsBudget = IPC_LDS_BUDGET;
 
-template <int M, int NL, bool KEEP_TRIAL>
+template <int M, int NL, bool KEEP_TRIAL, bool LAZY_SD = false>
 static hipError_t launch_wave_one(int n, hipStream_t st, const Se2View& P, const int2* cells, SolveParams prm, CellOut out,
                                   unsigned* counter, int n_cu)
 {
@@ -44,12 +54,12 @@
     const size_t staged = scratch + sizeof(double) * (size_t)F_SG * wstride;
     const int groups = std::max(1, std::min(n_cu, (n + kWavesPerGroup - 1) / kWavesPerGroup));
     if (staged <= (size_t)kLdsBudget) {
-        auto k = se2_wave_kernel_of<M, NL, true, KEEP_TRIAL>();
+        auto k = se2_wave_kernel_of<M, NL, true, KEEP_TRIAL, LAZY_SD>();
         hipError_t e = hipFuncSetAttribute(reinterpret_cast<const void*>(k), hipFuncAttributeMaxDynamicSharedMemorySize, (int)staged);
         if (e != hipSuccess) return e;
         hipLaunchKernelGGL(k, dim3(groups), dim3(64 * kWavesPerGroup), staged, st, P, cells, n, counter, prm, out, 0, E, wstride);
     } else {
-        auto k = se2_wave_kernel_of<M, NL, false, KEEP_TRIAL>();
+        auto k = se2_wave_kernel_of<M, NL, false, KEEP_TRIAL, LAZY_SD>();
         hipLaunchKernelGGL(k, dim3(groups), dim3(64 * kWavesPerGroup), scratch, st, P, cells, n, counter, prm, out, 0, E, wstride);
     }
     return hipGetLastError();
diff --git a/ipc_amd/csrc/se2_wave_kernel_def.hpp b/ipc_amd/csrc/se2_wave_kernel_def.hpp
--- a/ipc_amd/csrc/se2_wave_kernel_def.hpp
+++ b/ipc_amd/csrc/se2_wave_kernel_def.hpp
@@ -31,8 +31,8 @@
         const int base = NL == 1 ? prm.fast_iter : prm.slow_iter;
         const int iterations = (L + NL > 100) ? base * 5 : base;
         CellResult r;
-        se2_wave_solve<M, NL, STAGED, 1, se2_err_store<M>(), IPC_WAVE_KEEP_TRIAL>(P, lo, L, cand, iterations, sh, cst, wlo,
-                                                                                  wstride, r);
+        se2_wave_solve<M, NL, STAGED, 1, se2_err_store<M>(), IPC_WAVE_KEEP_TRIAL, IPC_WAVE_LAZY_SD>(P, lo, L, cand, iterations, sh, cst,
+                                                                                                    wlo, wstride, r);
         if (lane == 0) {
             out.max_chi2[c] = r.max_chi2;
             out.chi2_total[c] = r.chi2_total;
diff --git a/ipc_amd/csrc/se2_wave_lz.hip b/ipc_amd/csrc/se2_wave_lz.hip
--- /dev/null
+++ b/ipc_amd/csrc/se2_wave_lz.hip
@@ -0,0 +1,26 @@
+#include "se2_wave_kernel.hpp"
+
+namespace ipc {
+hipError_t launch_se2_wave_lz(int nl, int M, int n, hipStream_t st, const Se2View& P, const int2* cells, SolveParams prm,
+                              CellOut out, unsigned* counter, int n_cu)
+{
+#define IPC_WCASE(MM)                                                                                                  \
+    case MM:                                                                                                           \
+        return nl == 1 ? launch_wave_one<MM, 1, (MM <= kLazyKeepTrialMaxM), true>(n, st, P, cells, prm, out, counter, n_cu)    \
+                       : launch_wave_one<MM, 2, (MM <= kLazyKeepTrialMaxM), true>(n, st, P, cells, prm, out, counter, n_cu);
+    switch (M) {
+#ifdef IPC_WAVE_LZ_ONLY_M
+        IPC_WCASE(IPC_WAVE_LZ_ONLY_M)
+#else
+        IPC_WCASE(5)
+        IPC_WCASE(7)
+        IPC_WCASE(9)
+        IPC_WCASE(11)
+        IPC_WCASE(13)
+#endif
+        default: return hipErrorInvalidValue;
+    }
+#undef IPC_WCASE
+}
+
+}
```

Measured after the change: 2.095 million candidate-pairs/s (median of 6 runs). 1.6% higher.
